# JuliaGraphics/Hikari.jl

Measured on AMD Instinct MI355X. Metric: Mrays/s, higher is better.
Workload: dtype f32

## Files before the change

hikari.jl_amd/_abi.py:

```python
import ctypes as C

c_f = C.c_float
c_i = C.c_int32
c_u = C.c_uint32
PF = C.POINTER(C.c_float)

HK_OK = 0
HK_ERR_INVALID, HK_ERR_DEVICE, HK_ERR_UNSUPPORTED = -1, -2, -3
HK_UNSET = -100

(HK_MAT_MATTE, HK_MAT_MIRROR, HK_MAT_GLASS, HK_MAT_CONDUCTOR, HK_MAT_COATED_DIFFUSE, HK_MAT_THIN_DIELECTRIC,
 HK_MAT_DIFFUSE_TRANSMISSION, HK_MAT_COATED_DIFFUSE_TRANSMISSION, HK_MAT_COATED_CONDUCTOR, HK_MAT_MIX,
 HK_MAT_FALLBACK) = range(11)
HK_MATF_REMAP_ROUGHNESS, HK_MATF_USE_ETA_K = 1, 2
(HK_LIGHT_POINT, HK_LIGHT_SPOT, HK_LIGHT_DIRECTIONAL, HK_LIGHT_SUN, HK_LIGHT_AMBIENT, HK_LIGHT_ENVIRONMENT,
 HK_LIGHT_DIFFUSE_AREA) = range(7)
HK_SPEC_RGB, HK_SPEC_ILLUMINANT = 0, 1
HK_TONEMAP_NONE, HK_TONEMAP_REINHARD, HK_TONEMAP_REINHARD_EXT, HK_TONEMAP_ACES, HK_TONEMAP_UNCHARTED2, HK_TONEMAP_FILMIC = range(6)
HK_MEDIUM_HOMOGENEOUS, HK_MEDIUM_GRID, HK_MEDIUM_RGB_GRID, HK_MEDIUM_NANOVDB = range(4)
HK_FILTER_BOX, HK_FILTER_TRIANGLE, HK_FILTER_GAUSSIAN, HK_FILTER_MITCHELL, HK_FILTER_LANCZOS = 1, 2, 3, 4, 5
HK_COHERENCE_NONE, HK_COHERENCE_SORTED, HK_COHERENCE_PER_TYPE = 0, 1, 2


class hk_texture(C.Structure):
    _fields_ = [("width", c_i), ("height", c_i), ("channels", c_i), ("kind", c_i), ("data", PF)]


class hk_tex_rgba(C.Structure):
    _fields_ = [("c", c_f * 4), ("tex", c_i)]


class hk_tex_f32(C.Structure):
    _fields_ = [("v", c_f), ("tex", c_i)]


class hk_material(C.Structure):
    _fields_ = [("kind", c_i), ("flags", c_i), ("rgb", hk_tex_rgba * 4), ("f", hk_tex_f32 * 8), ("i", c_i * 4),
                ("spectrum", c_i * 2), ("mix_key", c_u * 4)]


class hk_pl_spectrum(C.Structure):
    _fields_ = [("n", c_i), ("_pad", c_i), ("lambdas", PF), ("values", PF)]


class hk_medium_interface(C.Structure):
    _fields_ = [("material", c_i), ("inside", c_i), ("outside", c_i)]


class hk_tri_meta(C.Structure):
    _fields_ = [("medium_interface_idx", c_u), ("primitive_index", c_u), ("arealight_flat_idx_1based", c_u)]


class hk_light(C.Structure):
    _fields_ = [("kind", c_i), ("spectrum_kind", c_i), ("i_rgb", c_f * 4), ("poly", c_f * 3), ("illum_scale", c_f),
                ("scale", c_f), ("position", c_f * 3), ("direction", c_f * 3), ("world_to_light", c_f * 16),
                ("light_to_world", c_f * 16), ("cos_total_width", c_f), ("cos_falloff_start", c_f), ("v", c_f * 9),
                ("normal", c_f * 3), ("area", c_f), ("uv", c_f * 6), ("Le", hk_tex_rgba), ("two_sided", c_i),
                ("envmap", c_i)]


class hk_envmap(C.Structure):
    _fields_ = [("width", c_i), ("height", c_i), ("data", PF), ("rotation", c_f * 9), ("nu", c_i), ("nv", c_i),
                ("conditional_func", PF), ("conditional_cdf", PF), ("conditional_func_int", PF), ("marginal_func", PF),
                ("marginal_cdf", PF), ("marginal_func_int", c_f), ("_pad", c_i)]


class hk_medium(C.Structure):
    _fields_ = [("kind", c_i), ("sigma_a", c_f * 4), ("sigma_s", c_f * 4), ("Le", c_f * 4), ("g", c_f),
                ("sigma_scale", c_f), ("Le_scale", c_f), ("bounds_min", c_f * 3), ("bounds_max", c_f * 3),
                ("render_to_medium", c_f * 16), ("medium_to_render", c_f * 16), ("res", c_i * 3), ("density", PF),
                ("sigma_a_grid", PF), ("sigma_s_grid", PF), ("Le_grid", PF), ("majorant_res", c_i * 3),
                ("majorant", PF), ("max_density", c_f), ("nvdb_bytes", C.POINTER(C.c_uint8)), ("nvdb_size", C.c_int64),
                ("root_offset_1based", C.c_int64), ("upper_offset_1based", C.c_int64),
                ("lower_offset_1based", C.c_int64), ("leaf_offset_1based", C.c_int64), ("upper_count", c_i),
                ("lower_count", c_i), ("leaf_count", c_i), ("root_table_size", c_i), ("inv_mat", c_f * 9),
                ("vec", c_f * 3), ("index_bbox_min", c_i * 3), ("index_bbox_max", c_i * 3)]


class hk_scene_desc(C.Structure):
    _fields_ = [("n_triangles", c_i), ("n_materials", c_i), ("n_textures", c_i), ("n_media_interfaces", c_i),
                ("n_lights", c_i), ("n_envmaps", c_i), ("n_media", c_i), ("n_spectra", c_i), ("positions", PF),
                ("normals", PF), ("uvs", PF), ("tangents", PF), ("meta", C.POINTER(hk_tri_meta)),
                ("materials", C.POINTER(hk_material)), ("textures", C.POINTER(hk_texture)),
                ("media_interfaces", C.POINTER(hk_medium_interface)), ("lights", C.POINTER(hk_light)),
                ("envmaps", C.POINTER(hk_envmap)), ("media", C.POINTER(hk_medium)),
                ("spectra", C.POINTER(hk_pl_spectrum))]


class hk_tables(C.Structure):
    _fields_ = [("sobol_matrices", C.POINTER(c_u)), ("sobol_count", c_i), ("rgb2spec_res", c_i), ("cie_x", PF),
                ("cie_y", PF), ("cie_z", PF), ("rgb2spec_scale", PF), ("rgb2spec_coeffs", PF)]


class hk_integrator_params(C.Structure):
    _fields_ = [("max_depth", c_i), ("samples_per_pixel", c_i), ("russian_roulette_depth", c_i), ("regularize", c_i),
                ("material_coherence", c_i), ("max_component_value", c_f), ("filter_type", c_i),
                ("filter_radius", c_f * 2), ("filter_param1", c_f), ("filter_param2", c_f), ("accumulate_f64", c_i),
                ("sampler_seed", c_u), ("samples_per_pass", c_i)]


class hk_postprocess_params(C.Structure):
    _fields_ = [("exposure", c_f), ("tonemap", c_i), ("inv_gamma", c_f), ("apply_gamma", c_i), ("white_point", c_f),
                ("imaging_ratio", c_f), ("apply_wb", c_i), ("wb", c_f * 9), ("mask_escaped", c_i), ("bg", c_f * 3)]


class hk_denoise_params(C.Structure):
    _fields_ = [("iterations", c_i), ("sigma_color", c_f), ("sigma_normal", c_f), ("sigma_depth", c_f), ("use_variance", c_i)]


class hk_camera(C.Structure):
    _fields_ = [("raster_to_camera", c_f * 16), ("camera_to_world", c_f * 16), ("lens_radius", c_f),
                ("focal_distance", c_f), ("shutter_open", c_f), ("shutter_close", c_f), ("dx_camera", c_f * 3),
                ("dy_camera", c_f * 3)]


class hk_stats(C.Structure):
    _fields_ = [("rays_closest", C.c_uint64), ("rays_shadow", C.c_uint64), ("bvh_nodes_visited", C.c_uint64),
                ("tris_tested", C.c_uint64), ("hits_accepted", C.c_uint64), ("path_vertices", C.c_uint64),
                ("medium_collisions", C.c_uint64), ("light_bvh_nodes", C.c_uint64), ("seconds_trace", C.c_double),
                ("seconds_total", C.c_double), ("trace_launches", C.c_uint64), ("trace_nodes", C.c_uint64),
                ("trace_tris", C.c_uint64), ("shadow_nodes", C.c_uint64), ("shadow_tris", C.c_uint64),
                ("shadow_launches", C.c_uint64), ("shade_launches", C.c_uint64), ("seconds_shadow", C.c_double),
                ("seconds_shade", C.c_double), ("seconds_other", C.c_double), ("bytes_algorithmic_trace", C.c_uint64),
                ("bytes_algorithmic_shadow", C.c_uint64), ("bytes_algorithmic_shade", C.c_uint64), ("seconds_media", C.c_double),
                ("track_collisions", C.c_uint64), ("shadow_collisions", C.c_uint64), ("track_dda_steps", C.c_uint64),
                ("shadow_dda_steps", C.c_uint64), ("scatter_vertices", C.c_uint64), ("media_launches", C.c_uint64),
                ("bytes_algorithmic_media", C.c_uint64), ("seconds_select", C.c_double), ("select_launches", C.c_uint64),
                ("fused_passes", C.c_uint64), ("view_cache_hits", C.c_uint64)]


EXPORTED_SYMBOLS = [
    "hk_ctx_create", "hk_ctx_destroy", "hk_last_error", "hk_ctx_set_tables", "hk_scene_create", "hk_scene_destroy",
    "hk_integrator_create", "hk_integrator_destroy", "hk_film_create", "hk_film_destroy", "hk_film_clear", "hk_render",
    "hk_film_read_rgb", "hk_film_read_accum", "hk_film_accum_device_ptr", "hk_sync", "hk_stats_get", "hk_stats_reset",
    "hk_stats_enable_counters", "hk_trace_closest", "hk_test_sobol", "hk_test_camera", "hk_test_uplift",
    "hk_test_light_bvh", "hk_test_bsdf", "hk_film_postprocess", "hk_film_fill_aux", "hk_postprocess", "hk_test_light", "hk_scene_bvh_info", "hk_scene_light_bvh_copy",
    "hk_denoise", "hk_test_mix", "hk_test_medium", "hk_test_trace_lean",
    "hk_render_tile", "hk_comm_create", "hk_comm_unique_id", "hk_comm_create_rank", "hk_comm_destroy", "hk_film_reduce",
    "hk_ctx_set_option", "hk_ctx_get_option", "hk_trim_cache", "hk_flush", "hk_film_read_rgb_async", "hk_film_read_wait",
    "hk_film_pin_host", "hk_film_unpin_host", "hk_scene_set_transform", "hk_scene_update_materials", "hk_scene_update_lights", "hk_scene_update_envmap",
    "hk_film_update_aux", "hk_film_read_aux", "hk_film_present", "hk_film_present_async",
    "hk_scene_update_medium", "hk_scene_medium_copy", "hk_test_medium_bricks",
]
```

hikari.jl_amd/csrc/hk_ctx.cpp:

```cpp
#include "hk_host.h"

thread_local std::string g_err;
SlabCache g_slabs;

namespace hk {
static thread_local const Knobs* tl_knobs = nullptr;
const char* knob(const char* name) {
    if (!tl_knobs) return nullptr;
    auto it = tl_knobs->kv.find(name);
    return it == tl_knobs->kv.end() ? nullptr : it->second.c_str();
}
static const char* const KNOB_NAMES[] = {
    "HK_BATCH_PATHS_M", "HK_BVH_LEAF", "HK_BVH_BINS", "HK_QNODES", "HK_DEBUG_ALLOC", "HK_DELTA_ADVANCE", "HK_DYNAMIC_SEGMENTS", "HK_GREY", "HK_GREY_COMPACT", "HK_GREY_FLAT", "HK_MAX_PATHS_M",
    "HK_MID_LISTS", "HK_MID_PASS_PATHS_M", "HK_NODE_CACHE", "HK_NVDB_DENSE_MB", "HK_OVERLAP", "HK_PIPELINE", "HK_PIPELINE_AFTER", "HK_PIPELINE_MAX_PATHS_M", "HK_PRESELECT",
    "HK_SELECT_MIN_IDLE", "HK_SHADOW_FEED_ROUNDS", "HK_SHADOW_TRACK_BATCH", "HK_SMALL_PASS", "HK_SMALL_PASS_WAVES", "HK_SOBOL_LO_GB", "HK_SOBOL_TABLE_ONLY",
    "HK_STATE_CACHE_GB", "HK_STATE_SLAB", "HK_TICKET_SHARE", "HK_TRACK_ADVANCE", "HK_TRACK_EXTRA_ADVANCE", "HK_TRACK_MIN_PENDING", "HK_TRACK_POOL", "HK_TRACK_REFILL_IDLE",
    "HK_WALK_POOL", "HK_WALK_REFILL_IDLE", "HK_WALK_SPLIT", "HK_WAVES_PER_CU", "HK_READBACK_PIN", "HK_DEFER_EXTERNAL", "HK_SELECT_POOL", "HK_SMALL_PASS_FUSED", "HK_SMALL_PASS_MERGED", "HK_OCC_SCALE", "HK_ESCAPED_UNROLL", "HK_SHADOW_FINAL", "HK_TRI_PACK", "HK_LEAN_RECORDS", "HK_VIEW_CACHE", "HK_MAJORANT_BLOCK_VOXELS"};
static bool known_knob(const char* name) {
    for (const char* k : KNOB_NAMES)
        if (std::strcmp(k, name) == 0) return true;
    return false;
}
}
KnobScope::KnobScope(const hk::Knobs* k) : prev(hk::tl_knobs) { hk::tl_knobs = k; }
KnobScope::~KnobScope() { hk::tl_knobs = prev; }

void quiesce(hk_ctx* c) {
    if (!c) return;
    (void)hipStreamSynchronize(c->stream);
    if (c->aux) (void)hipStreamSynchronize(c->aux);
    for (auto& l : c->lanes)
        if (l.stream) (void)hipStreamSynchronize(l.stream);
}
int join_lanes(hk_ctx* c) {
    if (!c) return HK_OK;
    if (int e = flush_pending(c)) return e;
    if (!c->lanes_dirty) return HK_OK;
    for (auto& l : c->lanes)
        if (l.done) HIP_TRY(hipStreamWaitEvent(c->stream, l.done, 0));
    c->lanes_dirty = false;
    c->film_chain = false;
    if (c->have_span) HIP_TRY(hipEventRecord(c->ev_end, c->stream));
    return HK_OK;
}
hipEvent_t get_event(hk_ctx* c) {
    if (!c->event_pool.empty()) {
        hipEvent_t e = c->event_pool.back();
        c->event_pool.pop_back();
        return e;
    }
    hipEvent_t e;
    (void)hipEventCreate(&e);
    return e;
}
DCamera make_camera(const hk_camera& c) {
    DCamera d;
    std::memcpy(d.r2c, c.raster_to_camera, 64);
    std::memcpy(d.c2w, c.camera_to_world, 64);
    d.lens_radius = c.lens_radius;
    d.focal_distance = c.focal_distance;
    d.shutter_open = c.shutter_open;
    d.shutter_close = c.shutter_close;
    return d;
}

extern "C" const char* hk_last_error(void) { return g_err.c_str(); }

extern "C" int32_t hk_ctx_create(int32_t device_id, void* stream, hk_ctx** out) {
    if (!out) return fail(HK_ERR_INVALID, "out is null");
    int n = 0;
    HIP_TRY(hipGetDeviceCount(&n));
    if (device_id < 0 || device_id >= n) return fail(HK_ERR_INVALID, "bad device id");
    HIP_TRY(hipSetDevice(device_id));
    hk_ctx* c = new hk_ctx();
    c->device = device_id;
    c->stream = (hipStream_t)stream;
    hipDeviceProp_t prop;
    HIP_TRY(hipGetDeviceProperties(&prop, device_id));
    c->n_cu = prop.multiProcessorCount > 0 ? prop.multiProcessorCount : 256;
    c->own_stream_order = stream == nullptr;
    for (const char* name : hk::KNOB_NAMES)
        if (const char* e = std::getenv(name)) c->knobs.kv[name] = e;
    KnobScope knobs(&c->knobs);
    {
        c->waves_per_cu = hk::knob_int_in("HK_WAVES_PER_CU", 1, INT_MAX, 0);
        c->stat_rows = c->n_cu * 32 * 2;
        if (const char* e = hk::knob("HK_OVERLAP")) c->overlap = std::atoi(e) ? 1 : 0;
        else c->overlap = -1;
        if (const char* e = hk::knob("HK_STATE_CACHE_GB"))
            if (std::atol(e) >= 0) g_slabs.cap_bytes = (size_t)std::atol(e) << 30;
    }
    {
        std::vector<DStats> zero((size_t)c->stat_rows);
        std::memset(zero.data(), 0, zero.size() * sizeof(DStats));
        HIP_TRY(c->stats.upload(zero.data(), zero.size() * sizeof(DStats)));
    }
    HIP_TRY(hipEventCreate(&c->ev_begin));
    HIP_TRY(hipEventCreate(&c->ev_end));
    *out = c;
    return HK_OK;
}
extern "C" int32_t hk_ctx_destroy(hk_ctx* c) {
    if (!c) return HK_OK;
    (void)hipSetDevice(c->device);
    int status = join_lanes(c);
    if (hipStreamSynchronize(c->stream) != hipSuccess && status == HK_OK) status = fail(HK_ERR_DEVICE, "hk_ctx_destroy: the context's stream reports an error");
    for (auto& l : c->lanes) {
        if (l.stream) (void)hipStreamSynchronize(l.stream);
        if (l.done) (void)hipEventDestroy(l.done);
        if (l.stream) (void)hipStreamDestroy(l.stream);
    }
    if (c->ev_main) (void)hipEventDestroy(c->ev_main);
    if (c->ev_film) (void)hipEventDestroy(c->ev_film);
    for (auto& e : c->trace_events) {
        (void)hipEventDestroy(e.first);
        (void)hipEventDestroy(e.second);
    }
    for (auto e : c->event_pool) (void)hipEventDestroy(e);
    if (c->ev_begin) (void)hipEventDestroy(c->ev_begin);
    if (c->ev_end) (void)hipEventDestroy(c->ev_end);
    if (c->ev_fork) (void)hipEventDestroy(c->ev_fork);
    if (c->ev_join) (void)hipEventDestroy(c->ev_join);
    if (c->aux) (void)hipStreamDestroy(c->aux);
    g_slabs.trim(c->device);
    delete c;
    return status;
}
extern "C" int32_t hk_ctx_set_option(hk_ctx* c, const char* name, const char* value) {
    if (!c || !name) return fail(HK_ERR_INVALID, "null argument");
    if (!hk::known_knob(name)) return fail(HK_ERR_INVALID, std::string("unknown option ") + name);
    HIP_TRY(hipSetDevice(c->device));
    if (int e = join_lanes(c)) return e;
    if (value) c->knobs.kv[name] = value;
    else c->knobs.kv.erase(name);
    if (std::strcmp(name, "HK_STATE_CACHE_GB") == 0) {
        g_slabs.cap_bytes = (size_t)(value && std::atol(value) >= 0 ? std::atol(value) : 128) << 30;
        if (g_slabs.cap_bytes == 0) g_slabs.trim(c->device);
    }
    return HK_OK;
}
extern "C" int32_t hk_ctx_get_option(hk_ctx* c, const char* name, char* out, int32_t out_bytes) {
    if (!c || !name || (out_bytes > 0 && !out)) return fail(HK_ERR_INVALID, "null argument");
    if (!hk::known_knob(name)) return fail(HK_ERR_INVALID, std::string("unknown option ") + name);
    auto it = c->knobs.kv.find(name);
    if (it == c->knobs.kv.end()) {
        if (out_bytes > 0) out[0] = 0;
        return HK_UNSET;
    }
    if (out_bytes > 0) std::snprintf(out, (size_t)out_bytes, "%s", it->second.c_str());
    return (int32_t)it->second.size();
}
extern "C" int32_t hk_flush(hk_ctx* c) {
    if (!c) return fail(HK_ERR_INVALID, "null ctx");
    HIP_TRY(hipSetDevice(c->device));
    return join_lanes(c);
}
extern "C" int32_t hk_trim_cache(hk_ctx* c) {
    if (!c) return fail(HK_ERR_INVALID, "null ctx");
    HIP_TRY(hipSetDevice(c->device));
    g_slabs.trim(c->device);
    return HK_OK;
}
extern "C" int32_t hk_ctx_set_tables(hk_ctx* c, const hk_tables* t) {
    if (!c || !t || !t->sobol_matrices || t->sobol_count < 104 || !t->cie_x || !t->rgb2spec_coeffs) return fail(HK_ERR_INVALID, "bad tables");
    HIP_TRY(hipSetDevice(c->device));
    if (int e = flush_pending(c)) return e;
    if (c->lanes_dirty) {
        if (int e = join_lanes(c)) return e;
        HIP_TRY(hipStreamSynchronize(c->stream));
    }
    HIP_TRY(c->sobol.upload(t->sobol_matrices, 104 * sizeof(uint32_t)));
    std::vector<float> cie(3 * 471);
    std::memcpy(&cie[0], t->cie_x, 471 * 4);
    std::memcpy(&cie[471], t->cie_y, 471 * 4);
    std::memcpy(&cie[942], t->cie_z, 471 * 4);
    HIP_TRY(c->cie.upload(cie.data(), cie.size() * 4));
    int res = t->rgb2spec_res;
    size_t nco = (size_t)3 * res * res * res * 3;
    c->h_r2s_scale.assign(t->rgb2spec_scale, t->rgb2spec_scale + res);
    c->h_r2s_coeffs.assign(t->rgb2spec_coeffs, t->rgb2spec_coeffs + nco);
    c->r2s_host.res = res;
    c->r2s_host.scale = c->h_r2s_scale.data();
    c->r2s_host.coeffs = c->h_r2s_coeffs.data();
    HIP_TRY(c->r2s_scale.upload(t->rgb2spec_scale, res * 4));
    HIP_TRY(c->r2s_coeffs.upload(t->rgb2spec_coeffs, nco * 4));
    {
        const size_t R = (size_t)res;
        std::vector<float> pts(3 * R * R * R * 4);
        for (size_t m = 0; m < 3; ++m)
            for (size_t z = 0; z < R; ++z)
                for (size_t y = 0; y < R; ++y)
                    for (size_t x = 0; x < R; ++x) {
                        float* o = &pts[((((m * R + z) * R + y) * R) + x) * 4];
                        for (size_t k = 0; k < 3; ++k) o[k] = t->rgb2spec_coeffs[m + 3 * (z + R * (y + R * (x + R * k)))];
                        o[3] = 0.0f;
                    }
        HIP_TRY(c->r2s_points.upload(pts.data(), pts.size() * 4));
        bool sorted = true;
        for (int i = 1; i < res; ++i)
            if (!(t->rgb2spec_scale[i - 1] <= t->rgb2spec_scale[i])) sorted = false;
        c->tables.rgb2spec_sorted = sorted ? 1 : 0;
    }
    bool closed = true;
    {
        uint32_t col = 0x80000000u;
        for (int b = 0; b < 52; ++b) {
            uint32_t d0 = b < 32 ? (0x80000000u >> b) : 0u;
            if (t->sobol_matrices[b] != d0) closed = false;
            if (b % 32 == 0) col = 0x80000000u;
            if (t->sobol_matrices[52 + b] != col) closed = false;
            col ^= col >> 1;
        }
    }
    c->tables.sobol = closed ? nullptr : c->sobol.as<uint32_t>();
    c->tables.cie = c->cie.as<float>();
    c->tables.rgb2spec_scale = c->r2s_scale.as<float>();
    c->tables.rgb2spec_coeffs = c->r2s_coeffs.as<float>();
    c->tables.rgb2spec_res = res;
    c->tables.rgb2spec_points = c->r2s_points.as<float4>();
    c->have_tables = true;
    c->tables_epoch++;
    return HK_OK;
}

extern "C" int32_t hk_sync(hk_ctx* c) {
    if (!c) return fail(HK_ERR_INVALID, "null ctx");
    HIP_TRY(hipSetDevice(c->device));
    if (int e = join_lanes(c)) return e;
    HIP_TRY(hipStreamSynchronize(c->stream));
    if (c->aux) HIP_TRY(hipStreamSynchronize(c->aux));
    return HK_OK;
}
extern "C" int32_t hk_stats_enable_counters(hk_ctx* c, int32_t flags) {
    if (!c) return fail(HK_ERR_INVALID, "null ctx");
    if (int e = join_lanes(c)) return e;
    c->count_nodes = (flags & 1) ? 1 : 0;
    c->time_kernels = (flags & 2) ? 1 : 0;
    return HK_OK;
}
extern "C" int32_t hk_stats_reset(hk_ctx* c) {
    if (!c) return fail(HK_ERR_INVALID, "null ctx");
    HIP_TRY(hipSetDevice(c->device));
    if (int e = join_lanes(c)) return e;
    HIP_TRY(hipStreamSynchronize(c->stream));
    HIP_TRY(hipMemset(c->stats.p, 0, (size_t)c->stat_rows * sizeof(DStats)));
    for (auto& l : c->lanes)
        if (l.stats.p) HIP_TRY(hipMemset(l.stats.p, 0, (size_t)c->stat_rows * sizeof(DStats)));
    for (auto& e : c->trace_events) {
        c->event_pool.push_back(e.first);
        c->event_pool.push_back(e.second);
    }
    c->trace_events.clear();
    for (auto& v : c->class_events) {
        for (auto& e : v) {
            c->event_pool.push_back(e.first);
            c->event_pool.push_back(e.second);
        }
        v.clear();
    }
    c->seconds_trace = c->seconds_total = 0.0;
    c->trace_launches = c->shadow_launches = c->shade_launches = c->media_launches = c->select_launches = 0;
    c->fused_passes = c->view_cache_hits = 0;
    c->have_span = false;
    return HK_OK;
}
extern "C" int32_t hk_stats_get(hk_ctx* c, hk_stats* out) {
    if (!c || !out) return fail(HK_ERR_INVALID, "null argument");
    HIP_TRY(hipSetDevice(c->device));
    if (int e = join_lanes(c)) return e;
    HIP_TRY(hipStreamSynchronize(c->stream));
    DStats h{};
    {
        std::vector<const void*> blocks{c->stats.p};
        for (const auto& l : c->lanes)
            if (l.stats.p) blocks.push_back(l.stats.p);
        std::vector<DStats> rows((size_t)c->stat_rows * blocks.size());
        for (size_t b = 0; b < blocks.size(); ++b)
            HIP_TRY(hipMemcpy(rows.data() + b * (size_t)c->stat_rows, blocks[b], (size_t)c->stat_rows * sizeof(DStats), hipMemcpyDeviceToHost));
        for (const DStats& r : rows) {
            h.rays_closest += r.rays_closest;
            h.rays_shadow += r.rays_shadow;
            h.nodes += r.nodes;
            h.tris += r.tris;
            h.hits += r.hits;
            h.vertices += r.vertices;
            h.collisions += r.collisions;
            h.light_nodes += r.light_nodes;
            h.sh_nodes += r.sh_nodes;
            h.sh_tris += r.sh_tris;
            h.sh_collisions += r.sh_collisions;
            h.nvdb_collisions += r.nvdb_collisions;
            h.sh_nvdb_collisions += r.sh_nvdb_collisions;
            h.dda_steps += r.dda_steps;
            h.sh_dda_steps += r.sh_dda_steps;
            h.scatter_vertices += r.scatter_vertices;
            h.sc_light_nodes += r.sc_light_nodes;
#ifdef HK_DEBUG_UTIL
            for (int k = 0; k < 32; ++k) h.dbg[k] += r.dbg[k];
#endif
        }
#ifdef HK_DEBUG_UTIL
        for (int k = 0; k < 16; ++k)
            if (h.dbg[2 * k]) std::fprintf(stderr, "HK_DEBUG_UTIL[%d]: %.3f of %llu lane-slots\n", k, (double)h.dbg[2 * k + 1] / (double)h.dbg[2 * k], h.dbg[2 * k]);
#endif
    }
    double tr = 0.0;
    for (auto& e : c->trace_events) {
        float ms = 0.0f;
        if (hipEventElapsedTime(&ms, e.first, e.second) == hipSuccess) tr += ms * 1e-3;
    }
    double total = 0.0;
    if (c->have_span) {
        float ms = 0.0f;
        if (hipEventElapsedTime(&ms, c->ev_begin, c->ev_end) == hipSuccess) total = ms * 1e-3;
    }
    std::memset(out, 0, sizeof *out);
    out->rays_closest = h.rays_closest;
    out->rays_shadow = h.rays_shadow;
    out->bvh_nodes_visited = h.nodes;
    out->tris_tested = h.tris;
    out->hits_accepted = h.hits;
    out->path_vertices = h.vertices;
    out->medium_collisions = h.collisions + h.sh_collisions;
    out->track_collisions = h.collisions;
    out->shadow_collisions = h.sh_collisions;
    out->track_dda_steps = h.dda_steps;
    out->shadow_dda_steps = h.sh_dda_steps;
    out->scatter_vertices = h.scatter_vertices;
    out->light_bvh_nodes = h.light_nodes + h.sc_light_nodes;
    out->seconds_trace = tr;
    out->seconds_total = total;
    out->trace_launches = c->trace_launches;
    out->trace_nodes = h.nodes;
    out->trace_tris = h.tris;
    out->shadow_nodes = h.sh_nodes;
    out->shadow_tris = h.sh_tris;
    out->bvh_nodes_visited = h.nodes + h.sh_nodes;
    out->tris_tested = h.tris + h.sh_tris;
    out->shadow_launches = c->shadow_launches;
    out->shade_launches = c->shade_launches;
    out->media_launches = c->media_launches;
    double cls[6] = {0, 0, 0, 0, 0, 0};
    for (int k = 1; k < 6; ++k)
        for (auto& e : c->class_events[k]) {
            float ms = 0.0f;
            if (hipEventElapsedTime(&ms, e.first, e.second) == hipSuccess) cls[k] += ms * 1e-3;
        }
    out->seconds_shadow = cls[1];
    out->seconds_shade = cls[2] + cls[5];
    out->seconds_other = cls[3];
    out->seconds_media = cls[4];
    out->seconds_select = cls[5];
    out->select_launches = c->select_launches;
    out->fused_passes = c->fused_passes;
    out->view_cache_hits = c->view_cache_hits;
    {
        const uint64_t hits_closest = h.hits < h.rays_closest ? h.hits : h.rays_closest;
        out->bytes_algorithmic_trace = h.rays_closest * (32 + 16) + 64 * h.nodes + 36 * h.tris + 96 * hits_closest;
        out->bytes_algorithmic_shadow = h.rays_shadow * (32 + 16) + 64 * h.sh_nodes + 36 * h.sh_tris;
        out->bytes_algorithmic_shade = h.vertices * (2 * 104 + 64 + 96) + 60 * h.light_nodes;
        out->bytes_algorithmic_media = h.collisions * 36 + h.nvdb_collisions * (84 - 36) + 4 * h.dda_steps + h.scatter_vertices * (2 * 104 + 96) + 60 * h.sc_light_nodes;
        out->bytes_algorithmic_shadow += h.sh_collisions * 36 + h.sh_nvdb_collisions * (84 - 36) + 4 * h.sh_dda_steps;
    }
    return HK_OK;
}
```

hikari.jl_amd/csrc/hk_host.h:

```cpp
#pragma once
#include <hip/hip_runtime.h>

#include <climits>
#include <cstddef>
#include <cmath>
#include <cstdio>
#include <cstdlib>
#include <cstring>
#include <limits>
#include <map>
#include <memory>
#include <mutex>
#include <string>
#include <unordered_map>
#include <vector>

#include "bvh_build.h"
#include "hikari_mi355x.h"
#include "hk_launch.h"
#include "hk_nanovdb.h"
#include "hk_types.h"

#pragma GCC visibility push(hidden)

extern thread_local std::string g_err;
inline int fail(int code, const std::string& msg) {
    g_err = msg;
    return code;
}

namespace hk {
struct Knobs {
    std::unordered_map<std::string, std::string> kv;
};
}
struct KnobScope {
    const hk::Knobs* prev;
    explicit KnobScope(const hk::Knobs* k);
    ~KnobScope();
};
#define HIP_TRY(expr)                                                                                          \
    do {                                                                                                       \
        hipError_t e_ = (expr);                                                                                \
        if (e_ != hipSuccess) return fail(HK_ERR_DEVICE, std::string(#expr) + ": " + hipGetErrorString(e_)); \
    } while (0)

struct SlabCache {
    struct Entry {
        void* p;
        size_t bytes;
        int dev;
    };
    std::mutex m;
    std::vector<Entry> free_list;
    size_t cap_bytes = (size_t)128 << 30;
    size_t cap() const { return cap_bytes; }
    size_t total(int dev) {
        std::lock_guard<std::mutex> g(m);
        size_t t = 0;
        for (const Entry& e : free_list) t += e.dev == dev ? e.bytes : 0;
        return t;
    }
    void* take(int dev, size_t need, size_t& got) {
        std::lock_guard<std::mutex> g(m);
        int best = -1;
        for (int i = 0; i < (int)free_list.size(); ++i) {
            const Entry& e = free_list[i];
            if (e.dev == dev && e.bytes >= need && e.bytes <= 2 * need + ((size_t)64 << 20) && (best < 0 || e.bytes < free_list[best].bytes)) best = i;
        }
        if (best < 0) return nullptr;
        void* p = free_list[best].p;
        got = free_list[best].bytes;
        free_list.erase(free_list.begin() + best);
        return p;
    }
    void give(int dev, void* p, size_t bytes) {
        std::vector<void*> drop;
        {
            std::lock_guard<std::mutex> g(m);
            free_list.push_back(Entry{p, bytes, dev});
            size_t t = 0;
            for (const Entry& e : free_list) t += e.bytes;
            const size_t limit = cap();
            while (!free_list.empty() && (t > limit || free_list.size() > 8)) {
                int k = 0;
                for (int i = 1; i < (int)free_list.size(); ++i)
                    if (free_list[i].bytes < free_list[k].bytes) k = i;
                t -= free_list[k].bytes;
                drop.push_back(free_list[k].p);
                free_list.erase(free_list.begin() + k);
            }
        }
        for (void* q : drop) (void)hipFree(q);
    }
    void trim(int dev) {
        std::vector<void*> drop;
        {
            std::lock_guard<std::mutex> g(m);
            for (int i = (int)free_list.size() - 1; i >= 0; --i)
                if (dev < 0 || free_list[i].dev == dev) {
                    drop.push_back(free_list[i].p);
                    free_list.erase(free_list.begin() + i);
                }
        }
        for (void* q : drop) (void)hipFree(q);
    }
};
extern SlabCache g_slabs;
struct DevBuf {
    void* p = nullptr;
    size_t bytes = 0;
    int slab_dev = -1;
    void release() {
        if (p && slab_dev >= 0) {
            g_slabs.give(slab_dev, p, bytes);
        } else if (p)
            (void)hipFree(p);
        p = nullptr, bytes = 0, slab_dev = -1;
    }
    ~DevBuf() { release(); }
    hipError_t alloc(size_t n) {
        release();
        bytes = n;
        if (n == 0) return hipSuccess;
        hipError_t e = hipMalloc(&p, n);
        if (e != hipSuccess) {
            (void)hipGetLastError();
            g_slabs.trim(-1);
            e = hipMalloc(&p, n);
        }
        if (e != hipSuccess) p = nullptr, bytes = 0;
        return e;
    }
    hipError_t alloc_slab(int dev, size_t n) {
        release();
        size_t got = 0;
        if (void* q = g_slabs.take(dev, n, got)) {
            p = q, bytes = got, slab_dev = dev;
            return hipSuccess;
        }
        const hipError_t e = alloc(n);
        if (e == hipSuccess) slab_dev = dev;
        return e;
    }
    hipError_t upload(const void* src, size_t n) {
        hipError_t e = alloc(n ? n : 4);
        if (e != hipSuccess) return e;
        if (n) e = hipMemcpy(p, src, n, hipMemcpyHostToDevice);
        return e;
    }
    template <class T>
    T* as() const {
        return reinterpret_cast<T*>(p);
    }
};

struct hk_ctx {
    int device = 0;
    hk::Knobs knobs;
    bool own_stream_order = true;
    hipStream_t stream = nullptr;
    hipStream_t aux = nullptr;
    hipEvent_t ev_fork = nullptr, ev_join = nullptr;
    int overlap = -1;
    int small_streak = 0;
    int n_cu = 256;
    int waves_per_cu = 0;
    int stat_rows = 8192;
    DevBuf sobol, cie, r2s_scale, r2s_coeffs, r2s_points, stats;
    DTables tables{};
    bool have_tables = false;
    unsigned tables_epoch = 0;
    std::vector<float> h_r2s_scale, h_r2s_coeffs;
    hk::RGB2Spec r2s_host;
    int count_nodes = 0, time_kernels = 0;
    unsigned long long fused_passes = 0;
    unsigned long long view_cache_hits = 0;
    std::vector<std::pair<hipEvent_t, hipEvent_t>> trace_events;
    std::vector<std::pair<hipEvent_t, hipEvent_t>> class_events[6];
    uint64_t shadow_launches = 0, shade_launches = 0, media_launches = 0, select_launches = 0;
    std::vector<hipEvent_t> event_pool;
    hipEvent_t ev_begin = nullptr, ev_end = nullptr;
    bool have_span = false;
    double seconds_trace = 0.0, seconds_total = 0.0;
    uint64_t trace_launches = 0;
    DStats host_stats{};
    struct Lane {
        hipStream_t stream = nullptr;
        hipEvent_t done = nullptr;
        DevBuf stats;
    };
    enum { MAX_LANES = 16 };
    Lane lanes[MAX_LANES];
    int next_lane = 0;
    struct Pending {
        bool active = false;
        hk_scene* sc = nullptr;
        hk_integrator* I = nullptr;
        hk_film* film = nullptr;
        hk_camera cam{};
        int first = 0, n = 0, stride = 1, x0 = 0, y0 = 0, x1 = 0, y1 = 0, calls = 0;
    } pending;
    bool lanes_dirty = false;
    bool film_chain = false;
    hipEvent_t ev_main = nullptr, ev_film = nullptr;
};

void quiesce(hk_ctx* c);
int flush_pending(hk_ctx* c);
int join_lanes(hk_ctx* c);
hipEvent_t get_event(hk_ctx* c);
DCamera make_camera(const hk_camera& c);

struct hk_scene {
    hk_ctx* ctx = nullptr;
    DevBuf nodes, qnodes, leaf_tris, positions, normals, uvs, tangents, meta, tri_shade, materials, textures, spectra, mis, lights, lnodes, trails, infinite;
    DevBuf envmaps;
    DevBuf media;
    DScene d{};
    uint32_t kinds_mask = 0;
    int n_materials = 0;
    int bvh_nodes = 0, bvh_leaf_tris = 0, bvh_depth = 0;
    hk::LightBVH lbvh;
    std::vector<hk_material> h_materials;
    std::vector<hk_light> h_lights;
    std::vector<DEnvMap> h_envmaps;
    int n_textures = 0, n_spectra = 0;
    std::vector<int> level_start;
    DevBuf base_pos, base_nrm, base_tan, slot_of_prim;
    bool have_base = false;
    bool qnodes_built = false;
    enum { XF_BLOCK = 1024 };
    std::vector<float> block_box;
    struct Xf {
        int end;
        bool identity;
        float m[12];
    };
    std::map<int, Xf> xf;
    struct Staging {
        void* host = nullptr;
        size_t bytes = 0;
        hipEvent_t ev = nullptr;
    };
    std::vector<Staging> staging;
    struct Medium {
        hk_medium rec{};
        DMedium d{};
        DevBuf *majorant = nullptr, *maj_zero = nullptr, *density = nullptr, *rgb[3] = {nullptr, nullptr, nullptr};
        DevBuf *nvdb = nullptr, *blocks = nullptr, *bricks = nullptr;
    };
    std::vector<Medium> h_media;
    std::vector<std::unique_ptr<DevBuf>> owned;
    DevBuf& own() {
        owned.emplace_back(new DevBuf());
        return *owned.back();
    }
    ~hk_scene() {
        for (auto& st : staging) {
            if (st.ev) (void)hipEventSynchronize(st.ev), (void)hipEventDestroy(st.ev);
            if (st.host) (void)hipHostFree(st.host);
        }
    }
};
void bake_material(const hk::RGB2Spec& t, const hk_material& m, DMaterial& o);
bool material_alpha_tested(const hk_material& m);
void bake_light(const hk::RGB2Spec& r2s, const hk_light& l, DLight& o);
std::string check_medium_record(const hk_medium& m);
void bake_medium_fields(const hk::RGB2Spec& r2s, const hk_medium& m, DMedium& o);
struct NvdbPlan {
    int nvb_min[3] = {0, 0, 0}, nvb_dim[3] = {0, 0, 0};
    float background = 0.0f;
    long long total = 0;
    std::vector<uint2> table;
    bool bricks = false;
    void fill(DMedium& o) const;
};
int plan_nanovdb(const hk_medium& m, NvdbPlan& p);
struct MediaClasses {
    int media_mask = 0, all_grey = 0, grey_pool = 0, grey_bricks = 0;
};
MediaClasses classify_media(const std::vector<DMedium>& dmed, int n_media);
inline size_t light_table_capacity(int n_lights) { return n_lights > 0 ? (size_t)n_lights : 1; }

struct hk_film {
    hk_ctx* ctx = nullptr;
    int width = 0, height = 0;
    bool f64 = false;
    DevBuf own;
    void* accum = nullptr;
    bool external = false;
    bool exposed = false;
    DevBuf readback;
    float* staging[2] = {nullptr, nullptr};
    int staging_next = 0, staging_last = -1;
    bool read_in_flight = false;
    hipEvent_t ev_read = nullptr;
    void* last_out = nullptr;
    void* pinned_user = nullptr;
    bool pinned_explicit = false;
    void* pin_failed = nullptr;
    DevBuf guides, albedo;
    DevBuf frame[2], variance;
    bool have_aux = false;
};

struct hk_integrator {
    hk_ctx* ctx = nullptr;
    hk_integrator_params p{};
    DFilter filter{};
    DevBuf f_func, f_mcdf, f_mfunc, f_ccdf;
    DPathState st{};
    std::vector<std::unique_ptr<DevBuf>> bufs;
    int st_capacity = 0, st_depth = 0, st_media = -1;
    DPathGen cam_gen{};
    bool cam_unfit = false;
    std::string view_key;
    bool mid_pass = false;
    int slab_mode = 0;
    void* slab_base = nullptr;
    size_t slab_off = 0;
    DevBuf sobol_table;
    int sobol_rows = 0, sobol_stride = 0, sobol_log2 = -1, sobol_digits = -1, sobol_x0 = -1, sobol_y0 = -1, sobol_tiles_x = -1;
    DevBuf sobol_lo;
    int lo_rows = 0, lo_base = -1, lo_sample_stride = -1, lo_count = 0;
    struct StateSet {
        DPathState st{};
        std::vector<std::unique_ptr<DevBuf>> bufs;
        int st_capacity = 0, st_depth = 0, st_media = -1;
        DPathGen cam_gen{};
        bool cam_unfit = false;
        std::string view_key;
    };
    std::vector<StateSet> lane_sets;
    void swap_set(StateSet& o) {
        std::swap(st, o.st);
        std::swap(bufs, o.bufs);
        std::swap(st_capacity, o.st_capacity);
        std::swap(st_depth, o.st_depth);
        std::swap(st_media, o.st_media);
        std::swap(cam_gen, o.cam_gen);
        std::swap(cam_unfit, o.cam_unfit);
        std::swap(view_key, o.view_key);
    }
};
int ceil_log2(long v);
DSobol make_sobol(const hk_integrator_params& p, int w, int h);

struct hk_comm {
    std::vector<hk_ctx*> ctxs;
    std::vector<void*> comms;
    int world = 1;
};

#pragma GCC visibility pop
```

hikari.jl_amd/csrc/hk_kernels.hip:

```cpp
#include <hip/hip_runtime.h>
#include <type_traits>
#include <cstdlib>
#include <cstdio>

#include "hikari_mi355x.h"
#include "hk_device.h"

using namespace hkd;

namespace {

__device__ __forceinline__ int lane_id() { return (int)(threadIdx.x & 63); }

struct WaveQ {
    uint32_t* base;
    int count;
};
__device__ __forceinline__ int global_wave() {
    const int w = (int)(threadIdx.x >> 6), b = (int)blockIdx.x;
    if (blockDim.x == 1024 && (gridDim.x & 7) == 0) return ((((b >> 3) * 4 + (w >> 2)) * 8 + (b & 7)) << 2) + (w & 3);
    if (blockDim.x == 512 && (gridDim.x & 7) == 0) return ((((b >> 3) * 2 + (w >> 2)) * 8 + (b & 7)) << 2) + (w & 3);
    return b * (int)(blockDim.x >> 6) + w;
}
__device__ __forceinline__ int physical_waves() { return (int)(gridDim.x * (blockDim.x >> 6)); }
// ... 589 lines not shown
#ifndef HK_LEAF_BREAK_A
#define HK_LEAF_BREAK_A 2
#endif
#ifndef HK_POSTPONE_CLOSEST
#define HK_POSTPONE_CLOSEST 0
#endif
#ifndef HK_POSTPONE_ANYHIT
#define HK_POSTPONE_ANYHIT 0
#endif
#ifndef HK_NODE_UNROLL
#define HK_NODE_UNROLL 3
#endif
struct LaneRay {
    v3 o, d;
    RaySlab rs;
    float t_max;
    HitRec best;
    int cur, sp;
    int pend;
    bool any;
};
template <bool QN = false>
HKD void lane_ray_start(LaneRay& r, const DScene& sc, v3 o, v3 d, float t_max) {
    r.o = o;
    r.d = d;
    r.t_max = t_max;
    r.best.t = t_max;
    r.best.prim = -1;
    r.best.u = r.best.v = 0.0f;
    r.rs = QN ? ray_slab_grid(sc, o, d) : ray_slab(o, d);
    r.sp = 0;
    r.cur = sc.n_tris == 0 ? (int)0x80000000 : sc.root_ref;
    r.pend = (int)0x80000000;
    r.any = false;
}
template <bool ANYHIT, bool COUNT, int NC = 0, bool POSTPONE = (ANYHIT ? HK_POSTPONE_ANYHIT != 0 : HK_POSTPONE_CLOSEST != 0), bool MIXED = false, bool QN = false>
HKD void lane_ray_round(LaneRay& r, bool active, const DScene& sc, int* __restrict__ stack, int lane, unsigned& n_nodes, unsigned& n_tris, const NodeCache& cache = NodeCache(),
                        bool may_wait = false
#ifdef HK_DEBUG_UTIL
                        , unsigned long long* dbg_ = nullptr
#endif
                        ) {
    const int DONE = (int)0x80000000;
    const unsigned long long act_m = __builtin_amdgcn_ballot_w64(active);
    const int break_a = (!ANYHIT && NC > 0 && sc.n_nodes <= NC) ? HK_LEAF_BREAK_A : 1;
    for (;;) {
        const unsigned long long in_nodes = act_m & __builtin_amdgcn_ballot_w64(r.cur >= 0);
        if (in_nodes == 0ull) break;
        const int n_desc = __builtin_popcountll(in_nodes), n_leaf = __builtin_popcountll(act_m & __builtin_amdgcn_ballot_w64((unsigned)r.cur > 0x80000000u));
        if (break_a * n_desc < n_leaf) break;
#ifdef HK_DEBUG_UTIL
        if (dbg_) HK_DBG(0, active && r.cur >= 0);
#endif
#pragma unroll
        for (int rep = 1; rep < HK_NODE_UNROLL; ++rep)
            if (active && r.cur >= 0) {
                if (COUNT) ++n_nodes;
                node_step<NC, QN>(sc, r.rs, r.best.t, stack, lane, r.cur, r.sp, cache);
            }
        if (active && r.cur >= 0) {
            if (COUNT) ++n_nodes;
            node_step<NC, QN>(sc, r.rs, r.best.t, stack, lane, r.cur, r.sp, cache);
            if (POSTPONE) {
                if (r.cur == DONE) {
                    r.cur = r.pend;
                    r.pend = DONE;
                } else if (r.cur < 0 && r.pend == DONE && r.sp > 0) {
                    r.pend = r.cur;
                    --r.sp;
                    r.cur = stack[r.sp * 64 + lane];
                }
            }
        }
    }
    constexpr int LEAF_MIN = ANYHIT ? (NC > 0 ? HK_ANYHIT_LEAF_MIN : 0) : HK_CLOSEST_LEAF_MIN;
    static_assert(LEAF_MIN == 0 || 64 - 2 * LEAF_MIN >= HK_TRACE_MIN_IDLE, "waiting leaf holders must leave enough idle lanes for the caller's refill to trigger");
    if (LEAF_MIN > 0 && may_wait && __builtin_popcountll(act_m & __builtin_amdgcn_ballot_w64((unsigned)r.cur > 0x80000000u)) < LEAF_MIN) return;
    const bool has_pend = POSTPONE && r.pend != DONE;
#ifdef HK_DEBUG_UTIL
    if (dbg_) HK_DBG(1, active && (has_pend || (r.cur < 0 && r.cur != DONE)));
#endif
#ifdef HK_DEBUG_UTIL
    if (dbg_) {
        const bool holds = active && (has_pend || (r.cur < 0 && r.cur != DONE));
        int c = holds ? ((~(has_pend ? r.pend : r.cur)) & 7) + 1 : 0, mx = c, sm = c;
        for (int off = 32; off > 0; off >>= 1) {
            mx = max(mx, __shfl_xor(mx, off));
            sm += __shfl_xor(sm, off);
        }
        dbg_[ANYHIT ? 8 : 12] += 64ull * (unsigned)mx;
        dbg_[ANYHIT ? 9 : 13] += (unsigned)sm;
    }
#endif
    if (active && (has_pend || (r.cur < 0 && r.cur != DONE))) {
        int ref = ~(has_pend ? r.pend : r.cur);
        int first = ref >> 3, count = (ref & 7) + 1;
        bool stop = false;
        if (!ANYHIT && !MIXED) {
            const float4* tp = sc.leaf_tris + 3 * (size_t)first;
            float4 T0 = tp[0], T1 = tp[1], T2 = tp[2];
            for (int i = 0; i < count; ++i) {
                float4 N0 = T0, N1 = T1, N2 = T2;
                if (i + 1 < count) N0 = tp[3 * i + 3], N1 = tp[3 * i + 4], N2 = tp[3 * i + 5];
                asm volatile("" ::"v"(T0.x), "v"(T0.y), "v"(T0.z), "v"(T0.w));
                if (COUNT) ++n_tris;
                float t, u, v;
                if (intersect_triangle(r.o, r.d, r.t_max, mk3(T0.x, T0.y, T0.z), mk3(T1.x, T1.y, T1.z), mk3(T2.x, T2.y, T2.z), t, u, v)) {
                    int prim = __float_as_int(T0.w);
                    if (r.best.prim < 0 || t < r.best.t || (t == r.best.t && prim < r.best.prim)) {
                        r.best.t = t;
                        r.best.prim = prim;
                        r.best.u = u;
                        r.best.v = v;
                    }
                }
                T0 = N0, T1 = N1, T2 = N2;
            }
        } else
        for (int i = 0; i < count && !stop; ++i) {
            const float4* tp = sc.leaf_tris + 3 * (size_t)(first + i);
            float4 T0 = tp[0], T1 = tp[1], T2 = tp[2];
            asm volatile("" ::"v"(T0.x), "v"(T0.y), "v"(T0.z), "v"(T0.w));
            if (COUNT) ++n_tris;
            float t, u, v;
            if (intersect_triangle(r.o, r.d, r.t_max, mk3(T0.x, T0.y, T0.z), mk3(T1.x, T1.y, T1.z), mk3(T2.x, T2.y, T2.z), t, u, v)) {
                int prim = __float_as_int(T0.w);
                if (MIXED ? r.any : ANYHIT) {
                    r.best.t = t;
                    r.best.prim = prim;
                    stop = true;
                } else if (r.best.prim < 0 || t < r.best.t || (t == r.best.t && prim < r.best.prim)) {
                    r.best.t = t;
                    r.best.prim = prim;
                    r.best.u = u;
                    r.best.v = v;
                }
            }
        }
        if (stop) {
            r.cur = DONE;
            if (POSTPONE) r.pend = DONE;
        } else if (has_pend)
            r.pend = DONE;
        else if (r.sp > 0) {
            --r.sp;
            r.cur = stack[r.sp * 64 + lane];
        } else
            r.cur = DONE;
    }
}

enum { LR_EMPTY = 0, LR_ACTIVE = 1 };

template <bool COUNT, int NC, bool QN = false, int MIN_IDLE = HK_TRACE_MIN_IDLE>
__device__ __forceinline__ void trace_lean_body(const DPathState& st, const DScene& sc, int depth, DStats* stats, const SegTickets& src, int* __restrict__ stack, const NodeCache& cache) {
    const int lane = lane_id();
    const unsigned long long lt_mask = (1ull << lane) - 1ull;
    const int DONE = (int)0x80000000;
    unsigned n_nodes = 0, n_tris = 0, n_casts = 0, n_hits = 0;
    HK_DBG_DECL
    HK_FOR_EACH_SEGMENT_FROM(gw, st, src) {
    const DPathGen g = gen_at(st, depth);
    const uint32_t seg = (uint32_t)gw * (uint32_t)st.wave_cap;
    const int n = *count_ptr(st, depth, Q_RAY, gw);
    WaveQ q_escaped = wq_open(st.escaped_q, st, gw);
    int kind_count[HK_MAX_KINDS];
#pragma unroll
    for (int k = 0; k < HK_MAX_KINDS; ++k) kind_count[k] = 0;
    int cursor = 0;
    int state = LR_EMPTY;
    uint32_t slot = 0;
    LaneRay r;
    r.cur = r.pend = DONE;
    for (;;) {
        const unsigned long long run_m = __ballot(state == LR_ACTIVE && r.cur != DONE);
        if (run_m == 0ull || (64 - __popcll(run_m) >= MIN_IDLE && cursor < n)) {
            HK_DBG(8, state == LR_ACTIVE && r.cur == DONE);
            int kind = -1;
            if (state == LR_ACTIVE && r.cur == DONE) {
                if (r.best.prim < 0)
                    kind = -2;
                else {
                    ++n_hits;
                    const DTriMeta hm = sc.meta[r.best.prim];
                    int mat = sc.mis[hm.mi].material;
                    if (sc.materials[mat].kind == HK_MAT_MIX) {
                        float w = 1.0f - r.best.u - r.best.v;
                        mat = resolve_mix_material(sc, mat, r.o + r.d * r.best.t, -r.d, uv_at(sc, r.best.prim, w, r.best.u, r.best.v));
                    }
                    kind = sc.materials[mat].kind;
                    if (kind == HK_MAT_MIX) kind = HK_MAT_FALLBACK;
                    stream_st(&st.hit[slot], make_float4(r.best.t, __int_as_float(r.best.prim), r.best.u, r.best.v));
                    stream_st(reinterpret_cast<uint32_t*>(st.mat_id) + slot, (uint32_t)(mat | (hm.arealight > 0 ? HK_MAT_EMISSIVE_BIT : 0)));
                }
                state = LR_EMPTY;
            }
            wq_push(q_escaped, slot, kind == -2);
            unsigned long long pending = __ballot(kind >= 0);
            while (pending) {
                int src = __ffsll((long long)pending) - 1;
                const int k = __builtin_amdgcn_readlane(kind, src);
                bool mine = kind == k;
                unsigned long long m = __ballot(mine);
                int cnt = 0;
#pragma unroll
                for (int kk = 0; kk < HK_MAX_KINDS; ++kk) cnt = (kk == k) ? kind_count[kk] : cnt;
                if (mine) stream_st(&st.mat_q[((size_t)k * st.n_waves + gw) * st.wave_cap + cnt + __popcll(m & lt_mask)], slot);
                int add = __popcll(m);
#pragma unroll
                for (int kk = 0; kk < HK_MAX_KINDS; ++kk) kind_count[kk] += (kk == k) ? add : 0;
                pending &= ~m;
            }
            const unsigned long long want = __ballot(state == LR_EMPTY);
            const int avail = n - cursor;
            const int rank = __popcll(want & lt_mask);
            if (state == LR_EMPTY && rank < avail) {
                slot = seg + (uint32_t)(cursor + rank);
                float4 O = ld_ray_o(st, g, slot, depth, seg), D = stream_ld(&g.ray_d[slot]);
                ++n_casts;
                lane_ray_start<QN>(r, sc, mk3(O.x, O.y, O.z), mk3(D.x, D.y, D.z), O.w);
                state = LR_ACTIVE;
            }
            const int want_n = __popcll(want);
            cursor += want_n < avail ? want_n : (avail > 0 ? avail : 0);
            if (__ballot(state == LR_ACTIVE) == 0ull) break;
        }
#ifdef HK_DEBUG_UTIL
        HK_DBG(2, state == LR_ACTIVE && r.cur != DONE);
        lane_ray_round<false, COUNT, NC, HK_POSTPONE_CLOSEST != 0, false, QN>(r, state == LR_ACTIVE && r.cur != DONE, sc, stack, lane, n_nodes, n_tris, cache, cursor < n, dbg_);
#else
        lane_ray_round<false, COUNT, NC, HK_POSTPONE_CLOSEST != 0, false, QN>(r, state == LR_ACTIVE && r.cur != DONE, sc, stack, lane, n_nodes, n_tris, cache, cursor < n);
#endif
    }
    wq_close(q_escaped, count_ptr(st, depth, Q_ESCAPED, gw));
    if (lane == 0) {
        *count_ptr(st, depth, Q_MEDIUM, gw) = 0;
#pragma unroll
        for (int k = 0; k < HK_MAX_KINDS; ++k) *count_ptr(st, depth, Q_MAT0 + k, gw) = kind_count[k];
    }
    }
    stats += global_wave();
    wave_add(&stats->rays_closest, n_casts);
    wave_add(&stats->hits, n_hits);
    if (COUNT) {
        wave_add(&stats->nodes, n_nodes);
        wave_add(&stats->tris, n_tris);
    }
    HK_DBG_FLUSH(stats);
}
template <bool COUNT, int STACK, int BLOCK = HK_TRACE_BLOCK, int NC = 0, bool QN = false>
__global__ void __launch_bounds__(BLOCK) k_trace_lean(DPathState st, DScene sc, int depth, DStats* stats) {
    __shared__ int lds_stack[(BLOCK / 64) * STACK * 64];
    __shared__ float4 lds_box[NC > 0 ? 3 * NC : 1];
    __shared__ int2 lds_child[NC > 0 ? NC : 1];
    int* stack = lds_stack + (threadIdx.x >> 6) * (STACK * 64);
    const NodeCache cache = node_cache_fill<NC, BLOCK, QN>(sc, lds_box, lds_child);
    trace_lean_body<COUNT, NC, QN, (NC >= 1024 ? HK_CLOSEST_MIN_IDLE_LDS : HK_TRACE_MIN_IDLE)>(st, sc, depth, stats, seg_open(st, ticket_ptr(st, depth, TK_TRACE), st.dynamic_segments != 0, depth, Q_RAY), stack, cache);
}

#ifndef HK_REFILL_MIN_IDLE
#define HK_REFILL_MIN_IDLE 8
#endif
#ifndef HK_MEDIA_WAVES
#define HK_MEDIA_WAVES 2
#endif
#ifndef HK_TRACK_ADVANCE
#define HK_TRACK_ADVANCE 4
#endif
#ifndef HK_DELTA_ADVANCE
#define HK_DELTA_ADVANCE 6
#endif
#ifndef HK_SKIP_ZERO
#define HK_SKIP_ZERO 0
#endif
#ifndef HK_GREY_TRACK_WAVES
#define HK_GREY_TRACK_WAVES 4
#endif
enum { TR_BUSY = -101, TR_EMPTY = -100, TR_SCATTER = -3, TR_ESCAPED = -2 };

struct TrackSeg {
    int gw;
    int esc, sca;
    int kind_count[HK_MAX_KINDS];
};
template <int MM, bool GREY = false>
__global__ void __attribute__((amdgpu_flat_work_group_size(256, 256), amdgpu_waves_per_eu(GREY ? HK_GREY_TRACK_WAVES : HK_MEDIA_WAVES))) k_track(DPathState st, DScene sc, DTables T, DFrame fr, int depth, DStats* stats, const DMedium* __restrict__ media) {
    const int lane = lane_id();
    const unsigned long long lt_mask = (1ull << lane) - 1ull;
    unsigned n_coll = 0, n_dda = 0;
    const DPathGen g = gen_at(st, depth);
    const bool ones = depth == 0 && fr.implicit_ones;
    SegStream stream = stream_open(st, ticket_ptr(st, depth, TK_TRACK), true, depth, Q_MEDIUM);
    TrackSeg seg[2];
    seg[0].gw = seg[1].gw = -1;
    int cur_tag = 0;
    const uint32_t* __restrict__ queue = st.medium_q;
    int n = 0, cursor = 0;
    bool more = true;
    auto open_seg = [&](TrackSeg& s, int gw) {
        s.gw = gw;
        s.esc = *count_ptr(st, depth, Q_ESCAPED, gw);
        s.sca = 0;
#pragma unroll
        for (int k = 0; k < HK_MAX_KINDS; ++k) s.kind_count[k] = *count_ptr(st, depth, Q_MAT0 + k, gw);
    };
    auto close_seg = [&](TrackSeg& s) {
        if (s.gw >= 0 && lane == 0) {
            *count_ptr(st, depth, Q_SCATTER, s.gw) = s.sca;
            *count_ptr(st, depth, Q_ESCAPED, s.gw) = s.esc;
#pragma unroll
            for (int k = 0; k < HK_MAX_KINDS; ++k) *count_ptr(st, depth, Q_MAT0 + k, s.gw) = s.kind_count[k];
        }
        s.gw = -1;
    };
    {
        int state = TR_EMPTY, tag = 0;
        uint32_t slot = 0, pslot = 0;
        v3 ro = mk3(0, 0, 0), rd = mk3(0, 0, 1), cur_o = mk3(0, 0, 0);
        S4 lambda = s4(0.0f), beta = s4(0.0f), r_u = s4(0.0f), r_l = s4(0.0f), base_a = s4(0.0f), base_s = s4(0.0f), base_Le = s4(0.0f), sm = s4(0.0f);
        float a0 = 0.0f, s0 = 0.0f, rl_f = 1.0f;
        bool dead_null = false;
        uint64_t rng = 0;
        MajorantIter it = exhausted_iter();
        float seg1 = 0.0f, sm0 = 0.0f, t = 0.0f;
        bool in_seg = false, pending = false;
        float pend_dt = 0.0f;
        int k_in_seg = 0, segi = 0, medium_idx = 0;
        for (;;) {
            const unsigned long long busy_m = __ballot(state == TR_BUSY);
            if (busy_m == 0ull || (64 - __popcll(busy_m) >= fr.refill_idle && (cursor < n || more))) {
#pragma unroll
                for (int tg = 0; tg < 2; ++tg) {
                    TrackSeg& S = seg[tg];
                    const bool sel = tag == tg && state != TR_BUSY && state != TR_EMPTY;
                    if (__ballot(sel) == 0ull) continue;
                    const size_t base = (size_t)S.gw * st.wave_cap;
                    {
                        const unsigned long long m = __ballot(sel && state == TR_SCATTER);
                        if (sel && state == TR_SCATTER) st.scatter_q[base + S.sca + __popcll(m & lt_mask)] = slot;
                        S.sca += __popcll(m);
                    }
                    {
                        const unsigned long long m = __ballot(sel && state == TR_ESCAPED);
                        if (sel && state == TR_ESCAPED) st.escaped_q[base + S.esc + __popcll(m & lt_mask)] = slot;
                        S.esc += __popcll(m);
                    }
                    unsigned long long todo_k = __ballot(sel && state >= 0);
                    while (todo_k) {
                        int src = __ffsll((long long)todo_k) - 1;
                        const int k = __builtin_amdgcn_readlane(state, src);
                        bool mine = sel && state == k;
                        unsigned long long m = __ballot(mine);
                        int cnt = 0;
#pragma unroll
                        for (int kk = 0; kk < HK_MAX_KINDS; ++kk) cnt = (kk == k) ? S.kind_count[kk] : cnt;
                        if (mine) st.mat_q[((size_t)k * st.n_waves + S.gw) * st.wave_cap + cnt + __popcll(m & lt_mask)] = slot;
                        int add = __popcll(m);
#pragma unroll
                        for (int kk = 0; kk < HK_MAX_KINDS; ++kk) S.kind_count[kk] += (kk == k) ? add : 0;
                        todo_k &= ~m;
                    }
                }
                if (state != TR_BUSY) state = TR_EMPTY;
                while (more && cursor >= n) {
                    const int other = cur_tag ^ 1;
                    const bool other_busy = __ballot(state == TR_BUSY && tag == other) != 0ull;
                    if (other_busy) break;
                    if (other == 0) close_seg(seg[0]); else close_seg(seg[1]);
                    const int gw = stream_next(stream, st.n_waves);
                    if (gw >= st.n_waves) {
                        more = false;
                        break;
                    }
                    if (other == 0) open_seg(seg[0], gw); else open_seg(seg[1], gw);
                    cur_tag = other;
                    queue = st.medium_q + (size_t)gw * st.wave_cap;
                    n = *count_ptr(st, depth, Q_MEDIUM, gw);
                    cursor = 0;
                }
                const unsigned long long want = __ballot(state == TR_EMPTY);
                const int avail = n - cursor;
                const int rank = __popcll(want & lt_mask);
                if (state == TR_EMPTY && rank < avail) {
                    slot = queue[cursor + rank];
                    tag = cur_tag;
                    float4 O = g.ray_o[slot], D = g.ray_d[slot];
                    ro = mk3(O.x, O.y, O.z);
                    rd = mk3(D.x, D.y, D.z);
                    const float t_max = st.hit[slot].x;
                    const uint2 meta = g.meta[slot];
                    medium_idx = (int)(meta.x >> 16) - 1;
                    pslot = meta.y;
                    const DMedium& med = sc.n_media == 1 ? media[0] : media[medium_idx];
                    if constexpr (GREY) {
                        a0 = eval_flat(med.sigma_a);
                        s0 = eval_flat(med.sigma_s);
                        base_a = s4(a0);
                        base_s = s4(s0);
                        rl_f = 1.0f;
                        dead_null = is_black(ld_throughput(g.beta, slot, ones)) || is_black(ld_throughput(g.r_u, slot, ones));
                    } else {
                        lambda = ld_lambda(st, g, slot, pslot);
                        beta = ld_throughput(g.beta, slot, ones);
                        r_u = ld_throughput(g.r_u, slot, ones);
                        r_l = ld_throughput(g.r_l, slot, ones);
                        base_a = eval_scaled(med.sigma_a, lambda);
                        base_s = eval_scaled(med.sigma_s, lambda);
                        if (HK_HAS_MEDIUM(MM, HK_MEDIUM_HOMOGENEOUS)) base_Le = eval_scaled(med.Le, lambda);
                    }
                    rng = lcg_init(ro, rd, t_max);
// ... 1164 lines not shown
                        int pix, k;
                        split_slot(fr, ld_meta(st, g, e, depth).y, pix, k);
                        const SobolCtx sctx = sobol_ctx_slot(sob, T.sobol, fr.x0, fr.y0, fr.tiles_x, pix, k, fr.first_sample + k * fr.sample_stride);
                        const float u = sobol_1d<FT>(sctx, base_dim + 1);
                        int res_light = 0;
                        float res_pmf = 0.0f;
                        if (ninf + nbvh > 0) {
                            if (ninf > 0 && u < p_inf) {
                                const float ur = u / p_inf;
                                int idx = (int)floorf(ur * (float)ninf);
                                idx = (idx < ninf - 1 ? idx : ninf - 1) + 1;
                                res_pmf = p_inf / (float)ninf;
                                res_light = sc.infinite_lights[idx - 1];
                            } else if (has_bvh) {
                                u_b = ninf > 0 ? minf((u - p_inf) / (1.0f - p_inf), 0.99999994f) : minf(u, 0.99999994f);
                                if (root_bits & 2u) {
                                    res_pmf = 1.0f - p_inf;
                                    res_light = (int)root_child;
                                } else
                                    descend = true;
                            }
                        }
                        if (!descend) st.sel_light[e] = make_uint2((uint32_t)res_light, __float_as_uint(res_pmf));
                    }
                    cursor += take;
                    const unsigned long long dm = __ballot(descend);
                    if (descend) {
                        const int at = __popcll(dm & lt_mask);
                        pool[0][at] = e;
                        pool[1][at] = __float_as_uint(sp.x), pool[2][at] = __float_as_uint(sp.y), pool[3][at] = __float_as_uint(sp.z);
                        pool[4][at] = __float_as_uint(sn.x), pool[5][at] = __float_as_uint(sn.y), pool[6][at] = __float_as_uint(sn.z);
                        pool[7][at] = __float_as_uint(u_b);
                    }
                    pool_n = __popcll(dm);
                    __builtin_amdgcn_wave_barrier();
                }
            }
            const int avail = pool_n - pool_head;
            if (avail > 0) {
                const int rank = __popcll(free_m & lt_mask);
                if (!busy && rank < avail) {
                    const int at = pool_head + rank;
                    slot = pool[0][at];
                    p = mk3(__uint_as_float(pool[1][at]), __uint_as_float(pool[2][at]), __uint_as_float(pool[3][at]));
                    nn = mk3(__uint_as_float(pool[4][at]), __uint_as_float(pool[5][at]), __uint_as_float(pool[6][at]));
                    ub = __uint_as_float(pool[7][at]);
                    pmf = 1.0f - p_inf;
                    bits = root_bits, child = root_child;
                    lvl = 0;
                    busy = true;
                }
                const int free_n = __popcll(free_m);
                pool_head += free_n < avail ? free_n : avail;
            }
            if (__ballot(busy) == 0ull) {
                if (!more && pool_head == pool_n) break;
                continue;
            }
        }
        if (busy) {
            int res_light = -1;
            float res_pmf = 0.0f;
            if (lvl >= 64) {
                res_light = 0;
            } else {
                ++lvl;
                DLightNode n0, n1;
                if (NTOP > 0 && (int)child + 1 < n_top) {
                    n0 = lds_light_node<NTOP>(top, (int)child), n1 = lds_light_node<NTOP>(top, (int)child + 1);
                    asm volatile("" : "+v"(n0.bits));
                } else
                    n0 = load_light_node(sc.lnodes, (int)child), n1 = load_light_node(sc.lnodes, (int)child + 1);
                const float c0 = node_importance(n0, p, nn);
                const float c1 = node_importance(n1, p, nn);
                n_lnodes += 2;
                if (c0 == 0.0f && c1 == 0.0f) {
                    res_light = 0;
                } else {
                    const float p0 = c0 / (c0 + c1);
                    if (ub < p0) {
                        pmf *= p0;
                        ub = ub / p0;
                        bits = n0.bits, child = n0.child1_or_light;
                    } else {
                        pmf *= (1.0f - p0);
                        ub = (ub - p0) / (1.0f - p0);
                        bits = n1.bits, child = n1.child1_or_light;
                    }
                    if ((bits & 2u) && lvl < 64) {
                        res_light = (int)child;
                        res_pmf = pmf;
                    }
                }
            }
            if (res_light >= 0) {
                st.sel_light[slot] = make_uint2((uint32_t)res_light, __float_as_uint(res_pmf));
                busy = false;
            }
        }
    }
    stats += global_wave();
    wave_add(&stats->light_nodes, n_lnodes);
}

#ifndef HK_SHADE_WAVES_MATTE
#define HK_SHADE_WAVES_MATTE 4
#endif
#ifndef HK_SHADE_WAVES
#define HK_SHADE_WAVES 3
#endif
template <bool TWO_PLANES, bool SIMPLE>
HKD void shade_emission(const DPathState& st, const DPathGen& g, bool ones, const DScene& sc, const DTables& T, uint32_t slot, unsigned& n_lnodes, int depth, size_t seg) {
    const float4 H = st.hit[slot];
    const float4 O = ld_ray_o(st, g, slot, depth, seg), D = g.ray_d[slot];
    const v3 ro = mk3(O.x, O.y, O.z), rd = mk3(D.x, D.y, D.z);
    const float t_hit = H.x;
    const int prim = __float_as_int(H.y);
    const DTriMeta meta = tri_meta(sc, prim);
    if (meta.arealight <= 0) return;
    const Surface sf = surface_at(sc, prim, H.z, H.w, ro, rd, t_hit);
    const v3 wo = -rd;
    const uint2 pmeta = ld_meta(st, g, slot, depth);
    const S4 lambda = ld_lambda(st, g, slot, pmeta.y);
    const DLight& light = sc.lights[meta.arealight - 1];
    S4 Le = arealight_Le<TWO_PLANES, SIMPLE>(sc, T, light, wo, sf.n, sf.uv, lambda);
    if (is_black(Le)) return;
    const S4 beta = ld_throughput(g.beta, slot, ones), r_u = ld_ru(g, slot, ones, st.compact != 0), r_l = ld_rl(g, slot, ones, st.compact != 0);
    const uint32_t fl = pmeta.x;
    const int pdepth = (int)(fl & 0xff);
    const bool specular_bounce = (fl >> 8) & 1u;
    S4 contribution = beta * Le;
    S4 fin;
    if (pdepth == 0 || specular_bounce)
        fin = contribution / average(r_u);
    else {
        float choice = bvh_pmf(sc, sf.pi, sf.n, (int)meta.arealight, n_lnodes);
        float ct = fabsf(dot(sf.n, normalize(rd)));
        float light_pdf = 0.0f;
        if (ct > 0.0f && sf.area > 0.0f) light_pdf = choice * ((t_hit * t_hit) / (ct * sf.area));
        S4 rl = r_l * light_pdf;
        float den = average(r_u + rl);
        fin = den > 1e-10f ? contribution / den : contribution / average(r_u);
    }
    st4(&st.L[pmeta.y], ld4(&st.L[pmeta.y]) + fin);
}

template <int KIND>
struct ShadeWaves {
    static constexpr int value = (KIND == HK_MAT_COATED_DIFFUSE || KIND == HK_MAT_COATED_DIFFUSE_TRANSMISSION) ? 1 : (KIND == HK_MAT_MATTE ? HK_SHADE_WAVES_MATTE : HK_SHADE_WAVES);
};
#ifndef HK_SHADE_MIN_WAVES
#define HK_SHADE_MIN_WAVES 1
#endif
template <int KIND, bool SIMPLE, bool FT, bool PRE>
__device__ __forceinline__ void shade_body(const DPathState& st, const DScene& sc, const DTables& T, const DFrame& fr, const DSobol& sob, int depth, int first_kind, DStats* stats, const SegTickets& src,
                                           uint32_t* __restrict__ elist) {
    const int lane = lane_id();
    unsigned n_vertices = 0, n_lnodes = 0;
    HK_FOR_EACH_SEGMENT_FROM(gw, st, src) {
    const uint32_t* __restrict__ queue = st.mat_q + ((size_t)KIND * st.n_waves + gw) * st.wave_cap;
    const int n = *count_ptr(st, depth, Q_MAT0 + KIND, gw);
    const DPathGen g = gen_at(st, depth), gn = st.gen[(depth + 1) & 1];
    const size_t seg = (size_t)gw * st.wave_cap;
    const bool ones = depth == 0 && fr.implicit_ones;
    WavePos q_shadow{0}, q_next{0};
    if (!first_kind) {
        q_shadow.count = *count_ptr(st, depth, Q_SHADOW, gw);
        q_next.count = *count_ptr(st, depth + 1, Q_RAY, gw);
    }
    {
        int n_emit = 0;
        for (int base = 0; base < n || n_emit > 0; base += 64) {
            if (base < n) {
                const int i = base + lane;
                const uint32_t cand = i < n ? queue[i] : 0u;
                const bool em = i < n && (st.mat_id[cand] & HK_MAT_EMISSIVE_BIT) != 0;
                const unsigned long long m = __ballot(em);
                if (em) elist[n_emit + __popcll(m & ((1ull << lane) - 1ull))] = cand;
                n_emit += __popcll(m);
                if (n_emit < 64 && base + 64 < n) continue;
            }
            __builtin_amdgcn_fence(__ATOMIC_SEQ_CST, "wavefront");
            const int take = n_emit < 64 ? n_emit : 64;
            if (lane < take) shade_emission<KIND == HK_MAT_MATTE, SIMPLE>(st, g, ones, sc, T, elist[lane], n_lnodes, depth, seg);
            const int rest = n_emit - take;
            const uint32_t moved = lane < rest ? elist[64 + lane] : 0u;
            __builtin_amdgcn_fence(__ATOMIC_SEQ_CST, "wavefront");
            if (lane < rest) elist[lane] = moved;
            n_emit = rest;
        }
    }
    for (int base = 0; base < n; base += 64) {
        int i = base + lane;
        bool active = i < n;
        uint32_t slot = active ? queue[i] : 0u;
        bool push_shadow = false, push_ray = false;
        float4 H = make_float4(0, 0, 0, 0);
        Surface sf;
        v3 wo = mk3(0, 0, 1);
        DTriMeta meta{0u, 0u, 0u};
        S4 lambda = s4(0.0f), beta = s4(0.0f), r_u = s4(0.0f), kd_matte = s4(0.0f);
        uint32_t fl = 0, pslot = 0;
        int pdepth = 0, medium = -1;
        bool any_non_specular = false;
        SobolCtx sctx;
        const int base_dim = 6 + 7 * depth;
        float4 shO = make_float4(0, 0, 0, 0), shD = shO;
        S4 shLd = s4(0.0f), shRu = s4(0.0f), shRl = s4(0.0f);
        if (active) {
            ++n_vertices;
            H = stream_ld(&st.hit[slot]);
            float4 O = ld_ray_o(st, g, slot, depth, seg), D = stream_ld(&g.ray_d[slot]);
            v3 ro = mk3(O.x, O.y, O.z), rd = mk3(D.x, D.y, D.z);
            float t_hit = H.x;
            int prim = __float_as_int(H.y);
            sf = surface_at(sc, prim, H.z, H.w, ro, rd, t_hit);
            wo = -rd;
            meta = tri_meta(sc, prim);
            const uint2 pmeta = ld_meta(st, g, slot, depth);
            lambda = ld_lambda(st, g, slot, pmeta.y);
            if (ones)
                beta = s4(1.0f);
            else {
                const float4 bv = stream_ld(&g.beta[slot]);
                beta = s4(bv.x, bv.y, bv.z, bv.w);
            }
            r_u = ld_ru(g, slot, ones, st.compact != 0);
            fl = pmeta.x;
            pslot = pmeta.y;
            pdepth = (int)(fl & 0xff);
            any_non_specular = (fl >> 9) & 1u;
            medium = (int)(fl >> 16) - 1;

            int pix, k;
            split_slot(fr, pslot, pix, k);
            sctx = sobol_ctx_slot(sob, T.sobol, fr.x0, fr.y0, fr.tiles_x, pix, k, fr.first_sample + k * fr.sample_stride);

            if (KIND == HK_MAT_MATTE) kd_matte = matte_kd<SIMPLE>(sc, T, sc.materials[st.mat_id[slot] & ~HK_MAT_EMISSIVE_BIT], TexCtx(sf.uv, meta.prim_index, H.z, H.w), lambda);
#ifdef HK_ABLATE
            {
                float sink = 0.0f;
                if (HK_ABLATE == 1) {
                    uint32_t ps2 = pslot;
                    int d2 = base_dim;
                    asm volatile("" : "+v"(ps2));
                    asm volatile("" : "+s"(d2));
                    int pix2, k2;
                    split_slot(fr, ps2, pix2, k2);
                    SobolCtx c2 = sobol_ctx_slot(sob, T.sobol, fr.x0, fr.y0, fr.tiles_x, pix2, k2, fr.first_sample + k2 * fr.sample_stride);
                    v2 a = sobol_2d(c2, d2 + 3), b = sobol_2d(c2, d2 + 6);
                    sink = sobol_1d(c2, d2 + 1) + a.x + a.y + b.x + b.y + sobol_1d(c2, d2 + 7);
                }
                if (HK_ABLATE == 2 && sc.n_lights > 0) {
                    float u2 = H.z, pmf2;
                    asm volatile("" : "+v"(u2));
                    unsigned dummy = 0;
                    sink = (float)bvh_sample_light(sc, sf.pi, sf.ns, u2, pmf2, dummy) + pmf2;
                }
                if (HK_ABLATE == 3 && sc.n_lights > 0) {
                    uint32_t li = pslot;
                    asm volatile("" : "+v"(li));
                    LightSample l2 = sample_light(sc, T, sc.lights[li % (uint32_t)sc.n_lights], sf.pi, lambda, mk2(H.z, H.w));
                    sink = l2.pdf + l2.Li.x + l2.Li.w + l2.wi.x + l2.p_light.z;
                }
                if (HK_ABLATE == 4) {
                    S4 l2 = lambda;
                    asm volatile("" : "+v"(l2.x), "+v"(l2.y), "+v"(l2.z), "+v"(l2.w));
                    S4 k2 = matte_kd(sc, T, sc.materials[st.mat_id[slot] & ~HK_MAT_EMISSIVE_BIT], TexCtx(sf.uv, meta.prim_index, H.z, H.w), l2);
                    sink = k2.x + k2.y + k2.z + k2.w;
                }
                if (HK_ABLATE == 5) {
                    float b2 = H.z;
                    asm volatile("" : "+v"(b2));
                    Surface s2 = surface_at(sc, prim, b2, H.w, ro, rd, t_hit);
                    sink = s2.pi.x + s2.n.y + s2.ns.z + s2.uv.x + s2.area;
                }
                if (HK_ABLATE == 6) {
                    v3 w2 = wo;
                    asm volatile("" : "+v"(w2.x), "+v"(w2.y), "+v"(w2.z));
                    float p2;
                    S4 f2 = eval_matte_kd(kd_matte, w2, sf.n, sf.ns, p2);
                    BSDFSample s2 = sample_matte_kd(sc, sc.materials[st.mat_id[slot] & ~HK_MAT_EMISSIVE_BIT], kd_matte, w2, sf.ns, TexCtx(sf.uv, meta.prim_index, H.z, H.w), mk2(H.z, H.w));
                    sink = f2.x + f2.w + p2 + s2.pdf + s2.wi.x + s2.f.y;
                }
                asm volatile("" : : "v"(sink));
            }
#endif

            if (sc.n_lights > 0) {
                const DMaterial& mat = sc.materials[st.mat_id[slot] & ~HK_MAT_EMISSIVE_BIT];
                float light_pmf;
                int light_idx;
                if constexpr (PRE) {
                    const uint2 pre = st.sel_light[slot];
                    light_idx = (int)pre.x;
                    light_pmf = __uint_as_float(pre.y);
                } else {
                    float light_select = sobol_1d<FT>(sctx, base_dim + 1);
                    light_idx = bvh_sample_light(sc, sf.pi, sf.ns, light_select, light_pmf, n_lnodes);
                }
                if (light_idx >= 1 && light_idx <= sc.n_lights && light_pmf > 0.0f) {
                    const DLight& sel = sc.lights[light_idx - 1];
                    v2 u_light = mk2(0.0f, 0.0f);
                    if (sel.kind >= HK_LIGHT_AMBIENT) u_light = sobol_2d<FT>(sctx, base_dim + 3);
                    LightSample ls = sample_light<KIND == HK_MAT_MATTE, SIMPLE>(sc, T, sel, sf.pi, lambda, u_light);
                    if (ls.pdf > 0.0f && !is_black(ls.Li)) {
                        float bsdf_pdf;
                        S4 f = KIND == HK_MAT_MATTE ? eval_matte_kd(kd_matte, wo, ls.wi, sf.ns, bsdf_pdf)
                                                    : eval_bsdf<KIND>(sc, T, mat, wo, ls.wi, sf.ns, TexCtx(sf.uv, meta.prim_index, H.z, H.w), lambda, bsdf_pdf);
                        if (!is_black(f)) {
                            float ct = fabsf(dot(ls.wi, sf.ns));
                            S4 Ld = beta * f * ls.Li * ct;
                            if (!is_black(Ld)) {
                                v3 off = 1e-4f * sf.ns;
                                v3 so = dot(ls.wi, sf.ns) > 0.0f ? sf.pi + off : sf.pi - off;
                                v3 tl = ls.p_light - so;
                                float tmax = sqrtf(dot(tl, tl)) - 1e-3f;
                                float nbp = ls.is_delta ? 0.0f : bsdf_pdf;
                                shO = make_float4(so.x, so.y, so.z, tmax);
                                shD = make_float4(ls.wi.x, ls.wi.y, ls.wi.z, __int_as_float(medium));
                                shLd = Ld;
                                shRu = r_u * nbp;
                                shRl = (r_u * ls.pdf) * light_pmf;
                                push_shadow = true;
                            }
                        }
                    }
                }
            }
        }
        {
            const size_t ps = seg + (size_t)wp_push(q_shadow, push_shadow);
            if (push_shadow && st.sh_final) {
                const S4 mis = s4(shRu.x) * s4(1.0f) + s4(shRl.x) * s4(1.0f);
                shD.w = average(mis);
                stream_st(&st.sh_o[ps], shO);
                stream_st(&st.sh_d[ps], shD);
                stream_st(&st.sh_Ld[ps], shLd);
                stream_st(&st.sh_slot[ps], pslot);
            } else if (push_shadow) {
                stream_st(&st.sh_o[ps], shO);
                stream_st(&st.sh_d[ps], shD);
                stream_st(&st.sh_Ld[ps], shLd);
                if (st.compact) {
#if HK_NT
                    __builtin_nontemporal_store((hk_f2){shRu.x, shRl.x}, (hk_f2*)(reinterpret_cast<float2*>(st.sh_ru) + ps));
#else
                    reinterpret_cast<float2*>(st.sh_ru)[ps] = make_float2(shRu.x, shRl.x);
#endif
                } else
                    st_shadow_weights(st, ps, shRu, shRl);
                stream_st(&st.sh_slot[ps], pslot);
            }
        }
        float4 nO = make_float4(0, 0, 0, 0), nD = nO;
        S4 nb = s4(0.0f), nrl = s4(0.0f);
        uint32_t nflags = 0;
        if (active) {
            int new_depth = pdepth + 1;
            if (new_depth < fr.max_depth) {
                const DMaterial& mat = sc.materials[st.mat_id[slot] & ~HK_MAT_EMISSIVE_BIT];
                const DMediumInterface mi = sc.mis[meta.mi];
                float uc = (KIND == HK_MAT_GLASS || KIND > HK_MAT_CONDUCTOR) && KIND != HK_MAT_FALLBACK ? sobol_1d<FT>(sctx, base_dim + 4) : 0.0f;
                v2 u = (KIND == HK_MAT_MIRROR || KIND == HK_MAT_GLASS || KIND == HK_MAT_THIN_DIELECTRIC) ? mk2(0.0f, 0.0f) : sobol_2d<FT>(sctx, base_dim + 6);
                bool regularize = fr.regularize && any_non_specular;
                BSDFSample s = KIND == HK_MAT_MATTE ? sample_matte_kd<SIMPLE>(sc, mat, kd_matte, wo, sf.ns, TexCtx(sf.uv, meta.prim_index, H.z, H.w), u)
                                                    : sample_bsdf<KIND>(sc, T, mat, wo, sf.ns, TexCtx(sf.uv, meta.prim_index, H.z, H.w), lambda, u, uc, regularize);
                if (s.pdf > 0.0f && !is_black(s.f)) {
                    float ct = fabsf(dot(s.wi, sf.ns));
                    nb = s.is_specular ? beta * s.f : beta * s.f * ct / s.pdf;
                    nrl = s.is_specular ? r_u : r_u / s.pdf;
                    bool cont = true;
                    if (new_depth > 3) {
                        float rr = sobol_1d<FT>(sctx, base_dim + 7);
                        float q = maxf(0.05f, 1.0f - max_component(nb));
                        if (rr < q)
                            cont = false;
                        else
                            nb = nb * (1.0f / (1.0f - q));
                    }
                    if (cont) {
                        int new_medium = (mi.inside != mi.outside) ? (dot(s.wi, sf.n) > 0.0f ? mi.outside : mi.inside) : medium;
                        v3 off = dot(s.wi, sf.n) > 0.0f ? sf.n : -sf.n;
                        v3 no = sf.pi + off * 0.0001f;
                        nO = make_float4(no.x, no.y, no.z, INF_F);
                        nD = make_float4(s.wi.x, s.wi.y, s.wi.z, 0.0f);
                        bool ans = any_non_specular || !s.is_specular;
                        nflags = (uint32_t)new_depth | ((s.is_specular ? 1u : 0u) << 8) | ((ans ? 1u : 0u) << 9) | ((uint32_t)(new_medium + 1) << 16);
                        push_ray = true;
                    }
                }
            }
        }
        {
            const size_t pn = seg + (size_t)wp_push(q_next, push_ray);
            if (push_ray) {
                stream_st(&gn.ray_o[pn], nO);
                if (st.compact) nD.w = nrl.x;
                stream_st(&gn.ray_d[pn], nD);
                stream_st(&gn.beta[pn], nb);
                st_ru_rl(gn, pn, r_u, nrl, st.compact != 0);
                st_lambda(gn, pn, lambda);
                st_meta(st, gn, pn, nflags, pslot);
            }
        }
    }
    if (lane == 0) {
        *count_ptr(st, depth, Q_SHADOW, gw) = q_shadow.count;
        *count_ptr(st, depth + 1, Q_RAY, gw) = q_next.count;
    }
    }
    stats += global_wave();
    wave_add(&stats->vertices, n_vertices);
    wave_add(&stats->light_nodes, n_lnodes);
}
template <int KIND, bool SIMPLE = false, bool FT = false, bool PRE = false>
__global__ void __attribute__((amdgpu_flat_work_group_size(256, 256), amdgpu_waves_per_eu(ShadeWaves<KIND>::value))) k_shade(DPathState st, DScene sc, DTables T, DFrame fr, DSobol sob, int depth, int first_kind, DStats* stats) {
    __shared__ uint32_t emit_list[4 * 128];
    shade_body<KIND, SIMPLE, FT, PRE>(st, sc, T, fr, sob, depth, first_kind, stats, seg_open(st, ticket_ptr(st, depth, TK_SHADE0 + KIND), st.dynamic_segments != 0, depth, Q_MAT0 + KIND),
                                      emit_list + (threadIdx.x >> 6) * 128);
}

template <class W> HKD W wone();
template <> HKD float wone<float>() { return 1.0f; }
template <> HKD S4 wone<S4>() { return s4(1.0f); }
HKD S4 wide(S4 v) { return v; }
HKD S4 wide(float v) { return s4(v); }
HKD bool is_black(float v) { return v == 0.0f; }
template <bool COMPACT>
HKD void shadow_contribute(const DPathState& st, uint32_t rec, S4 T_ray, S4 tr_u, S4 tr_l) {
    if (is_black(T_ray)) return;
    S4 w_u, w_l;
    ld_shadow_weights<COMPACT>(st, rec, w_u, w_l);
    S4 mis = w_u * tr_u + w_l * tr_l;
    float den = average(mis);
    if (den > 1e-10f) {
        S4 fin = ld4(&st.sh_Ld[rec]) * T_ray / den;
        if (!is_black(fin)) {
            const uint32_t pslot = st.sh_slot[rec];
            st4(&st.L[pslot], ld4(&st.L[pslot]) + fin);
        }
    }
}

HKD void shadow_contribute_final(const DPathState& st, uint32_t rec, float den) {
    if (den > 1e-10f) {
        const S4 fin = ld4(&st.sh_Ld[rec]) * s4(1.0f) / den;
        if (!is_black(fin)) {
            const uint32_t pslot = st.sh_slot[rec];
            st4(&st.L[pslot], ld4(&st.L[pslot]) + fin);
        }
    }
}
HKD void shadow_contribute_rt(const DPathState& st, uint32_t rec, S4 T_ray, S4 tr_u, S4 tr_l) {
    if (st.compact)
        shadow_contribute<true>(st, rec, T_ray, tr_u, tr_l);
    else
        shadow_contribute<false>(st, rec, T_ray, tr_u, tr_l);
}

template <bool COUNT, int NC, bool QN = false>
__device__ __forceinline__ void shadow_body(const DPathState& st, const DScene& sc, int depth, DStats* stats, SegStream stream, int* __restrict__ stack, const NodeCache& cache) {
    const int lane = lane_id();
    const unsigned long long lt_mask = (1ull << lane) - 1ull;
    const int DONE = (int)0x80000000;
    unsigned n_nodes = 0, n_tris = 0, n_casts = 0, n_hits = 0;
    HK_DBG_DECL
    uint32_t seg = 0;
    int n = 0, cursor = 0;
    bool more = true;
    bool have = false;
    uint32_t slot = 0;
    float rec_den = 0.0f;
    LaneRay r;
    r.cur = r.pend = DONE;
    for (;;) {
        const unsigned long long run_m = __ballot(have && r.cur != DONE);
        if (run_m == 0ull || (64 - __popcll(run_m) >= HK_TRACE_MIN_IDLE && (cursor < n || more))) {
            if (have && r.cur == DONE) {
                if (r.best.prim < 0) {
                    if (st.sh_final)
                        shadow_contribute_final(st, slot, rec_den);
                    else
                        shadow_contribute<true>(st, slot, s4(1.0f), s4(1.0f), s4(1.0f));
                } else
                    ++n_hits;
                have = false;
            }
            while (more && cursor >= n) {
                const int gw = stream_next(stream, st.n_waves);
                if (gw >= st.n_waves) {
                    more = false;
                    break;
                }
                seg = (uint32_t)gw * (uint32_t)st.wave_cap;
                n = *count_ptr(st, depth, Q_SHADOW, gw);
                cursor = 0;
            }
            const unsigned long long want = __ballot(!have);
            const int avail = n - cursor;
            const int rank = __popcll(want & lt_mask);
            if (!have && rank < avail) {
                slot = seg + (uint32_t)(cursor + rank);
                float4 O = stream_ld(&st.sh_o[slot]), D = stream_ld(&st.sh_d[slot]);
                rec_den = D.w;
                if (O.w >= 1e-6f) {
                    ++n_casts;
                    lane_ray_start<QN>(r, sc, mk3(O.x, O.y, O.z), mk3(D.x, D.y, D.z), O.w);
                    have = true;
                }
            }
            const int want_n = __popcll(want);
            cursor += want_n < avail ? want_n : (avail > 0 ? avail : 0);
            if (__ballot(have) == 0ull) {
                if (cursor >= n && !more) break;
                continue;
            }
        }
#ifdef HK_DEBUG_UTIL
        HK_DBG(5, have && r.cur != DONE);
        lane_ray_round<true, COUNT, NC, HK_POSTPONE_ANYHIT != 0, false, QN>(r, have && r.cur != DONE, sc, stack, lane, n_nodes, n_tris, cache, cursor < n || more, dbg_ + 6);
#else
        lane_ray_round<true, COUNT, NC, HK_POSTPONE_ANYHIT != 0, false, QN>(r, have && r.cur != DONE, sc, stack, lane, n_nodes, n_tris, cache, cursor < n || more);
#endif
    }
    stats += global_wave();
    HK_DBG_FLUSH(stats);
    wave_add(&stats->rays_shadow, n_casts);
    wave_add(&stats->hits, n_hits);
    if (COUNT) {
        wave_add(&stats->sh_nodes, n_nodes);
        wave_add(&stats->sh_tris, n_tris);
    }
}
template <bool COUNT, int STACK, int BLOCK = HK_TRACE_BLOCK, int NC = 0, bool QN = false>
__global__ void __launch_bounds__(BLOCK) k_shadow(DPathState st, DScene sc, int depth, DStats* stats) {
    __shared__ int lds_stack[(BLOCK / 64) * STACK * 64];
    __shared__ float4 lds_box[NC > 0 ? 3 * NC : 1];
    __shared__ int2 lds_child[NC > 0 ? NC : 1];
    int* stack = lds_stack + (threadIdx.x >> 6) * (STACK * 64);
    const NodeCache cache = node_cache_fill<NC, BLOCK, QN>(sc, lds_box, lds_child);
    shadow_body<COUNT, NC, QN>(st, sc, depth, stats, stream_open(st, ticket_ptr(st, depth, TK_SHADOW), false, depth, Q_SHADOW), stack, cache);
}

template <int NC>
__device__ __forceinline__ void trace_shadow_body(const DPathState& st, const DScene& sc, int depth, DStats* stats, int gw, int* __restrict__ stack, const NodeCache& cache) {
    const int lane = lane_id();
    const unsigned long long lt_mask = (1ull << lane) - 1ull;
    const int DONE = (int)0x80000000;
    unsigned n_nodes = 0, n_tris = 0, n_casts = 0, n_hits = 0, n_sh_casts = 0;
    const int dt = depth + 1;
    const DPathGen g = gen_at(st, dt);
    const uint32_t seg = (uint32_t)gw * (uint32_t)st.wave_cap;
    const int n_ray = *count_ptr(st, dt, Q_RAY, gw), n_sh = *count_ptr(st, depth, Q_SHADOW, gw);
    WaveQ q_escaped = wq_open(st.escaped_q, st, gw);
    int kind_count[HK_MAX_KINDS];
#pragma unroll
    for (int k = 0; k < HK_MAX_KINDS; ++k) kind_count[k] = 0;
    int cur_ray = 0, cur_sh = 0;
    int state = LR_EMPTY;
    uint32_t slot = 0;
    float rec_den = 0.0f;
    LaneRay r;
    r.cur = r.pend = DONE;
    r.any = false;
    for (;;) {
        const unsigned long long run_m = __ballot(state == LR_ACTIVE && r.cur != DONE);
        if (run_m == 0ull || (64 - __popcll(run_m) >= HK_TRACE_MIN_IDLE && (cur_ray < n_ray || cur_sh < n_sh))) {
            int kind = -1;
            if (state == LR_ACTIVE && r.cur == DONE) {
                if (r.any) {
                    if (r.best.prim < 0) {
                        if (st.sh_final)
// ... 1630 lines not shown
```

hikari.jl_amd/csrc/hk_launch.h:

```cpp
#pragma once
#include "hikari_mi355x.h"
#include "hk_types.h"

namespace hk {

inline bool lean_scene(const DScene& sc) { return sc.all_opaque != 0 && sc.n_media == 0; }
inline int walk_split_mode() { return knob_int("HK_WALK_SPLIT", 0); }

bool grey_compact_ok(const DScene& sc);
bool preselect_lights(const DScene& sc, const DPathState& st);
bool small_pass_fusable(const DScene& sc, uint32_t kinds_mask);

void launch_camera(hipStream_t s, int n_cu, const DPathState& st, const DFrame& fr, const DTables& T, const DFilter& flt, const DCamera& cam, const DSobol& sob, int initial_medium);
void launch_trace(hipStream_t s, int n_cu, const DPathState& st, const DScene& sc, const DTables& T, const DFrame& fr, int depth, DStats* stats);
void launch_shadow(hipStream_t s, int n_cu, const DPathState& st, const DScene& sc, const DTables& T, const DFrame& fr, int depth, DStats* stats);
void launch_escaped(hipStream_t s, int n_cu, const DPathState& st, const DScene& sc, const DTables& T, const DFrame& fr, int depth);
void launch_medium(hipStream_t s, int n_cu, const DPathState& st, const DScene& sc, const DTables& T, const DFrame& fr, const DSobol& sob, int depth, DStats* stats);
void launch_detect_camera_medium(hipStream_t s, const DPathState& st, const DScene& sc, float x, float y, float z, DStats* stats);
void launch_light_select(hipStream_t s, int n_cu, const DPathState& st, const DScene& sc, const DTables& T, const DFrame& fr, const DSobol& sob, int depth, uint32_t kinds_mask, DStats* stats);
void launch_shade(hipStream_t s, int n_cu, int kind, const DPathState& st, const DScene& sc, const DTables& T, const DFrame& fr, const DSobol& sob, int depth, int first_kind, DStats* stats);
bool launch_small_pass(hipStream_t s, int n_cu, const DPathState& st, const DScene& sc, const DTables& T, const DFrame& fr, const DFilter& flt, const DCamera& cam, const DSobol& sob, int max_depth,
                       uint32_t kinds_mask, DStats* stats, bool dry, void* accum, int film_mode);
void launch_segment_lists(hipStream_t s, const DPathState& st, int n, const int* depths, const int* queues);
void launch_film(hipStream_t s, const DPathState& st, const DFrame& fr, const DTables& T, void* accum, bool f64);

void launch_sobol_table(hipStream_t s, const DSobol& sob, const DFrame& fr, uint2* table, int rows);
void launch_sobol_lo_table(hipStream_t s, const DSobol& sob, const DFrame& fr, uint16_t* table, int rows, int base, int stride, int count);
template <class Layout> void launch_finalize(hipStream_t s, const void* accum, bool f64, Layout out, int w, int h);
template <class Layout> void launch_aux(hipStream_t s, const DScene& sc, const DCamera& cam, int h, int w, float miss_depth, float* albedo, Layout out);
template <class Layout> void launch_variance(hipStream_t s, Layout src, float* variance, int h, int w);
template <class Layout> void launch_postprocess(hipStream_t s, const hk_postprocess_params& P, Layout src, float* out, int h, int w);
void launch_atrous(hipStream_t s, const hk_denoise_params& P, int step, PlanarPixels src, const float* variance, PlanarPixels dst, int h, int w);
void launch_atrous(hipStream_t s, const hk_denoise_params& P, int step, PackedPixels src, const float* variance, PackedPixels dst, float* out, const hk_postprocess_params* pp, int h, int w);
void launch_slot_of_prim(hipStream_t s, const float4* leaf, int n, int* slot_of_prim);
void launch_xform_tris(hipStream_t s, const DXform& X, int first, int n, const float* bp, const float* bn, const float* bt, const int* slot_of_prim, float* pos, float* nrm, float* tan, float* shade,
                       float4* leaf);
void launch_refit_level(hipStream_t s, int begin, int end, DNode* nodes, DQNode* qnodes, const DQGrid& grid, const float4* leaf, const float* pos);
void launch_envmap_tables(hipStream_t s, const DEnvMap& e, DEnvMap* record);
void launch_majorant_grid(hipStream_t s, const DMedium& m);
void launch_majorant_nanovdb(hipStream_t s, const DMedium& m, const DIndexBox& index_bbox);
void launch_nvdb_bricks(hipStream_t s, const DMedium& m, size_t n_blocks);

void launch_test_trace(hipStream_t s, const DScene& sc, int n, const float* o, const float* d, const float* tmax, float* t, int* prim, float* uv);
void launch_test_trace_lean(hipStream_t s, int n_cu, const DScene& sc, int anyhit, int n, const float* o, const float* d, const float* tmax, float* t, int* prim, float* uv);
void launch_test_sobol(hipStream_t s, const DTables& T, const DSobol& sob, int n, const int* px, const int* py, const int* si, const int* dim, float* o1, float* o2);
void launch_test_camera(hipStream_t s, const DTables& T, const DFilter& flt, const DCamera& cam, const DSobol& sob, int height, int n, const int* px, const int* py, const int* si, float* out);
void launch_test_uplift(hipStream_t s, const DTables& T, int mode, int n, const float* rgb, const float* lam, float* out);
void launch_test_light_bvh(hipStream_t s, const DScene& sc, int n, const float* p, const float* nn, const float* u, int* out_light, float* out_pmf, const int* query, float* out_qpmf);
void launch_test_light(hipStream_t s, const DScene& sc, const DTables& T, int mode, int light_idx, int n, const float* p3, const float* in3, const float* lambda, float* out);
void launch_test_bsdf(hipStream_t s, const DScene& sc, const DTables& T, int mode, int mat_idx, int regularize, int n, const float* wo, const float* wi, const float* ns, const float* lambda,
                      const float* u, const float* uc, float* out);
void launch_test_mix(hipStream_t s, const DScene& sc, int mat_idx, int n, const float* p3, const float* wo3, const float* uv2, int* out);
void launch_test_medium(hipStream_t s, const DScene& sc, const DTables& T, int mode, int medium_idx, int n, const float* a3, const float* b3, const float* tmax, const float* lambda, float* out);
int test_majorant_stride();

}
```

hikari.jl_amd/csrc/hk_launch_impl.h:

```cpp
#pragma once
#include "hk_launch.h"

namespace hk {

template <bool V>
using bool_c = std::bool_constant<V>;
template <int V>
using int_c = std::integral_constant<int, V>;
template <class F>
static void with_bool(bool b, F&& f) {
    if (b) f(bool_c<true>{});
    else f(bool_c<false>{});
}
template <int V0, int... Vs, class F>
static void with_int(int v, F&& f) {
    if constexpr (sizeof...(Vs) == 0) f(int_c<V0>{});
    else if (v == V0) f(int_c<V0>{});
    else with_int<Vs...>(v, f);
}

#ifndef HK_OCC_SCALE_DEFAULT
#define HK_OCC_SCALE_DEFAULT 1.0f
#endif
static inline int grid_for(int n, int block, int cap) {
    long g = ((long)n + block - 1) / block;
    if (g < 1) g = 1;
    if (g > cap) g = cap;
    return (int)g;
}

template <class K>
static int resident_blocks(K kernel, int block) {
    int per_cu = 0;
    if (hipOccupancyMaxActiveBlocksPerMultiprocessor(&per_cu, kernel, block, 0) != hipSuccess || per_cu < 1) per_cu = 1;
    return per_cu;
}
static float occ_scale() {
    const char* e = hk::knob("HK_OCC_SCALE");
    const float v = e ? (float)std::atof(e) : HK_OCC_SCALE_DEFAULT;
    return v >= 0.25f && v <= 8.0f ? v : 1.0f;
}
#define HK_MAX_DEVICES 64
template <auto Kernel>
static int cached_blocks(int block, int n_cu, int cap_per_cu) {
    static int cache[HK_MAX_DEVICES];
    int dev = 0, per_cu;
    if (hipGetDevice(&dev) != hipSuccess || dev < 0 || dev >= HK_MAX_DEVICES)
        per_cu = resident_blocks(Kernel, block);
    else {
        if (cache[dev] == 0) {
            cache[dev] = resident_blocks(Kernel, block);
            if (hk::knob("HK_DEBUG_ALLOC")) std::fprintf(stderr, "HK_DEBUG_ALLOC occupancy API: %d blocks of %d per CU for %s\n", cache[dev], block, __PRETTY_FUNCTION__);
        }
        per_cu = cache[dev];
    }
    per_cu = (int)((float)per_cu * occ_scale() + 0.5f);
    if (per_cu < 1) per_cu = 1;
    if (per_cu > cap_per_cu) per_cu = cap_per_cu;
    return per_cu * n_cu;
}
static int clamp_blocks(int blocks, const DPathState& st, int waves_per_block = 4) {
    const int units = st.n_waves / waves_per_block;
    if (blocks >= units) return units;
    if (st.dynamic_segments) return blocks;
    int best = 1;
    for (int b = blocks; b >= 1; --b)
        if (units % b == 0) {
            best = b;
            break;
        }
    return best * 4 >= blocks * 3 ? best : blocks;
}
template <auto K, class... A>
static void launch_resident(hipStream_t s, int n_cu, const DPathState& st, int block, int cap_per_cu, A&&... args) {
    const int blocks = cached_blocks<K>(block, n_cu, cap_per_cu);
    hipLaunchKernelGGL(K, dim3(clamp_blocks(blocks, st, block / 64)), dim3(block), 0, s, st, args...);
}

static bool node_cache_on() { return knob_on("HK_NODE_CACHE"); }
static int grey_mode() { return knob_int("HK_GREY", 1); }
static int grey_flat_mode() { return knob_int("HK_GREY_FLAT", 1); }
static int walk_pool_mode() { return knob_int("HK_WALK_POOL", 1); }
static int track_pool_mode() { return knob_int("HK_TRACK_POOL", 1); }
static bool sobol_tables_cover(const DSobol& sob, int depth) {
    return sob.hi_table != nullptr && sob.lo_table != nullptr && 9 + 5 * depth < sob.lo_rows && 9 + 5 * depth < sob.hi_rows && knob_on("HK_SOBOL_TABLE_ONLY");
}
static int media_mask_class(const DScene& sc) {
    int m = sc.media_mask;
    return (m == 1 || m == 2 || m == 4 || m == 8) ? m : 15;
}

void launch_camera(hipStream_t s, int n_cu, const DPathState& st, const DFrame& fr, const DTables& T, const DFilter& flt, const DCamera& cam, const DSobol& sob, int initial_medium) {
    launch_resident<k_camera>(s, n_cu, st, 256, 8, fr, T, flt, cam, sob, initial_medium);
}

#ifndef HK_SHADOW_NC16
#define HK_SHADOW_NC16 560
#endif
#ifndef HK_SHADOW_BLOCK16
#define HK_SHADOW_BLOCK16 768
#endif
#ifndef HK_SHADOW_NC32
#define HK_SHADOW_NC32 0
#endif
#ifndef HK_TRACE_NC32
#define HK_TRACE_NC32 128
#endif
template <int B16, int NC16, int NC32, class F>
static void lean_dispatch(const DScene& sc, const DFrame& fr, F&& launch) {
    with_bool(fr.count_nodes != 0, [&](auto COUNT) {
        with_bool(node_cache_on(), [&](auto CACHE) {
            constexpr bool cache = decltype(CACHE)::value;
            if (sc.bvh_depth <= 16) launch(COUNT, int_c<16>{}, int_c<cache ? B16 : HK_TRACE_BLOCK>{}, int_c<cache ? NC16 : 0>{}, bool_c<false>{});
            else with_bool(sc.qnodes != nullptr, [&](auto QN) { launch(COUNT, int_c<HK_LDS_STACK>{}, int_c<HK_TRACE_BLOCK>{}, int_c<cache ? NC32 : 0>{}, QN); });
        });
    });
}
void launch_trace(hipStream_t s, int n_cu, const DPathState& st, const DScene& sc, const DTables& T, const DFrame& fr, int depth, DStats* stats) {
    if (lean_scene(sc)) {
        lean_dispatch<1024, 1536, HK_TRACE_NC32>(sc, fr, [&](auto COUNT, auto STACK, auto BLOCK, auto NC, auto QN) {
            constexpr int block = decltype(BLOCK)::value;
            launch_resident<k_trace_lean<decltype(COUNT)::value, decltype(STACK)::value, block, decltype(NC)::value, decltype(QN)::value>>(s, n_cu, st, block, 8, sc, depth, stats);
        });
        return;
    }
    with_bool(fr.count_nodes != 0, [&](auto COUNT) { launch_resident<k_trace<decltype(COUNT)::value>>(s, n_cu, st, HK_TRACE_BLOCK, 8, sc, T, fr, depth, stats); });
}
template <bool C, int MM>
static void launch_walk_split(hipStream_t s, int n_cu, const DPathState& st, const DScene& sc, const DFrame& fr, int depth, DStats* stats) {
    const int cb = clamp_blocks(cached_blocks<k_walk_cast<C, MM, 16>>(HK_TRACE_BLOCK, n_cu, 8), st);
    const int tb = clamp_blocks(cached_blocks<k_walk_track<MM>>(256, n_cu, 8), st);
    for (int round = 0; round < HK_WALK_ROUNDS; ++round) {
        hipLaunchKernelGGL((k_walk_cast<C, MM, 16>), dim3(cb), dim3(HK_TRACE_BLOCK), 0, s, st, sc, depth, round, stats, sc.media);
        hipLaunchKernelGGL((k_walk_track<MM>), dim3(tb), dim3(256), 0, s, st, sc, depth, round, fr.walk_tune, stats, sc.media);
    }
}
bool grey_compact_ok(const DScene& sc) {
    if (!knob_on("HK_GREY_COMPACT")) return false;
    const int mc = sc.n_media > 0 ? media_mask_class(sc) : 0;
    return sc.n_media == 1 && sc.all_grey && sc.grey_pool && (mc == 2 || mc == 8) && sc.bvh_depth <= 16 && grey_mode() && grey_flat_mode() && track_pool_mode() && walk_pool_mode() &&
           !walk_split_mode();
}
template <bool C, int MM>
static void launch_shadow_walk(hipStream_t s, int n_cu, const DPathState& st, const DScene& sc, const DTables& T, const DFrame& fr, int depth, DStats* stats) {
    constexpr bool grey_kind = MM == 2 || MM == 8;
    constexpr int M2 = grey_kind ? MM : 8;
    const bool shallow = sc.bvh_depth <= 16;
    const int pool = walk_pool_mode();
    if (shallow && grey_kind && sc.grey_pool && grey_mode() && grey_flat_mode() && pool) {
        if (M2 == 8 && sc.grey_bricks && sc.bvh_depth <= 8 && pool == 1)
            launch_resident<k_walk_pool<C, 8, true, 8, 64>>(s, n_cu, st, HK_TRACE_BLOCK, 8, sc, depth, fr.walk_tune, fr.track_gate, stats, sc.media);
        else if (M2 == 8 && sc.grey_bricks)
            launch_resident<k_walk_pool<C, 8, true, 16, 56>>(s, n_cu, st, HK_TRACE_BLOCK, 8, sc, depth, fr.walk_tune, fr.track_gate, stats, sc.media);
        else
            launch_resident<k_walk_pool<C, M2, false, 16, 56>>(s, n_cu, st, HK_TRACE_BLOCK, 8, sc, depth, fr.walk_tune, fr.track_gate, stats, sc.media);
    } else if (shallow && grey_kind && sc.all_grey && grey_mode())
        launch_resident<k_shadow_walk<C, M2, 16, true>>(s, n_cu, st, HK_TRACE_BLOCK, 8, sc, T, depth, fr.walk_tune, stats, sc.media);
    else if (shallow)
        launch_resident<k_shadow_walk<C, MM, 16>>(s, n_cu, st, HK_TRACE_BLOCK, 8, sc, T, depth, fr.walk_tune, stats, sc.media);
    else
        launch_resident<k_shadow_walk<C, MM>>(s, n_cu, st, HK_TRACE_BLOCK, 8, sc, T, depth, fr.walk_tune, stats, sc.media);
}
void launch_shadow(hipStream_t s, int n_cu, const DPathState& st, const DScene& sc, const DTables& T, const DFrame& fr, int depth, DStats* stats) {
    if (lean_scene(sc)) {
        lean_dispatch<HK_SHADOW_BLOCK16, HK_SHADOW_NC16, HK_SHADOW_NC32>(sc, fr, [&](auto COUNT, auto STACK, auto BLOCK, auto NC, auto QN) {
            constexpr int block = decltype(BLOCK)::value;
            launch_resident<k_shadow<decltype(COUNT)::value, decltype(STACK)::value, block, decltype(NC)::value, decltype(QN)::value>>(s, n_cu, st, block, 8, sc, depth, stats);
        });
        return;
    }
    const int mc = sc.n_media > 0 ? media_mask_class(sc) : 0;
    const bool split = sc.all_grey && grey_mode() && walk_split_mode() && sc.bvh_depth <= 16 && st.wq_a != nullptr;
    with_bool(fr.count_nodes != 0, [&](auto COUNT) {
        constexpr bool c = decltype(COUNT)::value;
        if (split && mc == 8) launch_walk_split<c, 8>(s, n_cu, st, sc, fr, depth, stats);
        else if (split && mc == 2) launch_walk_split<c, 2>(s, n_cu, st, sc, fr, depth, stats);
        else with_int<0, 1, 2, 4, 8, 15>(mc, [&](auto MM) { launch_shadow_walk<c, decltype(MM)::value>(s, n_cu, st, sc, T, fr, depth, stats); });
    });
}
void launch_segment_lists(hipStream_t s, const DPathState& st, int n, const int* depths, const int* queues) {
    if (n <= 0) return;
    SegQueues qs;
    qs.n = n;
    for (int i = 0; i < n; ++i) {
        qs.depth[i] = depths[i];
        qs.q[i] = queues[i];
    }
    hipLaunchKernelGGL(k_segment_lists, dim3(n, HK_LIST_SPLIT), dim3(1024), 0, s, st, qs);
}
void launch_medium(hipStream_t s, int n_cu, const DPathState& st, const DScene& sc, const DTables& T, const DFrame& fr, const DSobol& sob, int depth, DStats* stats) {
    {
        const int d = depth, q = Q_MEDIUM;
        launch_segment_lists(s, st, 1, &d, &q);
    }
    const bool grey = sc.all_grey && grey_mode();
    const bool flat = grey && grey_flat_mode();
    const bool pool = flat && track_pool_mode() && sc.grey_pool;
    auto track = [&](auto MM, auto GREY) { launch_resident<k_track<decltype(MM)::value, decltype(GREY)::value>>(s, n_cu, st, 256, 8, sc, T, fr, depth, stats, sc.media); };
    auto track_flat = [&](auto MM, auto BRICKS) {
        constexpr int mm = decltype(MM)::value;
        constexpr bool bricks = decltype(BRICKS)::value;
        if (pool) launch_resident<k_track_pool<mm, bricks>>(s, n_cu, st, 256, 8, sc, fr, depth, stats, sc.media);
        else launch_resident<k_track_flat<mm, bricks>>(s, n_cu, st, 256, 8, sc, fr, depth, stats, sc.media);
    };
    switch (media_mask_class(sc)) {
        case 1: track(int_c<1>{}, bool_c<false>{}); break;
        case 2:
            if (flat) track_flat(int_c<2>{}, bool_c<false>{});
            else with_bool(grey, [&](auto GREY) { track(int_c<2>{}, GREY); });
            break;
        case 4: track(int_c<4>{}, bool_c<false>{}); break;
        case 8:
            if (flat) with_bool(sc.grey_bricks != 0, [&](auto BRICKS) { track_flat(int_c<8>{}, BRICKS); });
            else with_bool(grey, [&](auto GREY) { track(int_c<8>{}, GREY); });
            break;
        default: track(int_c<15>{}, bool_c<false>{}); break;
    }
    {
        const int d = depth, q = Q_SCATTER;
        launch_segment_lists(s, st, 1, &d, &q);
    }
    with_bool(sobol_tables_cover(sob, depth), [&](auto FT) { launch_resident<k_scatter<decltype(FT)::value>>(s, n_cu, st, 256, 8, sc, T, fr, sob, depth, stats); });
}
void launch_detect_camera_medium(hipStream_t s, const DPathState& st, const DScene& sc, float x, float y, float z, DStats* stats) {
    hipLaunchKernelGGL(k_detect_camera_medium, dim3(1), dim3(64), 0, s, st, sc, x, y, z, stats);
}
void launch_escaped(hipStream_t s, int n_cu, const DPathState& st, const DScene& sc, const DTables& T, const DFrame& fr, int depth) {
    with_bool(knob_int("HK_ESCAPED_UNROLL", 1) != 2, [&](auto ONE) { launch_resident<k_escaped<decltype(ONE)::value ? 1 : 2>>(s, n_cu, st, 256, 8, sc, T, depth, fr.implicit_ones); });
}
bool preselect_lights(const DScene& sc, const DPathState& st) {
    return sc.n_media == 0 && sc.num_bvh_lights >= HK_PRESELECT_MIN && st.sel_light != nullptr && knob_on("HK_PRESELECT");
}
void launch_light_select(hipStream_t s, int n_cu, const DPathState& st, const DScene& sc, const DTables& T, const DFrame& fr, const DSobol& sob, int depth, uint32_t kinds_mask, DStats* stats) {
    const int min_idle = knob_int_in("HK_SELECT_MIN_IDLE", 1, 64, HK_SELECT_MIN_IDLE);
    const bool pool = knob_on("HK_SELECT_POOL");
    with_bool(sobol_tables_cover(sob, depth), [&](auto FT) {
        constexpr bool ft = decltype(FT)::value;
        if (pool) launch_resident<k_light_select_pool<ft>>(s, n_cu, st, HK_SELECT_BLOCK, 8, sc, T, fr, sob, depth, kinds_mask, stats);
        else launch_resident<k_light_select<ft>>(s, n_cu, st, 256, 8, sc, T, fr, sob, depth, kinds_mask, min_idle, stats);
    });
}
void launch_shade(hipStream_t s, int n_cu, int kind, const DPathState& st, const DScene& sc, const DTables& T, const DFrame& fr, const DSobol& sob, int depth, int first_kind, DStats* stats) {
    auto shade = [&](auto KIND, auto SIMPLE, auto FT, auto PRE) {
        launch_resident<k_shade<decltype(KIND)::value, decltype(SIMPLE)::value, decltype(FT)::value, decltype(PRE)::value>>(s, n_cu, st, 256, 8, sc, T, fr, sob, depth, first_kind, stats);
    };
    const bool ft = sobol_tables_cover(sob, depth);
    const bool light_kind = kind == HK_MAT_MATTE || kind == HK_MAT_MIRROR || kind == HK_MAT_GLASS || kind == HK_MAT_CONDUCTOR;
    if (light_kind && preselect_lights(sc, st))
        with_int<HK_MAT_MATTE, HK_MAT_MIRROR, HK_MAT_GLASS, HK_MAT_CONDUCTOR>(kind, [&](auto KIND) { with_bool(ft, [&](auto FT) { shade(KIND, bool_c<false>{}, FT, bool_c<true>{}); }); });
    else if (kind == HK_MAT_MATTE && sc.simple_lights)
        with_bool(ft, [&](auto FT) { shade(int_c<HK_MAT_MATTE>{}, bool_c<true>{}, FT, bool_c<false>{}); });
    else if (light_kind && ft)
        with_int<HK_MAT_MATTE, HK_MAT_MIRROR, HK_MAT_GLASS, HK_MAT_CONDUCTOR>(kind, [&](auto KIND) { shade(KIND, bool_c<false>{}, bool_c<true>{}, bool_c<false>{}); });
    else
        with_int<HK_MAT_MATTE, HK_MAT_MIRROR, HK_MAT_GLASS, HK_MAT_CONDUCTOR, HK_MAT_COATED_DIFFUSE, HK_MAT_THIN_DIELECTRIC, HK_MAT_DIFFUSE_TRANSMISSION, HK_MAT_COATED_DIFFUSE_TRANSMISSION,
                 HK_MAT_COATED_CONDUCTOR, HK_MAT_FALLBACK>(kind, [&](auto KIND) { shade(KIND, bool_c<false>{}, bool_c<false>{}, bool_c<false>{}); });
}
#ifndef HK_SMALL_PASS_NC
#define HK_SMALL_PASS_NC 1536
#endif
static int small_pass_class(const DScene& sc, uint32_t kinds_mask) {
    const int mode = knob_int("HK_SMALL_PASS_FUSED", 2);
    if (mode == 0) return 0;
    if (!(lean_scene(sc) && sc.bvh_depth <= HK_LDS_STACK && node_cache_on())) return 0;
    if (kinds_mask == (1u << HK_MAT_MATTE) && sc.simple_lights && !sc.has_escape_lights && sc.bvh_depth <= 16 && sc.num_bvh_lights < HK_PRESELECT_MIN) return 1;
    const uint32_t light_kinds = (1u << HK_MAT_MATTE) | (1u << HK_MAT_MIRROR) | (1u << HK_MAT_GLASS) | (1u << HK_MAT_CONDUCTOR);
    return (mode >= 2 && kinds_mask != 0 && (kinds_mask & ~light_kinds) == 0) ? 2 : 0;
}
bool small_pass_fusable(const DScene& sc, uint32_t kinds_mask) { return small_pass_class(sc, kinds_mask) != 0; }
template <int BLOCK, bool GENERAL, int STACK, class... A>
static bool small_pass_blocks(hipStream_t s, int n_cu, const DPathState& st, bool dry, A&&... args) {
    constexpr auto kernel = k_small_pass<HK_SMALL_PASS_NC, BLOCK, GENERAL, STACK>;
    int blocks = cached_blocks<kernel>(BLOCK, n_cu, 1);
    if (blocks * (BLOCK / 64) > st.n_waves) blocks = st.n_waves / (BLOCK / 64);
    if (blocks < 1) return false;
    if (!dry) hipLaunchKernelGGL(kernel, dim3(blocks), dim3(BLOCK), 0, s, st, args...);
    return true;
}
bool launch_small_pass(hipStream_t s, int n_cu, const DPathState& st, const DScene& sc, const DTables& T, const DFrame& fr, const DFilter& flt, const DCamera& cam, const DSobol& sob, int max_depth,
                       uint32_t kinds_mask, DStats* stats, bool dry, void* accum, int film_mode) {
    const int cls = small_pass_class(sc, kinds_mask);
    if (cls == 0 || !st.small_pass || st.dynamic_segments || fr.count_nodes) return false;
    if (((long)st.capacity + 63) / 64 / 16 > 4L * n_cu) return false;
    for (int depth = 0; depth < max_depth; ++depth)
        if (sobol_tables_cover(sob, depth)) return false;
    const int merged = knob_on("HK_SMALL_PASS_MERGED") ? 1 : 0;
    if (st.n_waves > 8 * n_cu) return false;
    bool launched = false;
    auto pass = [&](auto GENERAL, auto STACK) {
        with_bool(st.n_waves > 4 * n_cu, [&](auto WIDE) {
            launched = small_pass_blocks<decltype(WIDE)::value ? 512 : 256, decltype(GENERAL)::value, decltype(STACK)::value>(s, n_cu, st, dry, sc, T, fr, flt, cam, sob, max_depth, sc.n_lights > 0 ? 1 : 0, merged,
                                                                                                                       accum, film_mode, kinds_mask, stats);
        });
    };
    if (cls == 2 && sc.bvh_depth > 16) pass(bool_c<true>{}, int_c<HK_LDS_STACK>{});
    else if (cls == 2) pass(bool_c<true>{}, int_c<16>{});
    else pass(bool_c<false>{}, int_c<16>{});
    return launched;
}
void launch_film(hipStream_t s, const DPathState& st, const DFrame& fr, const DTables& T, void* accum, bool f64) {
    int g = grid_for(fr.n_pixels_padded >> 6, 4, 4096);
    if (f64)
        hipLaunchKernelGGL(k_film<double>, dim3(g), dim3(256), 0, s, st, fr, T, (double*)accum);
    else
        hipLaunchKernelGGL(k_film<float>, dim3(g), dim3(256), 0, s, st, fr, T, (float*)accum);
}
void launch_sobol_table(hipStream_t s, const DSobol& sob, const DFrame& fr, uint2* table, int rows) {
    hipLaunchKernelGGL(k_sobol_table, dim3(grid_for((long)rows * fr.n_pixels_padded > 0x3fffffff ? 0x3fffffff : rows * fr.n_pixels_padded, 256, 8192)), dim3(256), 0, s, sob, fr, table, rows);
}
void launch_sobol_lo_table(hipStream_t s, const DSobol& sob, const DFrame& fr, uint16_t* table, int rows, int base, int stride, int count) {
    hipLaunchKernelGGL(k_sobol_lo_table, dim3(65536), dim3(256), 0, s, sob, fr, table, rows, base, stride, count);
}
template <class Layout>
void launch_finalize(hipStream_t s, const void* accum, bool f64, Layout out, int w, int h) {
    int g = grid_for(w * h, 256, 4096);
    if (f64)
        hipLaunchKernelGGL((k_finalize<double, Layout>), dim3(g), dim3(256), 0, s, (const double*)accum, out, w, h);
    else
        hipLaunchKernelGGL((k_finalize<float, Layout>), dim3(g), dim3(256), 0, s, (const float*)accum, out, w, h);
}
template <class Layout>
void launch_aux(hipStream_t s, const DScene& sc, const DCamera& cam, int h, int w, float miss_depth, float* albedo, Layout out) {
    hipLaunchKernelGGL(k_aux<Layout>, dim3(grid_for(h * w, HK_TRACE_BLOCK, 2048)), dim3(HK_TRACE_BLOCK), 0, s, sc, cam, h, w, miss_depth, albedo, out);
}
template <class Layout>
void launch_variance(hipStream_t s, Layout src, float* variance, int h, int w) {
    hipLaunchKernelGGL(k_variance<Layout>, dim3(grid_for(h * w, 256, 8192)), dim3(256), 0, s, src, variance, h, w);
}
template <class Layout>
void launch_postprocess(hipStream_t s, const hk_postprocess_params& P, Layout src, float* out, int h, int w) {
    hipLaunchKernelGGL(k_postprocess<Layout>, dim3(grid_for(h * w, 256, 8192)), dim3(256), 0, s, P, src, out, h, w);
}
template void launch_finalize<PlanarPixels>(hipStream_t, const void*, bool, PlanarPixels, int, int);
template void launch_aux<PlanarPixels>(hipStream_t, const DScene&, const DCamera&, int, int, float, float*, PlanarPixels);
template void launch_variance<PlanarPixels>(hipStream_t, PlanarPixels, float*, int, int);
template void launch_postprocess<PlanarPixels>(hipStream_t, const hk_postprocess_params&, PlanarPixels, float*, int, int);
template void launch_finalize<PackedPixels>(hipStream_t, const void*, bool, PackedPixels, int, int);
template void launch_aux<PackedPixels>(hipStream_t, const DScene&, const DCamera&, int, int, float, float*, PackedPixels);
template void launch_variance<PackedPixels>(hipStream_t, PackedPixels, float*, int, int);
template void launch_postprocess<PackedPixels>(hipStream_t, const hk_postprocess_params&, PackedPixels, float*, int, int);
template <class Layout, bool FINAL>
static void atrous(hipStream_t s, const hk_denoise_params& P, int step, Layout src, const float* variance, Layout dst, float* out, const hk_postprocess_params* pp, int h, int w) {
    const hk_postprocess_params PP = pp ? *pp : hk_postprocess_params{};
    hipLaunchKernelGGL((k_atrous<Layout, FINAL>), dim3(grid_for(h * w, 256, 8192)), dim3(256), 0, s, P, PP, pp ? 1 : 0, step, src, variance, dst, out, h, w);
}
void launch_atrous(hipStream_t s, const hk_denoise_params& P, int step, PlanarPixels src, const float* variance, PlanarPixels dst, int h, int w) {
    atrous<PlanarPixels, false>(s, P, step, src, variance, dst, nullptr, nullptr, h, w);
}
void launch_atrous(hipStream_t s, const hk_denoise_params& P, int step, PackedPixels src, const float* variance, PackedPixels dst, float* out, const hk_postprocess_params* pp, int h, int w) {
    with_bool(out != nullptr, [&](auto FINAL) { atrous<PackedPixels, decltype(FINAL)::value>(s, P, step, src, variance, dst, out, pp, h, w); });
}
void launch_slot_of_prim(hipStream_t s, const float4* leaf, int n, int* slot_of_prim) {
    hipLaunchKernelGGL(k_slot_of_prim, dim3(grid_for(n, 256, 8192)), dim3(256), 0, s, leaf, n, slot_of_prim);
}
void launch_xform_tris(hipStream_t s, const DXform& X, int first, int n, const float* bp, const float* bn, const float* bt, const int* slot_of_prim, float* pos, float* nrm,
                       float* tan, float* shade, float4* leaf) {
    hipLaunchKernelGGL(k_xform_tris, dim3(grid_for(n, 256, 8192)), dim3(256), 0, s, X, first, n, bp, bn, bt, slot_of_prim, pos, nrm, tan, shade, leaf);
}
void launch_refit_level(hipStream_t s, int begin, int end, DNode* nodes, DQNode* qnodes, const DQGrid& grid, const float4* leaf, const float* pos) {
    hipLaunchKernelGGL(k_refit_level, dim3(grid_for(end - begin, 256, 8192)), dim3(256), 0, s, begin, end, nodes, qnodes, grid, leaf, pos);
}
void launch_envmap_tables(hipStream_t s, const DEnvMap& e, DEnvMap* record) {
    hipLaunchKernelGGL(k_envmap_rows, dim3((e.nv + 63) / 64), dim3(64), 0, s, e.data, e.nu, e.nv, const_cast<float*>(e.cond_func), const_cast<float*>(e.cond_cdf),
                       const_cast<float*>(e.cond_func_int), const_cast<float*>(e.marg_func));
    hipLaunchKernelGGL(k_envmap_marginal, dim3(1), dim3(64), 0, s, e.nv, e.marg_func, const_cast<float*>(e.marg_cdf), record);
}

static int majorant_block_per_cell(double box_voxels) { return box_voxels > (double)knob_int("HK_MAJORANT_BLOCK_VOXELS", 8192) ? 1 : 0; }
static void majorant_zero_mask(hipStream_t s, const DMedium& m, int ncell) {
    hipLaunchKernelGGL(k_majorant_zero_mask, dim3((unsigned)(((long long)ncell + 255) / 256)), dim3(256), 0, s, m.majorant, ncell, const_cast<uint32_t*>(m.maj_zero));
}
void launch_majorant_grid(hipStream_t s, const DMedium& m) {
    const int ncell = m.mres[0] * m.mres[1] * m.mres[2];
    const int per_block = majorant_block_per_cell((double)m.res[0] * m.res[1] * m.res[2] / ncell);
    const dim3 grid((unsigned)(per_block ? ncell : ((long long)ncell + 3) / 4));
    with_bool(m.kind == HK_MEDIUM_RGB_GRID, [&](auto RGB) {
        hipLaunchKernelGGL((k_majorant_grid<decltype(RGB)::value>), grid, dim3(256), 0, s, m, ncell, per_block, const_cast<float*>(m.majorant));
    });
    majorant_zero_mask(s, m, ncell);
}
void launch_majorant_nanovdb(hipStream_t s, const DMedium& m, const DIndexBox& ib) {
    const int ncell = m.mres[0] * m.mres[1] * m.mres[2];
    double box = 1.0;
    for (int k = 0; k < 3; ++k) box *= ((double)ib.hi[k] - ib.lo[k] + 1.0) / m.mres[k] + 3.0;
    const int per_block = majorant_block_per_cell(box);
    hipLaunchKernelGGL(k_majorant_nanovdb, dim3((unsigned)(per_block ? ncell : ((long long)ncell + 3) / 4)), dim3(256), 0, s, m, ib, ncell, per_block, const_cast<float*>(m.majorant));
    majorant_zero_mask(s, m, ncell);
}
void launch_nvdb_bricks(hipStream_t s, const DMedium& m, size_t n_blocks) {
    const unsigned long long n_out = (unsigned long long)n_blocks * 729u;
    hipLaunchKernelGGL(k_nvdb_bricks, dim3((unsigned)std::min<unsigned long long>((n_out + 255) / 256, 1u << 20)), dim3(256), 0, s, m, n_out, const_cast<float*>(m.nv_bricks));
}

}
```

hikari.jl_amd/csrc/hk_render.cpp:

```cpp
#include "hk_host.h"

namespace {
float gaussian_1d(float x, float sigma) { return std::exp(-(x * x) / (2.0f * (sigma * sigma))); }
float mitchell_1d(float x, float B, float C) {
    x = std::fabs(x);
    if (x <= 1.0f) return ((12.0f - 9.0f * B - 6.0f * C) * (x * x * x) + (-18.0f + 12.0f * B + 6.0f * C) * (x * x) + (6.0f - 2.0f * B)) / 6.0f;
    if (x <= 2.0f) return ((-B - 6.0f * C) * (x * x * x) + (6.0f * B + 30.0f * C) * (x * x) + (-12.0f * B - 48.0f * C) * x + (8.0f * B + 24.0f * C)) / 6.0f;
    return 0.0f;
}
float sinc1(float x) {
    x = std::fabs(x);
    if (x < 1e-5f) return 1.0f;
    x *= 3.14159265358979323846f;
    return std::sin(x) / x;
}
float wsinc(float x, float r, float tau) {
    x = std::fabs(x);
    if (x > r) return 0.0f;
    return sinc1(x) * sinc1(x / tau);
}
float filter_eval(const hk_integrator_params& p, float ex, float ey, float x, float y) {
    float rx = p.filter_radius[0], ry = p.filter_radius[1];
    switch (p.filter_type) {
        case HK_FILTER_BOX: return (std::fabs(x) <= rx && std::fabs(y) <= ry) ? 1.0f : 0.0f;
// ... 332 lines not shown
    {
        const long by_memory = (8L << 30) / (440L * (long)S * fr.n_pixels_padded);
        if (n_lanes > by_memory) n_lanes = by_memory < 1 ? 1 : (int)by_memory;
    }
    const bool small_call = n_samples <= S && (long)S * fr.n_pixels_padded <= max_paths;
    int after = 4;
    after = hk::knob_int_in("HK_PIPELINE_AFTER", 0, INT_MAX, after);
    c->small_streak = small_call ? c->small_streak + 1 : 0;
    const bool lanes_started = c->ev_main != nullptr;
    if (n_lanes > 1 && !c->time_kernels && small_call && (lanes_started || c->small_streak > after)) {
        if ((int)I->lane_sets.size() < (int)hk_ctx::MAX_LANES) I->lane_sets.resize(hk_ctx::MAX_LANES);
        lane_idx = c->next_lane % n_lanes;
        c->next_lane = (lane_idx + 1) % n_lanes;
        hk_ctx::Lane& L = c->lanes[lane_idx];
        if (!L.stream) HIP_TRY(hipStreamCreateWithFlags(&L.stream, hipStreamNonBlocking));
        if (!L.done) {
            HIP_TRY(hipEventCreateWithFlags(&L.done, hipEventDisableTiming));
            std::vector<DStats> zero((size_t)c->stat_rows);
            std::memset(zero.data(), 0, zero.size() * sizeof(DStats));
            HIP_TRY(L.stats.upload(zero.data(), zero.size() * sizeof(DStats)));
        }
        if (!c->ev_main) {
            HIP_TRY(hipEventCreateWithFlags(&c->ev_main, hipEventDisableTiming));
            HIP_TRY(hipEventCreateWithFlags(&c->ev_film, hipEventDisableTiming));
        }
    } else {
        if (int e = join_lanes(c)) return e;
    }
    return HK_OK;
}
int ensure_sobol_tables(hk_ctx* c, hk_integrator* I, const DFrame& fr, DSobol& sob, int first_sample_idx, int n_samples, int sample_stride) {
    const int x0 = fr.x0, y0 = fr.y0;
    const int rows = 4 + 5 * (I->p.max_depth + 1);
    const bool table_same = !(I->sobol_rows != rows || I->sobol_stride != fr.n_pixels_padded || I->sobol_log2 != sob.log2_spp || I->sobol_digits != sob.n_base4_digits ||
                              I->sobol_x0 != x0 || I->sobol_y0 != y0 || I->sobol_tiles_x != fr.tiles_x);
    if (!table_same) {
        if (c->lanes_dirty) {
            if (int e = join_lanes(c)) return e;
            HIP_TRY(hipStreamSynchronize(c->stream));
        }
        HIP_TRY(I->sobol_table.alloc((size_t)rows * fr.n_pixels_padded * sizeof(uint2)));
        hk::launch_sobol_table(c->stream, sob, fr, I->sobol_table.as<uint2>(), rows);
        HIP_TRY(hipGetLastError());
        I->sobol_rows = rows;
        I->sobol_stride = fr.n_pixels_padded;
        I->sobol_log2 = sob.log2_spp;
        I->sobol_digits = sob.n_base4_digits;
        I->sobol_x0 = x0, I->sobol_y0 = y0, I->sobol_tiles_x = fr.tiles_x;
    }
    sob.hi_table = I->sobol_table.as<uint2>();
    sob.hi_rows = rows;
    sob.hi_stride = fr.n_pixels_padded;
    const long last_idx = (long)first_sample_idx + (long)(n_samples - 1) * sample_stride;
    if (n_samples >= 16 && sob.log2_spp >= 2 && sob.log2_spp <= 16 && (last_idx >> sob.log2_spp) == 0) {
        const int base = sample_stride == 1 ? (first_sample_idx & ~15) : first_sample_idx;
        const int count = (int)((((last_idx - base) / sample_stride + 1) + 15) & ~15L);
        bool same = table_same && I->lo_base == base && I->lo_sample_stride == sample_stride && I->lo_count == count && I->lo_rows > 0;
        if (!same) {
            if (c->lanes_dirty) {
                if (int e = join_lanes(c)) return e;
                HIP_TRY(hipStreamSynchronize(c->stream));
            }
            double gb = 32.0;
            if (const char* e = hk::knob("HK_SOBOL_LO_GB")) gb = std::atof(e);
            size_t budget = (size_t)(gb * 1e9), free_b = 0, total_b = 0;
            if (hipMemGetInfo(&free_b, &total_b) == hipSuccess && (free_b + I->sobol_lo.bytes) / 4 < budget) budget = (free_b + I->sobol_lo.bytes) / 4;
            const size_t per_row = (size_t)fr.n_pixels_padded * count * sizeof(uint16_t);
            int lo_rows = (int)(budget / per_row < (size_t)rows ? budget / per_row : (size_t)rows);
            I->lo_rows = 0;
            if (lo_rows > 0 && (size_t)fr.n_pixels_padded * count < 0xffffffffull) {
                bool have_buf = true;
                if (I->sobol_lo.bytes < per_row * lo_rows || I->sobol_lo.bytes > 2 * per_row * lo_rows) {
                    while (lo_rows > 0 && I->sobol_lo.alloc(per_row * lo_rows) != hipSuccess) {
                        (void)hipGetLastError();
                        lo_rows /= 2;
                    }
                    have_buf = lo_rows > 0;
                }
                if (have_buf) {
                    hk::launch_sobol_lo_table(c->stream, sob, fr, I->sobol_lo.as<uint16_t>(), lo_rows, base, sample_stride, count);
                    HIP_TRY(hipGetLastError());
                    I->lo_rows = lo_rows;
                    I->lo_base = base;
                    I->lo_sample_stride = sample_stride;
                    I->lo_count = count;
                }
            }
        }
        if (I->lo_rows > 0) {
            sob.lo_table = I->sobol_lo.as<uint16_t>();
            sob.lo_rows = I->lo_rows;
            sob.lo_count = I->lo_count;
        }
    }
    return HK_OK;
}
int detect_camera_medium(hipStream_t s, hk_integrator* I, const hk_scene* sc, const hk_camera* cam, DStats* dstats) {
    if (sc->d.n_media > 0) {
        const float* m = cam->camera_to_world;
        float w = m[15];
        float cx = m[3], cy = m[7], cz = m[11];
        if (w != 1.0f) {
            float inv = 1.0f / w;
            cx *= inv;
            cy *= inv;
            cz *= inv;
        }
        hk::launch_detect_camera_medium(s, I->st, sc->d, cx, cy, cz, dstats);
    } else
        HIP_TRY(hipMemsetAsync(I->st.initial_medium, 0xff, sizeof(int), s));
    return HK_OK;
}
struct ShadowStream {
    hk_ctx* c;
    bool overlap;
    bool in_flight = false;
    ~ShadowStream() {
        if (in_flight && c->aux) (void)hipStreamSynchronize(c->aux);
    }
};
struct PassCtx {
    hk_ctx* c;
    hk_scene* sc;
    hk_integrator* I;
    hk_film* film;
    DFrame fr;
    DSobol sob;
    DCamera dc;
    DStats* dstats;
    hipStream_t s;
    bool piped;
    int first_sample_idx, sample_stride;
    int view_mode = 0;
    std::string view_key_of() const;

    template <class F>
    int timed(int cls, F&& fn) {
        hipEvent_t e0 = nullptr, e1 = nullptr;
        if (c->time_kernels) {
            e0 = get_event(c);
            e1 = get_event(c);
            if (hipEventRecord(e0, s) != hipSuccess) return fail(HK_ERR_DEVICE, "event record failed");
        }
        fn();
        if (c->time_kernels) {
            if (hipEventRecord(e1, s) != hipSuccess) return fail(HK_ERR_DEVICE, "event record failed");
            (cls == 0 ? c->trace_events : c->class_events[cls]).emplace_back(e0, e1);
        }
        return HK_OK;
    }
    int lists(std::initializer_list<std::pair<int, int>> dq, bool kinds_of_depth = false, int kd = 0) {
        int dd[HK_MAX_KINDS + 6], qq[HK_MAX_KINDS + 6], n = 0;
        for (auto& e : dq) dd[n] = e.first, qq[n] = e.second, ++n;
        if (kinds_of_depth)
            for (int kind = 0; kind < HK_MAX_KINDS; ++kind)
                if (sc->kinds_mask & (1u << kind)) dd[n] = kd, qq[n] = Q_MAT0 + kind, ++n;
        if (I->st.small_pass) return HK_OK;
        return timed(3, [&] { hk::launch_segment_lists(s, I->st, n, dd, qq); });
    }
    int enqueue_depth(ShadowStream& sh, int depth);
    int enqueue_stages(bool view_hit);
    int enqueue_pass(int k, int done);
};
std::string PassCtx::view_key_of() const {
    std::string k;
    auto put = [&k](const void* p, size_t n) { k.append(static_cast<const char*>(p), n); };
    put(&dc, sizeof dc);
    put(&I->filter, sizeof I->filter);
    const int v[] = {fr.width, fr.height, fr.x0, fr.y0, fr.x1, fr.y1, fr.first_sample, fr.sample_stride, fr.samples_in_pass, sob.log2_spp, sob.n_base4_digits, (int)sob.seed, sob.width,
                     fr.implicit_ones, I->st.compact, I->st.meta32, I->st.const_origin, I->st.n_waves, I->st.wave_cap, I->st.dynamic_segments, view_mode, (int)c->tables_epoch};
    put(v, sizeof v);
    return k;
}
int PassCtx::enqueue_depth(ShadowStream& sh, int depth) {
    if (int e = timed(0, [&] { hk::launch_trace(s, c->n_cu, I->st, sc->d, c->tables, fr, depth, dstats); })) return e;
    c->trace_launches++;
    if (sh.in_flight) {
        HIP_TRY(hipStreamWaitEvent(s, c->ev_join, 0));
        sh.in_flight = false;
    }
    int first_kind = 1;
    if (sc->d.n_media > 0) {
        if (int e = timed(4, [&] { hk::launch_medium(s, c->n_cu, I->st, sc->d, c->tables, fr, sob, depth, dstats); })) return e;
        c->media_launches += 2;
        first_kind = 0;
    }
    if (sc->d.has_escape_lights) {
        if (int e = lists({{depth, Q_ESCAPED}}, true, depth)) return e;
        if (int e = timed(3, [&] { hk::launch_escaped(s, c->n_cu, I->st, sc->d, c->tables, fr, depth); })) return e;
    } else if (int e = lists({}, true, depth))
        return e;
    if (sc->d.n_lights > 0 && hk::preselect_lights(sc->d, I->st)) {
        if (int e = timed(5, [&] { hk::launch_light_select(s, c->n_cu, I->st, sc->d, c->tables, fr, sob, depth, sc->kinds_mask, dstats); })) return e;
        c->select_launches++;
    }
    for (int kind = 0; kind < HK_MAX_KINDS; ++kind)
        if (sc->kinds_mask & (1u << kind)) {
            if (int e = timed(2, [&] { hk::launch_shade(s, c->n_cu, kind, I->st, sc->d, c->tables, fr, sob, depth, first_kind, dstats); })) return e;
            first_kind = 0;
            c->shade_launches++;
        }
    if (int e = lists({{depth, Q_SHADOW}, {depth + 1, Q_RAY}})) return e;
    if (sc->d.n_lights > 0) {
        if (sh.overlap) {
            HIP_TRY(hipEventRecord(c->ev_fork, s));
            HIP_TRY(hipStreamWaitEvent(c->aux, c->ev_fork, 0));
            hk::launch_shadow(c->aux, c->n_cu, I->st, sc->d, c->tables, fr, depth, dstats + c->stat_rows / 2);
            HIP_TRY(hipEventRecord(c->ev_join, c->aux));
            sh.in_flight = true;
        } else
            if (int e = timed(1, [&] { hk::launch_shadow(s, c->n_cu, I->st, sc->d, c->tables, fr, depth, dstats); })) return e;
        c->shadow_launches++;
    }
    return HK_OK;
}
int PassCtx::enqueue_stages(bool view_hit) {
    HIP_TRY(hipMemsetAsync(I->st.tickets, 0, (size_t)I->st.ticket_rows * HK_TICKET_COLS * HK_TICKET_WAYS * HK_TICKET_STRIDE * sizeof(int), s));
    const size_t kept = view_hit ? (size_t)I->st.n_waves : 0;
    HIP_TRY(hipMemsetAsync(I->st.counters + kept, 0, ((size_t)(I->st_depth + 2) * Q_COUNT * I->st.n_waves - kept) * sizeof(int), s));
    if (I->st.wq_ctl) HIP_TRY(hipMemsetAsync(I->st.wq_ctl, 0, (size_t)(I->st_depth + 2) * 11 * 4 * sizeof(int), s));
    if (!view_hit) {
        if (int e = timed(3, [&] { hk::launch_camera(s, c->n_cu, I->st, fr, c->tables, I->filter, dc, sob, -1); })) return e;
    } else if (view_mode == 2)
        HIP_TRY(hipMemsetAsync(I->st.L, 0, (size_t)fr.n_pixels_padded * fr.samples_in_pass * sizeof(float4), s));
    if (int e = lists({{0, Q_RAY}})) return e;
    if (const char* e = hk::knob("HK_OVERLAP")) c->overlap = std::atoi(e) ? 1 : 0;
    else c->overlap = -1;
    const bool want_overlap = c->overlap < 0 ? sc->d.bvh_depth > 16 : c->overlap != 0;
    const bool overlap = want_overlap && !c->time_kernels && sc->d.n_lights > 0 && sc->d.n_media == 0 && !piped && (!I->mid_pass || c->overlap == 1);
    if (overlap && !c->aux) {
        HIP_TRY(hipStreamCreateWithFlags(&c->aux, hipStreamNonBlocking));
        HIP_TRY(hipEventCreateWithFlags(&c->ev_fork, hipEventDisableTiming));
        HIP_TRY(hipEventCreateWithFlags(&c->ev_join, hipEventDisableTiming));
    }
    ShadowStream sh{c, overlap};
    for (int depth = 0; depth < I->p.max_depth; ++depth)
        if (int e = enqueue_depth(sh, depth)) return e;
    if (sh.in_flight) {
        HIP_TRY(hipStreamWaitEvent(s, c->ev_join, 0));
        sh.in_flight = false;
    }
    return HK_OK;
}
int PassCtx::enqueue_pass(int k, int done) {
    fr.samples_in_pass = k;
    {
        int L = 0;
        while ((1 << L) < k) ++L;
        fr.s_shr = 30 + L;
        fr.s_mul = (uint32_t)((((uint64_t)1 << fr.s_shr) + (uint64_t)k - 1) / (uint64_t)k);
    }
    fr.first_sample = first_sample_idx + done * sample_stride;
    if (sob.lo_table) sob.lo_offset = (fr.first_sample - I->lo_base) / sample_stride;
    const bool fused = !c->time_kernels && !piped && hk::launch_small_pass(s, c->n_cu, I->st, sc->d, c->tables, fr, I->filter, dc, sob, I->p.max_depth, sc->kinds_mask, dstats, true, nullptr, 0);
    const int vm = fused ? 0 : view_mode;
    I->st.view_cache = vm;
    I->st.gen_cam = vm ? I->cam_gen : I->st.gen[0];
    const std::string view_key = vm ? view_key_of() : std::string();
    const bool view_hit = vm && I->view_key == view_key;
    I->view_key.clear();
    bool film_inline = false;
    if (fused) {
        film_inline = fr.samples_in_pass == 1;
        (void)hk::launch_small_pass(s, c->n_cu, I->st, sc->d, c->tables, fr, I->filter, dc, sob, I->p.max_depth, sc->kinds_mask, dstats, false, film->accum, film_inline ? (film->f64 ? 2 : 1) : 0);
        c->fused_passes++;
    } else if (int e = enqueue_stages(view_hit))
        return e;
    if (piped && c->film_chain) HIP_TRY(hipStreamWaitEvent(s, c->ev_film, 0));
    if (!film_inline)
        if (int e = timed(3, [&] { hk::launch_film(s, I->st, fr, c->tables, film->accum, film->f64); })) return e;
    if (vm) I->view_key = view_key;
    if (view_hit) c->view_cache_hits++;
    if (piped) {
        HIP_TRY(hipEventRecord(c->ev_film, s));
        c->film_chain = true;
    }
    return HK_OK;
}
}

extern "C" int32_t hk_render(hk_ctx* c, hk_scene* sc, hk_integrator* I, hk_film* film, const hk_camera* cam, int32_t first_sample_idx, int32_t n_samples,
                             int32_t sample_stride) {
    if (!film) return fail(HK_ERR_INVALID, "null argument");
    return hk_render_tile(c, sc, I, film, cam, first_sample_idx, n_samples, sample_stride, 0, 0, film->width, film->height);
}

static int render_tile_now(hk_ctx* c, hk_scene* sc, hk_integrator* I, hk_film* film, const hk_camera* cam, int32_t first_sample_idx, int32_t n_samples,
                           int32_t sample_stride, int32_t x0, int32_t y0, int32_t x1, int32_t y1);
int flush_pending(hk_ctx* c) {
    if (!c || !c->pending.active) return HK_OK;
    hk_ctx::Pending p = c->pending;
    c->pending.active = false;
    return render_tile_now(c, p.sc, p.I, p.film, &p.cam, p.first, p.n, p.stride, p.x0, p.y0, p.x1, p.y1);
}
extern "C" int32_t hk_render_tile(hk_ctx* c, hk_scene* sc, hk_integrator* I, hk_film* film, const hk_camera* cam, int32_t first_sample_idx, int32_t n_samples,
                                  int32_t sample_stride, int32_t x0, int32_t y0, int32_t x1, int32_t y1) {
    if (!c || !sc || !I || !film || !cam) return fail(HK_ERR_INVALID, "null argument");
    if (x0 < 0 || y0 < 0 || x1 > film->width || y1 > film->height || x0 > x1 || y0 > y1) return fail(HK_ERR_INVALID, "pixel range outside the film");
    if (x0 == x1 || y0 == y1) return HK_OK;
    if (n_samples < 0 || sample_stride < 1 || first_sample_idx < 1) return fail(HK_ERR_INVALID, "bad sample range");
    if (!c->have_tables) return fail(HK_ERR_INVALID, "hk_ctx_set_tables must be called first");
    if (sc->ctx != c || I->ctx != c || film->ctx != c) return fail(HK_ERR_INVALID, "scene / integrator / film belong to another context");
    if (film->f64 != (I->p.accumulate_f64 != 0)) return fail(HK_ERR_INVALID, "film / integrator accumulation type mismatch");
    if (n_samples == 0) return HK_OK;
    KnobScope knobs(&c->knobs);
    {
        long batch_paths = 64L << 20, small_paths = 8L << 20;
        if (const char* e = hk::knob("HK_BATCH_PATHS_M")) batch_paths = std::atol(e) >= 0 ? std::atol(e) << 20 : batch_paths;
        if (const char* e = hk::knob("HK_PIPELINE_MAX_PATHS_M")) small_paths = std::atol(e) > 0 ? std::atol(e) << 20 : small_paths;
        const long px = (long)((x1 - x0 + 7) / 8) * ((y1 - y0 + 7) / 8) * 64;
        hk_ctx::Pending& p = c->pending;
        const bool visible_order = (c->own_stream_order && !film->external && !film->exposed) || hk::knob_int("HK_DEFER_EXTERNAL", 0);
        const bool small = batch_paths > 0 && visible_order && !c->time_kernels && (long)n_samples * px <= small_paths && I->p.samples_per_pass <= 0;
        if (p.active && small && p.sc == sc && p.I == I && p.film == film && std::memcmp(&p.cam, cam, sizeof(hk_camera)) == 0 && p.stride == sample_stride && p.x0 == x0 &&
            p.y0 == y0 && p.x1 == x1 && p.y1 == y1 && (long)p.first + (long)p.n * p.stride == first_sample_idx && (long)(p.n + n_samples) * px <= batch_paths) {
            p.n += n_samples;
            p.calls += 1;
            return HK_OK;
        }
        if (int e = flush_pending(c)) return e;
        if (small) {
            p.active = true;
            p.sc = sc, p.I = I, p.film = film, p.cam = *cam;
            p.first = first_sample_idx, p.n = n_samples, p.stride = sample_stride, p.x0 = x0, p.y0 = y0, p.x1 = x1, p.y1 = y1, p.calls = 1;
            return HK_OK;
        }
    }
    return render_tile_now(c, sc, I, film, cam, first_sample_idx, n_samples, sample_stride, x0, y0, x1, y1);
}
static int render_tile_now(hk_ctx* c, hk_scene* sc, hk_integrator* I, hk_film* film, const hk_camera* cam, int32_t first_sample_idx, int32_t n_samples,
                           int32_t sample_stride, int32_t x0, int32_t y0, int32_t x1, int32_t y1) {
    HIP_TRY(hipSetDevice(c->device));
    KnobScope knobs(&c->knobs);
    const int W = film->width, H = film->height;
    DFrame fr{};
    fr.width = W;
    fr.height = H;
    fr.x0 = x0, fr.y0 = y0, fr.x1 = x1, fr.y1 = y1;
    fr.tiles_x = (x1 - x0 + 7) / 8;
    fr.tiles_y = (y1 - y0 + 7) / 8;
    fr.n_pixels_padded = fr.tiles_x * fr.tiles_y * 64;
    int S = 0, lane_idx = -1;
    if (int e = choose_samples_per_pass(c, I, fr, n_samples, S)) return e;
    if (int e = pick_lane(c, I, fr, S, n_samples, lane_idx)) return e;
    const bool piped = lane_idx >= 0;
    struct SetGuard {
        hk_integrator* I;
        hk_integrator::StateSet* ls;
        ~SetGuard() {
            if (ls) I->swap_set(*ls);
        }
    } set_guard{I, piped ? &I->lane_sets[lane_idx] : nullptr};
    if (piped) I->swap_set(I->lane_sets[lane_idx]);
    if (int e = ensure_state(I, S * fr.n_pixels_padded, pass_traits(sc, c, n_samples, piped), piped ? c->lanes[lane_idx].stream : nullptr)) return e;
    I->st.const_origin = (I->st.meta32 && !(cam->lens_radius > 0)) ? 1 : 0;
    fr.sample_stride = sample_stride;
    fr.max_depth = I->p.max_depth;
    fr.regularize = I->p.regularize;
    fr.max_component_value = I->p.max_component_value;
    fr.count_nodes = c->count_nodes;
    fr.implicit_ones = sc->d.n_media == 0 ? 1 : 0;
    {
        auto knob = [](const char* name, int dflt) { return hk::knob_int_in(name, 1, 255, dflt); };
        fr.track_gate = hk::knob_int_in("HK_TRACK_MIN_PENDING", 0, 64, 0) | (hk::knob_int_in("HK_TRACK_EXTRA_ADVANCE", 0, 255, 4) << 8);
        fr.delta_advance = knob("HK_DELTA_ADVANCE", 3);
        fr.refill_idle = knob("HK_TRACK_REFILL_IDLE", 24);
        fr.walk_tune = knob("HK_SHADOW_TRACK_BATCH", 8) | (knob("HK_TRACK_ADVANCE", 2) << 8) | (knob("HK_SHADOW_FEED_ROUNDS", 3) << 16) | ((knob("HK_WALK_REFILL_IDLE", 16) > 63 ? 63 : knob("HK_WALK_REFILL_IDLE", 16)) << 24);
    }
    DSobol sob = make_sobol(I->p, W, H);
    if (int e = ensure_sobol_tables(c, I, fr, sob, first_sample_idx, n_samples, sample_stride)) return e;
    DCamera dc = make_camera(*cam);
    DStats* dstats = c->stats.as<DStats>();
    hipStream_t s = c->stream;
    if (piped) {
        HIP_TRY(hipEventRecord(c->ev_main, c->stream));
        s = c->lanes[lane_idx].stream;
        HIP_TRY(hipStreamWaitEvent(s, c->ev_main, 0));
        dstats = c->lanes[lane_idx].stats.as<DStats>();
    }
    if (!c->have_span) {
        HIP_TRY(hipEventRecord(c->ev_begin, s));
        c->have_span = true;
    }
    if (int e = detect_camera_medium(s, I, sc, cam, dstats)) return e;
    PassCtx pass{c, sc, I, film, fr, sob, dc, dstats, s, piped, first_sample_idx, sample_stride};
    if (!piped && n_samples == S && I->cam_gen.ray_d != nullptr && I->st.meta32 && fr.implicit_ones) {
        const int mode = hk::knob_int("HK_VIEW_CACHE", 1);
        pass.view_mode = mode == 2 ? 2 : (mode != 0 ? 1 : 0);
    }
    for (int done = 0; done < n_samples;) {
        const int k = n_samples - done < S ? n_samples - done : S;
        if (int e = pass.enqueue_pass(k, done)) return e;
        done += k;
    }
    HIP_TRY(hipGetLastError());
    if (piped) {
        HIP_TRY(hipEventRecord(c->lanes[lane_idx].done, s));
        c->lanes_dirty = true;
    } else
        HIP_TRY(hipEventRecord(c->ev_end, s));
    return HK_OK;
}
```

hikari.jl_amd/csrc/hk_scene.cpp:

```cpp
#include "hk_host.h"

namespace {
inline float clampf(float v, float lo, float hi) { return v < lo ? lo : (v > hi ? hi : v); }
inline float max3(float a, float b, float c) {
    float m = a > b ? a : b;
    return m > c ? m : c;
}
void bake_bounded(const hk::RGB2Spec& t, float r, float g, float b, float out[4]) {
    hk::rgb_to_coeffs(t, r, g, b, out);
    out[3] = 1.0f;
}
void bake_unbounded(const hk::RGB2Spec& t, float r, float g, float b, float out[4]) {
    float m = max3(r, g, b);
    if (m <= 0.0f) {
        out[0] = out[1] = out[2] = out[3] = 0.0f;
        return;
    }
    hk::rgb_to_coeffs(t, r / m, g / m, b / m, out);
    out[3] = m / hk::poly_max(out);
}
void bake_illuminant(const hk::RGB2Spec& t, float r, float g, float b, float out[4]) {
    float m = max3(r, g, b);
    if (m <= 0.0f) {
        out[0] = out[1] = out[2] = out[3] = 0.0f;
// ... 129 lines not shown
    SurfaceClasses out;
    out.mi_opaque.assign(d->n_media_interfaces > 0 ? d->n_media_interfaces : 1, 1);
    for (int i = 0; i < d->n_media_interfaces; ++i) {
        const hk_medium_interface& mi = d->media_interfaces[i];
        const bool op = mi.inside == mi.outside && !material_alpha_tested(d->materials[mi.material]);
        out.mi_opaque[i] = op;
        if (!op) out.all_opaque = false;
    }
    return out;
}

struct BvhUpload {
    int root_ref = 0;
    bool have_qnodes = false;
    float q_base[3] = {0, 0, 0}, q_cell[3] = {1, 1, 1};
};
std::vector<DNode> pack_nodes(const hk::BVH& bvh) {
    std::vector<DNode> dn(bvh.nodes.size() ? bvh.nodes.size() : 1);
    for (size_t i = 0; i < bvh.nodes.size(); ++i) {
        const hk::BVHNode& n = bvh.nodes[i];
        float lo[2][3], hi[2][3];
        node_boxes(n, lo, hi);
        hk_pack_node_boxes(dn[i], lo, hi);
        dn[i].c0 = n.c0;
        dn[i].c1 = n.c1;
        dn[i].pad0 = dn[i].pad1 = 0;
    }
    return dn;
}
std::vector<float4> pack_leaf_tris(const hk::BVH& bvh, const hk_scene_desc* d, const std::vector<uint8_t>& mi_opaque) {
    std::vector<float4> lt(3 * (bvh.leaf_prims.size() ? bvh.leaf_prims.size() : 1));
    for (size_t i = 0; i < bvh.leaf_prims.size(); ++i) {
        int prim = bvh.leaf_prims[i];
        const float* p = d->positions + 9 * (size_t)prim;
        uint32_t flags = 0;
        uint32_t mi = d->meta[prim].medium_interface_idx;
        if (mi_opaque[mi]) flags |= HK_TRI_OPAQUE;
        float pw, fw;
        std::memcpy(&pw, &prim, 4);
        std::memcpy(&fw, &flags, 4);
        hk_pack_leaf_tri(&lt[3 * i], p, pw, fw, 0.0f);
    }
    return lt;
}
bool quantise_nodes(const hk::BVH& bvh, float q_base[3], float q_cell[3], std::vector<DQNode>& qn) {
    for (int k = 0; k < 3; ++k) {
        const double ext = (double)bvh.hi[k] - (double)bvh.lo[k];
        q_cell[k] = (float)std::max(ext / 65527.0, 1e-30);
        q_base[k] = (float)((double)bvh.lo[k] - 3.0 * (double)q_cell[k]);
    }
    qn.resize(bvh.nodes.size());
    bool ok = true;
    for (size_t i = 0; i < bvh.nodes.size(); ++i) {
        const hk::BVHNode& n = bvh.nodes[i];
        float lo[2][3], hi[2][3];
        node_boxes(n, lo, hi);
        hk_quant_node(qn[i], lo, hi, q_base, q_cell);
        for (int c = 0; c < 2; ++c)
            for (int k = 0; k < 3; ++k) {
                const uint32_t ql = qn[i].w[3 * c + k] & 0xffffu, qh = qn[i].w[3 * c + k] >> 16;
                if (std::isfinite(lo[c][k]) && std::isfinite(hi[c][k]) &&
                    ((double)q_base[k] + ql * (double)q_cell[k] > lo[c][k] || (double)q_base[k] + qh * (double)q_cell[k] < hi[c][k]))
                    ok = false;
            }
        qn[i].c0 = n.c0;
        qn[i].c1 = n.c1;
    }
    return ok;
}
int upload_bvh(hk_scene* s, const hk_scene_desc* d, const std::vector<uint8_t>& mi_opaque, const hk::BVH& bvh, BvhUpload& out) {
    s->bvh_nodes = (int)bvh.nodes.size();
    s->bvh_leaf_tris = (int)bvh.leaf_prims.size();
    s->bvh_depth = bvh.max_depth;
    out.root_ref = bvh.root_ref;
    const std::vector<DNode> dn = pack_nodes(bvh);
    const std::vector<float4> lt = pack_leaf_tris(bvh, d, mi_opaque);
    HIP_TRY(s->nodes.upload(dn.data(), dn.size() * sizeof(DNode)));
    if (bvh.max_depth > 16 && !bvh.nodes.empty() && hk::knob_on("HK_QNODES")) {
        std::vector<DQNode> qn;
        if (quantise_nodes(bvh, out.q_base, out.q_cell, qn)) {
            HIP_TRY(s->qnodes.upload(qn.data(), qn.size() * sizeof(DQNode)));
            out.have_qnodes = true;
        }
    }
    HIP_TRY(s->leaf_tris.upload(lt.data(), lt.size() * sizeof(float4)));
    return HK_OK;
}

int upload_attributes(hk_scene* s, const hk_scene_desc* d) {
    const int T = d->n_triangles;
    HIP_TRY(s->positions.upload(d->positions, (size_t)T * 9 * 4));
    if (d->normals) HIP_TRY(s->normals.upload(d->normals, (size_t)T * 9 * 4));
    if (d->uvs) HIP_TRY(s->uvs.upload(d->uvs, (size_t)T * 6 * 4));
    if (d->tangents) HIP_TRY(s->tangents.upload(d->tangents, (size_t)T * 9 * 4));
    static_assert(sizeof(DTriMeta) == sizeof(hk_tri_meta), "meta layout");
    HIP_TRY(s->meta.upload(d->meta, (size_t)T * sizeof(hk_tri_meta)));
    bool tri_pack = T >= 32768;
    if (const char* e = hk::knob("HK_TRI_PACK")) tri_pack = T > 0 && std::atoi(e) != 0;
    if (tri_pack) {
        std::vector<float> rec((size_t)T * 32, 0.0f);
        const float nan = std::numeric_limits<float>::quiet_NaN();
        static const float default_uv[6] = {0.0f, 0.0f, 1.0f, 0.0f, 1.0f, 1.0f};
        for (int t = 0; t < T; ++t) {
            float* r = rec.data() + (size_t)t * 32;
            std::memcpy(r, d->positions + 9 * (size_t)t, 36);
            if (d->normals) std::memcpy(r + 9, d->normals + 9 * (size_t)t, 36);
            else for (int k = 0; k < 9; ++k) r[9 + k] = nan;
            std::memcpy(r + 18, d->uvs ? d->uvs + 6 * (size_t)t : default_uv, 24);
            std::memcpy(r + 24, &d->meta[t], 12);
        }
        HIP_TRY(s->tri_shade.upload(rec.data(), rec.size() * sizeof(float)));
    }
    return HK_OK;
}

int upload_textures(hk_scene* s, const hk_scene_desc* d) {
    std::vector<DTexture> dt(d->n_textures > 0 ? d->n_textures : 1);
    for (int i = 0; i < d->n_textures; ++i) {
        const hk_texture& t = d->textures[i];
        DevBuf* b = &s->own();
        HIP_TRY(b->upload(t.data, (size_t)t.width * t.height * t.channels * 4));
        dt[i].data = b->as<float>();
        dt[i].width = t.width;
        dt[i].height = t.height;
        dt[i].channels = t.channels;
        dt[i].pad = t.kind;
    }
    HIP_TRY(s->textures.upload(dt.data(), dt.size() * sizeof(DTexture)));
    return HK_OK;
}
int upload_spectra(hk_scene* s, const hk_scene_desc* d) {
    std::vector<DPLSpectrum> dsp(d->n_spectra > 0 ? d->n_spectra : 1);
    for (int i = 0; i < d->n_spectra; ++i) {
        const hk_pl_spectrum& sp = d->spectra[i];
        DevBuf* b = &s->own();
        std::vector<float> both(2 * (size_t)sp.n);
        std::memcpy(both.data(), sp.lambdas, sp.n * 4);
        std::memcpy(both.data() + sp.n, sp.values, sp.n * 4);
        HIP_TRY(b->upload(both.data(), both.size() * 4));
        dsp[i].lambdas = b->as<float>();
        dsp[i].values = b->as<float>() + sp.n;
        dsp[i].n = sp.n;
        dsp[i].pad = 0;
    }
    HIP_TRY(s->spectra.upload(dsp.data(), dsp.size() * sizeof(DPLSpectrum)));
    return HK_OK;
}
int upload_materials(hk_scene* s, const hk_scene_desc* d, const hk::RGB2Spec& r2s) {
    std::vector<DMaterial> dm(d->n_materials > 0 ? d->n_materials : 1);
    std::memset(dm.data(), 0, dm.size() * sizeof(DMaterial));
    for (int i = 0; i < d->n_materials; ++i) {
        bake_material(r2s, d->materials[i], dm[i]);
        if (dm[i].kind != HK_MAT_MIX) s->kinds_mask |= 1u << dm[i].kind;
    }
    s->n_materials = d->n_materials;
    HIP_TRY(s->materials.upload(dm.data(), dm.size() * sizeof(DMaterial)));
    return HK_OK;
}
int upload_medium_interfaces(hk_scene* s, const hk_scene_desc* d) {
    static_assert(sizeof(DMediumInterface) == 16, "mi layout");
    std::vector<DMediumInterface> dmi(d->n_media_interfaces > 0 ? d->n_media_interfaces : 1);
    for (int i = 0; i < d->n_media_interfaces; ++i) dmi[i] = DMediumInterface{d->media_interfaces[i].material, d->media_interfaces[i].inside, d->media_interfaces[i].outside, 0};
    HIP_TRY(s->mis.upload(dmi.data(), dmi.size() * sizeof(DMediumInterface)));
    return HK_OK;
}

}
void bake_light(const hk::RGB2Spec& r2s, const hk_light& l, DLight& o) {
    o.kind = l.kind;
    o.flags = (l.two_sided ? 1 : 0) | (l.spectrum_kind == HK_SPEC_ILLUMINANT ? 2 : 0);
    o.scale = l.scale;
    o.area = l.area;
    o.Le_tex = -1;
    float cf[4] = {0, 0, 0, 0};
    if (l.kind == HK_LIGHT_DIFFUSE_AREA) {
        o.Le_tex = l.Le.tex;
        std::memcpy(o.Le_rgba, l.Le.c, 16);
        if (l.Le.tex < 0) bake_bounded(r2s, l.Le.c[0] * l.scale, l.Le.c[1] * l.scale, l.Le.c[2] * l.scale, cf);
        std::memcpy(o.v, l.v, sizeof o.v);
        std::memcpy(o.normal, l.normal, sizeof o.normal);
        std::memcpy(o.uv, l.uv, sizeof o.uv);
    } else {
        if (l.spectrum_kind == HK_SPEC_ILLUMINANT) {
            cf[0] = l.poly[0];
            cf[1] = l.poly[1];
            cf[2] = l.poly[2];
            cf[3] = l.illum_scale;
        } else
            bake_illuminant(r2s, l.i_rgb[0], l.i_rgb[1], l.i_rgb[2], cf);
        if (l.kind == HK_LIGHT_POINT || l.kind == HK_LIGHT_SPOT) std::memcpy(o.p, l.position, 12);
        if (l.kind == HK_LIGHT_DIRECTIONAL || l.kind == HK_LIGHT_SUN) std::memcpy(o.p, l.direction, 12);
        if (l.kind == HK_LIGHT_SPOT) {
            const float* m = l.world_to_light;
            float rows[9] = {m[0], m[1], m[2], m[4], m[5], m[6], m[8], m[9], m[10]};
            std::memcpy(o.v, rows, sizeof rows);
            o.cos_total_width = l.cos_total_width;
            o.cos_falloff_start = l.cos_falloff_start;
        }
        if (l.kind == HK_LIGHT_ENVIRONMENT) {
            std::memcpy(o.Le_rgba, l.i_rgb, 16);
            o.Le_tex = l.envmap;
        }
    }
    o.coef = make_float4(cf[0], cf[1], cf[2], cf[3]);
}
namespace {
int upload_lights(hk_scene* s, const hk_scene_desc* d, const hk::RGB2Spec& r2s, int& has_escape) {
    std::vector<DLight> dl(d->n_lights > 0 ? d->n_lights : 1);
    std::memset(dl.data(), 0, dl.size() * sizeof(DLight));
    has_escape = 0;
    for (int i = 0; i < d->n_lights; ++i) {
        bake_light(r2s, d->lights[i], dl[i]);
        if (d->lights[i].kind == HK_LIGHT_AMBIENT || d->lights[i].kind == HK_LIGHT_ENVIRONMENT) has_escape = 1;
    }
    HIP_TRY(s->lights.upload(dl.data(), dl.size() * sizeof(DLight)));
    static_assert(sizeof(DLightNode) == 64 && sizeof(hk::LightNodeRec) == sizeof(DLightNode), "light node layout");
    static_assert(offsetof(hk::LightNodeRec, half_diag) == offsetof(DLightNode, half_diag) && offsetof(hk::LightNodeRec, w) == offsetof(DLightNode, w) &&
                      offsetof(hk::LightNodeRec, sin_o) == offsetof(DLightNode, sin_o) && offsetof(hk::LightNodeRec, child1_or_light) == offsetof(DLightNode, child1_or_light),
                  "light node layout");
    hk::LightTables t;
    hk::derive_light_tables(d->lights, d->n_lights, s->lbvh, t);
    auto put = [](DevBuf& b, const void* src, size_t bytes, size_t cap) -> hipError_t {
        hipError_t e = b.alloc(cap);
        if (e == hipSuccess) e = hipMemset(b.p, 0, cap);
        if (e == hipSuccess) e = hipMemcpy(b.p, src, bytes, hipMemcpyHostToDevice);
        return e;
    };
    const size_t cap = light_table_capacity(d->n_lights);
    HIP_TRY(put(s->lnodes, t.nodes.data(), t.nodes.size() * sizeof(DLightNode), 2 * cap * sizeof(DLightNode)));
    HIP_TRY(put(s->trails, t.trails.data(), t.trails.size() * 4, cap * 4));
    HIP_TRY(put(s->infinite, t.infinite.data(), t.infinite.size() * 4, cap * 4));
    return HK_OK;
}

int upload_envmaps(hk_scene* s, const hk_scene_desc* d) {
    std::vector<DEnvMap> de(d->n_envmaps > 0 ? d->n_envmaps : 1);
    std::memset(de.data(), 0, de.size() * sizeof(DEnvMap));
    for (int i = 0; i < d->n_envmaps; ++i) {
        const hk_envmap& e = d->envmaps[i];
        auto up = [&](const float* src, size_t n, const float** dst) -> hipError_t {
            DevBuf* b = &s->own();
            hipError_t err = b->upload(src, n * 4);
            *dst = b->as<float>();
            return err;
        };
        DEnvMap& o = de[i];
        const float* texels = nullptr;
        HIP_TRY(up(e.data, (size_t)e.width * e.height * 4, &texels));
        o.data = reinterpret_cast<const float4*>(texels);
        HIP_TRY(up(e.conditional_func, (size_t)e.nu * e.nv, &o.cond_func));
        HIP_TRY(up(e.conditional_cdf, (size_t)(e.nu + 1) * e.nv, &o.cond_cdf));
        HIP_TRY(up(e.conditional_func_int, (size_t)e.nv, &o.cond_func_int));
        HIP_TRY(up(e.marginal_func, (size_t)e.nv, &o.marg_func));
        HIP_TRY(up(e.marginal_cdf, (size_t)e.nv + 1, &o.marg_cdf));
        o.marg_func_int = e.marginal_func_int;
        o.width = e.width, o.height = e.height, o.nu = e.nu, o.nv = e.nv;
        std::memcpy(o.rot, e.rotation, sizeof o.rot);
    }
    HIP_TRY(s->envmaps.upload(de.data(), de.size() * sizeof(DEnvMap)));
    s->h_envmaps.assign(de.begin(), de.begin() + (d->n_envmaps > 0 ? d->n_envmaps : 0));
    return HK_OK;
}

bool nvdb_block_extent(const hk_medium& m, float& bg_probe, int nvb_min[3], int nvb_dim[3]) {
    const unsigned char* B = m.nvdb_bytes;
    bg_probe = hknv::f32(B, m.root_offset_1based + 28);
    int lo[3] = {m.index_bbox_min[0] >> 3, m.index_bbox_min[1] >> 3, m.index_bbox_min[2] >> 3};
    int hi[3] = {m.index_bbox_max[0] >> 3, m.index_bbox_max[1] >> 3, m.index_bbox_max[2] >> 3};
    auto include = [&](long long x0, long long y0, long long z0, long long nblk) {
        long long o[3] = {x0 >> 3, y0 >> 3, z0 >> 3};
        for (int k = 0; k < 3; ++k) {
            if (o[k] < lo[k]) lo[k] = (int)o[k];
            if (o[k] + nblk - 1 > hi[k]) hi[k] = (int)(o[k] + nblk - 1);
        }
    };
    auto sext21 = [](unsigned long long v) { return (long long)((v & 0x100000ull) ? (v | ~0x1fffffull) : v); };
    bool unbounded = false;
    for (int i = 0; i < m.root_table_size; ++i) {
        long long tile = m.root_offset_1based + 64 + (long long)i * 32;
        unsigned long long key = (unsigned long long)hknv::i64(B, tile);
        long long tz = sext21(key & 0x1fffffull) << 12, ty = sext21((key >> 21) & 0x1fffffull) << 12, tx = sext21((key >> 42) & 0x1fffffull) << 12;
        long long child = hknv::i64(B, tile + 8);
        if (child == 0) {
            if (hknv::f32(B, tile + 20) != bg_probe) unbounded = true;
            continue;
        }
        long long upper = m.root_offset_1based + child;
        for (int nu = 0; nu < 32768; ++nu) {
            long long ux = tx + (((nu >> 10) & 31) << 7), uy = ty + (((nu >> 5) & 31) << 7), uz = tz + ((nu & 31) << 7);
            if (!hknv::mask(B, upper + 4128, nu)) {
                if (hknv::f32(B, upper + 8256 + (long long)nu * 8) != bg_probe) include(ux, uy, uz, 16);
                continue;
            }
            long long lower = upper + hknv::i64(B, upper + 8256 + (long long)nu * 8);
            for (int nl = 0; nl < 4096; ++nl) {
                long long lx = ux + (((nl >> 8) & 15) << 3), ly = uy + (((nl >> 4) & 15) << 3), lz = uz + ((nl & 15) << 3);
                if (hknv::mask(B, lower + 544, nl) || hknv::f32(B, lower + 1088 + (long long)nl * 8) != bg_probe) include(lx, ly, lz, 1);
            }
        }
    }
    if (unbounded) return false;
    for (int k = 0; k < 3; ++k) {
        nvb_min[k] = lo[k] - 1;
        nvb_dim[k] = hi[k] - lo[k] + 3;
    }
    return true;
// ... 324 lines not shown
```

hikari.jl_amd/csrc/hk_types.h:

```cpp
#pragma once
#include <hip/hip_runtime.h>
#include <stdint.h>
#include <cstdlib>

namespace hk {
const char* knob(const char* name);
inline bool knob_on(const char* name) {
    const char* e = knob(name);
    return !(e && std::atoi(e) == 0);
}
inline int knob_int(const char* name, int dflt) {
    const char* e = knob(name);
    return e ? std::atoi(e) : dflt;
}
inline int knob_int_in(const char* name, int lo, int hi, int dflt) {
    const int v = knob_int(name, dflt);
    return v >= lo && v <= hi ? v : dflt;
}
}

#define HK_TICKET_COLS 16
#define HK_TICKET_WAYS 64
#define HK_TICKET_STRIDE 64
#define HK_MAX_KINDS 11
// ... 144 lines not shown
    const double q = upper ? ceil(g) + 1.0 : floor(g) - 1.0;
    return (uint32_t)(q < 0.0 ? 0.0 : (q > 65535.0 ? 65535.0 : q));
}
__host__ __device__ inline void hk_quant_node(DQNode& q, const float lo[2][3], const float hi[2][3], const float base[3], const float cell[3]) {
    for (int c = 0; c < 2; ++c)
        for (int k = 0; k < 3; ++k) q.w[3 * c + k] = hk_quant_plane(lo[c][k], base[k], cell[k], false) | (hk_quant_plane(hi[c][k], base[k], cell[k], true) << 16);
}

struct DXform {
    float m[12];
    float nm[9];
    int copy;
};
struct DQGrid {
    float base[3], cell[3];
};

struct DScene {
    const DNode* nodes;
    const DQNode* qnodes;
    float q_base[3], q_cell[3];
    const float4* leaf_tris;
    int root_ref;
    int n_tris;
    int n_nodes;
    int pad_nodes;
    const float* positions;
    const float* normals;
    const float* uvs;
    const float* tangents;
    const DTriMeta* meta;
    const DMaterial* materials;
    const DTexture* textures;
    const DPLSpectrum* spectra;
    const DMediumInterface* mis;
    const DLight* lights;
    int n_lights;
    int n_materials;
    const DLightNode* lnodes;
    const uint32_t* bit_trails;
    const int* infinite_lights;
    int num_bvh_lights, num_infinite_lights;
    const DMedium* media;
    int n_media;
    int media_mask;
    const DEnvMap* envmaps;
    int n_envmaps;
    int has_escape_lights;
    int simple_lights;
    int all_opaque;
    int bvh_depth;
    int all_grey;
    int grey_pool;
    int grey_bricks;
    const float* tri_shade;
};

struct DTables {
    const uint32_t* sobol;
    const float* cie;
    const float* rgb2spec_scale;
    const float* rgb2spec_coeffs;
    int rgb2spec_res;
    const float4* rgb2spec_points;
    int rgb2spec_sorted;
};

struct DFilter {
    int type;
    float rx, ry, p1, p2;
    int nx, ny;
    const float* func;
    const float* marginal_cdf;
    const float* marginal_func;
    const float* conditional_cdf;
    float dmin_x, dmin_y, dmax_x, dmax_y;
    float func_integral;
};

struct DCamera {
    float r2c[16];
    float c2w[16];
    float lens_radius, focal_distance, shutter_open, shutter_close;
};

struct DSobol {
    int log2_spp, n_base4_digits;
    uint32_t seed;
    int width;
    const uint2* hi_table;
    int hi_rows, hi_stride;
    const uint16_t* lo_table;
    int lo_rows, lo_count;
    int lo_offset;
};

enum { Q_RAY = 0, Q_SHADOW = 1, Q_ESCAPED = 2, Q_MEDIUM = 3, Q_SCATTER = 4, Q_MAT0 = 5, Q_COUNT = Q_MAT0 + HK_MAX_KINDS };

#ifndef HK_LAMBDA_BY_SLOT
#define HK_LAMBDA_BY_SLOT 1
#endif
struct DPathGen {
    float4* ray_o;
    float4* ray_d;
    float4* beta;
    float4* r_u;
    float4* r_l;
    float4* lambda;
    uint2* meta;
};

struct DPathState {
    int capacity;
    int n_waves;
    int wave_cap;
    DPathGen gen[2];
    float4* hit;
    int* mat_id;
    uint2* sel_light;
    float4* lambda_s;
    float4* pdf;
    float4* L;
    float* filter_w;
    float4* sh_o;
    float4* sh_d;
    float4* sh_Ld;
    float4* sh_ru;
    float4* sh_rl;
    uint32_t* sh_slot;
    float4* sh_T;
    uint32_t* sh_aux;
    float4* sh_it;
    uint32_t* wq_a;
    uint32_t* wq_b;
    int* wq_ctl;
    uint32_t* escaped_q;
    uint32_t* medium_q;
    uint32_t* scatter_q;
    int* initial_medium;
    uint32_t* mat_q;
    int* counters;
    int* tickets;
    int ticket_rows;
    int* seg_list;
    int* seg_list_n;
    int dynamic_segments;
    int small_pass;
    int ticket_share;
    int compact;
    int meta32, const_origin;
    int sh_final;
    DPathGen gen_cam;
    int view_cache;
};

struct DStats {
    unsigned long long rays_closest, rays_shadow, nodes, tris, hits, vertices, collisions, light_nodes, sh_nodes, sh_tris;
    unsigned long long nvdb_collisions, sh_nvdb_collisions;
    unsigned long long sh_collisions, dda_steps, sh_dda_steps, scatter_vertices, sc_light_nodes;
#ifdef HK_DEBUG_UTIL
    unsigned long long dbg[32];
#endif
};

struct DFrame {
    int width, height, tiles_x, tiles_y;
    int x0, y0, x1, y1;
    int n_pixels_padded;
    int samples_in_pass;
    uint32_t s_mul;
    int s_shr;
    int first_sample, sample_stride;
    int max_depth;
    int regularize;
    float max_component_value;
    int count_nodes;
    int implicit_ones;
    int track_gate;
    int delta_advance;
    int refill_idle;
    int walk_tune;
};

__device__ __forceinline__ float luminance709(float r, float g, float b) { return 0.2126f * r + 0.7152f * g + 0.0722f * b; }
struct PlanarPixels {
    float *rgb, *normal, *depth;
    static constexpr int tap_unroll = 1;
    __device__ __forceinline__ float4 color(long q) const {
        const float r = rgb[3 * q], g = rgb[3 * q + 1], b = rgb[3 * q + 2];
        return make_float4(r, g, b, luminance709(r, g, b));
    }
    __device__ __forceinline__ float4 guide(long q) const { return make_float4(normal[3 * q], normal[3 * q + 1], normal[3 * q + 2], depth[q]); }
    __device__ __forceinline__ bool has_depth() const { return depth != nullptr; }
    __device__ __forceinline__ float depth_at(long q) const { return depth[q]; }
    __device__ __forceinline__ void store_color(long q, float r, float g, float b) const { rgb[3 * q] = r, rgb[3 * q + 1] = g, rgb[3 * q + 2] = b; }
    __device__ __forceinline__ void store_guide(long q, float4 g) const { normal[3 * q] = g.x, normal[3 * q + 1] = g.y, normal[3 * q + 2] = g.z, depth[q] = g.w; }
};
struct PackedPixels {
    float4 *frame, *guides;
    static constexpr int tap_unroll = 5;
    __device__ __forceinline__ float4 color(long q) const { return frame[q]; }
    __device__ __forceinline__ float4 guide(long q) const { return guides[q]; }
    __device__ __forceinline__ bool has_depth() const { return guides != nullptr; }
    __device__ __forceinline__ float depth_at(long q) const { return guides[q].w; }
    __device__ __forceinline__ void store_color(long q, float r, float g, float b) const { frame[q] = make_float4(r, g, b, luminance709(r, g, b)); }
    __device__ __forceinline__ void store_guide(long q, float4 g) const { guides[q] = g; }
};
```

include/hikari_mi355x.h:

```cpp
#ifndef HIKARI_MI355X_H
#define HIKARI_MI355X_H

#include <stdint.h>

#ifdef __cplusplus
extern "C" {
#endif

#define HK_OK 0
#define HK_ERR_INVALID -1
#define HK_ERR_DEVICE -2
#define HK_ERR_UNSUPPORTED -3
#define HK_UNSET -100

typedef struct hk_texture {
    int32_t width, height, channels;
    int32_t kind;
    const float* data;
} hk_texture;

typedef struct hk_tex_rgba {
    float c[4];
    int32_t tex;
} hk_tex_rgba;
// ... 60 lines not shown
enum {
    HK_SPEC_RGB = 0,
    HK_SPEC_ILLUMINANT = 1
};

typedef struct hk_light {
    int32_t kind;
    int32_t spectrum_kind;
    float i_rgb[4];
    float poly[3];
    float illum_scale;
    float scale;
    float position[3];
    float direction[3];
    float world_to_light[16];
    float light_to_world[16];
    float cos_total_width, cos_falloff_start;
    float v[9];
    float normal[3];
    float area;
    float uv[6];
    hk_tex_rgba Le;
    int32_t two_sided;
    int32_t envmap;
} hk_light;

typedef struct hk_envmap {
    int32_t width, height;
    const float* data;
    float rotation[9];
    int32_t nu, nv;
    const float* conditional_func;
    const float* conditional_cdf;
    const float* conditional_func_int;
    const float* marginal_func;
    const float* marginal_cdf;
    float marginal_func_int;
    int32_t _pad;
} hk_envmap;

enum { HK_MEDIUM_HOMOGENEOUS = 0, HK_MEDIUM_GRID = 1, HK_MEDIUM_RGB_GRID = 2, HK_MEDIUM_NANOVDB = 3 };

typedef struct hk_medium {
    int32_t kind;
    float sigma_a[4], sigma_s[4], Le[4];
    float g;
    float sigma_scale, Le_scale;
    float bounds_min[3], bounds_max[3];
    float render_to_medium[16], medium_to_render[16];
    int32_t res[3];
    const float* density;
    const float* sigma_a_grid;
    const float* sigma_s_grid;
    const float* Le_grid;
    int32_t majorant_res[3];
    const float* majorant;
    float max_density;
    const uint8_t* nvdb_bytes;
    int64_t nvdb_size;
    int64_t root_offset_1based, upper_offset_1based, lower_offset_1based, leaf_offset_1based;
    int32_t upper_count, lower_count, leaf_count, root_table_size;
    float inv_mat[9], vec[3];
    int32_t index_bbox_min[3], index_bbox_max[3];
} hk_medium;

typedef struct hk_scene_desc {
    int32_t n_triangles;
    int32_t n_materials;
    int32_t n_textures;
    int32_t n_media_interfaces;
    int32_t n_lights;
    int32_t n_envmaps;
    int32_t n_media;
    int32_t n_spectra;
    const float* positions;
    const float* normals;
    const float* uvs;
    const float* tangents;
    const hk_tri_meta* meta;
    const hk_material* materials;
    const hk_texture* textures;
    const hk_medium_interface* media_interfaces;
    const hk_light* lights;
    const hk_envmap* envmaps;
    const hk_medium* media;
    const hk_pl_spectrum* spectra;
} hk_scene_desc;

typedef struct hk_tables {
    const uint32_t* sobol_matrices;
    int32_t sobol_count;
    int32_t rgb2spec_res;
    const float* cie_x;
    const float* cie_y;
    const float* cie_z;
    const float* rgb2spec_scale;
    const float* rgb2spec_coeffs;
} hk_tables;

enum { HK_FILTER_BOX = 1, HK_FILTER_TRIANGLE = 2, HK_FILTER_GAUSSIAN = 3, HK_FILTER_MITCHELL = 4, HK_FILTER_LANCZOS = 5 };
enum { HK_COHERENCE_NONE = 0, HK_COHERENCE_SORTED = 1, HK_COHERENCE_PER_TYPE = 2 };

typedef struct hk_integrator_params {
    int32_t max_depth;
    int32_t samples_per_pixel;
    int32_t russian_roulette_depth;
    int32_t regularize;
    int32_t material_coherence;
    float max_component_value;
    int32_t filter_type;
    float filter_radius[2];
    float filter_param1;
    float filter_param2;
    int32_t accumulate_f64;
    uint32_t sampler_seed;
    int32_t samples_per_pass;
} hk_integrator_params;

typedef struct hk_camera {
    float raster_to_camera[16];
    float camera_to_world[16];
    float lens_radius, focal_distance;
    float shutter_open, shutter_close;
    float dx_camera[3], dy_camera[3];
} hk_camera;

typedef struct hk_stats {
    uint64_t rays_closest;
    uint64_t rays_shadow;
    uint64_t bvh_nodes_visited;
    uint64_t tris_tested;
    uint64_t hits_accepted;
    uint64_t path_vertices;
    uint64_t medium_collisions;
    uint64_t light_bvh_nodes;
    double seconds_trace;
    double seconds_total;
    uint64_t trace_launches;
    uint64_t trace_nodes, trace_tris;
    uint64_t shadow_nodes, shadow_tris;
    uint64_t shadow_launches, shade_launches;
    double seconds_shadow, seconds_shade, seconds_other;
    uint64_t bytes_algorithmic_trace, bytes_algorithmic_shadow, bytes_algorithmic_shade;
    double seconds_media;
    uint64_t track_collisions, shadow_collisions;
    uint64_t track_dda_steps, shadow_dda_steps;
    uint64_t scatter_vertices;
    uint64_t media_launches;
    uint64_t bytes_algorithmic_media;
    double seconds_select;
    uint64_t select_launches;
    uint64_t fused_passes;
    uint64_t view_cache_hits;
} hk_stats;

typedef struct hk_ctx hk_ctx;
typedef struct hk_scene hk_scene;
typedef struct hk_film hk_film;
typedef struct hk_integrator hk_integrator;

int32_t hk_ctx_create(int32_t device_id, void* stream, hk_ctx** out);
int32_t hk_ctx_destroy(hk_ctx* ctx);
const char* hk_last_error(void);
int32_t hk_ctx_set_tables(hk_ctx* ctx, const hk_tables* tables);
int32_t hk_ctx_set_option(hk_ctx* ctx, const char* name, const char* value);
int32_t hk_ctx_get_option(hk_ctx* ctx, const char* name, char* out, int32_t out_bytes);
int32_t hk_trim_cache(hk_ctx* ctx);

int32_t hk_scene_create(hk_ctx* ctx, const hk_scene_desc* desc, hk_scene** out);
int32_t hk_scene_destroy(hk_scene* scene);

int32_t hk_scene_set_transform(hk_scene* scene, int32_t first_tri, int32_t n_tris, const float* m34);
int32_t hk_scene_update_materials(hk_scene* scene, int32_t first, int32_t n, const hk_material* materials);
int32_t hk_scene_update_lights(hk_scene* scene, int32_t first, int32_t n, const hk_light* lights);
int32_t hk_scene_update_envmap(hk_scene* scene, int32_t idx, const float* data, const float* rotation);
int32_t hk_scene_update_medium(hk_scene* scene, int32_t idx, const hk_medium* medium);

int32_t hk_integrator_create(hk_ctx* ctx, const hk_integrator_params* params, hk_integrator** out);
int32_t hk_integrator_destroy(hk_integrator* integ);

int32_t hk_film_create(hk_ctx* ctx, int32_t width, int32_t height, int32_t f64, void* external_accum, hk_film** out);
int32_t hk_film_destroy(hk_film* film);
int32_t hk_film_clear(hk_film* film);

int32_t hk_render(hk_ctx* ctx, hk_scene* scene, hk_integrator* integ, hk_film* film, const hk_camera* cam,
                  int32_t first_sample_idx, int32_t n_samples, int32_t sample_stride);

int32_t hk_render_tile(hk_ctx* ctx, hk_scene* scene, hk_integrator* integ, hk_film* film, const hk_camera* cam,
                       int32_t first_sample_idx, int32_t n_samples, int32_t sample_stride, int32_t x0, int32_t y0, int32_t x1, int32_t y1);

typedef struct hk_comm hk_comm;
int32_t hk_comm_create(hk_ctx* const* ctxs, int32_t n, hk_comm** out);
int32_t hk_comm_unique_id(uint8_t* id_out128);
int32_t hk_comm_create_rank(hk_ctx* ctx, const uint8_t* id128, int32_t rank, int32_t world, hk_comm** out);
int32_t hk_comm_destroy(hk_comm* comm);
int32_t hk_film_reduce(hk_comm* comm, hk_film* const* films, int32_t n_films, int32_t root);

int32_t hk_film_read_rgb(hk_ctx* ctx, hk_film* film, float* out_hw3);
int32_t hk_film_read_rgb_async(hk_ctx* ctx, hk_film* film);
int32_t hk_film_read_wait(hk_ctx* ctx, hk_film* film, float* out_hw3, const float** frame);
int32_t hk_film_pin_host(hk_film* film, float* host_hw3);
int32_t hk_film_unpin_host(hk_film* film);
int32_t hk_film_read_accum(hk_ctx* ctx, hk_film* film, void* out);
void* hk_film_accum_device_ptr(hk_film* film);

int32_t hk_flush(hk_ctx* ctx);
int32_t hk_sync(hk_ctx* ctx);
int32_t hk_stats_get(hk_ctx* ctx, hk_stats* out);
int32_t hk_stats_reset(hk_ctx* ctx);
int32_t hk_stats_enable_counters(hk_ctx* ctx, int32_t flags);

int32_t hk_trace_closest(hk_ctx* ctx, hk_scene* scene, int32_t n, const float* o3, const float* d3, const float* tmax,
                         float* out_t, int32_t* out_prim, float* out_uv2);
int32_t hk_test_sobol(hk_ctx* ctx, int32_t width, int32_t height, int32_t spp, uint32_t seed, int32_t n,
                      const int32_t* px, const int32_t* py, const int32_t* sample_idx, const int32_t* dim,
                      float* out_1d, float* out_2d);
int32_t hk_test_camera(hk_ctx* ctx, hk_integrator* integ, const hk_camera* cam, int32_t width, int32_t height, int32_t n,
                       const int32_t* px, const int32_t* py, const int32_t* sample_idx, float* out15);
int32_t hk_test_uplift(hk_ctx* ctx, int32_t mode, int32_t n, const float* rgb, const float* lambda, float* out);
int32_t hk_test_light_bvh(hk_ctx* ctx, hk_scene* scene, int32_t n, const float* p3, const float* n3, const float* u,
                          int32_t* out_light, float* out_pmf, const int32_t* query_light, float* out_query_pmf);
enum { HK_TONEMAP_NONE = 0, HK_TONEMAP_REINHARD = 1, HK_TONEMAP_REINHARD_EXT = 2, HK_TONEMAP_ACES = 3, HK_TONEMAP_UNCHARTED2 = 4, HK_TONEMAP_FILMIC = 5 };
typedef struct hk_postprocess_params {
    float exposure;
    int32_t tonemap;
    float inv_gamma;
    int32_t apply_gamma;
    float white_point;
    float imaging_ratio;
    int32_t apply_wb;
    float wb[9];
    int32_t mask_escaped;
    float bg[3];
} hk_postprocess_params;
int32_t hk_film_postprocess(hk_ctx* ctx, hk_film* film, const hk_postprocess_params* params, const float* depth, float* dst_rgb);
int32_t hk_postprocess(hk_ctx* ctx, const hk_postprocess_params* params, int32_t width, int32_t height, const float* src_rgb,
                       const float* depth, float* dst_rgb);

typedef struct hk_denoise_params {
    int32_t iterations;
    float sigma_color;
    float sigma_normal;
    float sigma_depth;
    int32_t use_variance;
} hk_denoise_params;
int32_t hk_denoise(hk_ctx* ctx, const hk_denoise_params* params, int32_t width, int32_t height, const float* src_rgb, const float* normal,
                   const float* depth, float* dst_rgb, float* src_after);

int32_t hk_film_fill_aux(hk_ctx* ctx, hk_scene* scene, const hk_camera* cam, int32_t width, int32_t height, int32_t has_infinite_lights,
                         float* albedo, float* normal, float* depth);

int32_t hk_film_update_aux(hk_ctx* ctx, hk_film* film, hk_scene* scene, const hk_camera* cam, int32_t has_infinite_lights);
int32_t hk_film_read_aux(hk_ctx* ctx, hk_film* film, float* albedo, float* normal, float* depth);
int32_t hk_film_present(hk_ctx* ctx, hk_film* film, const hk_denoise_params* dn, const hk_postprocess_params* pp, float* out_hw3);
int32_t hk_film_present_async(hk_ctx* ctx, hk_film* film, const hk_denoise_params* dn, const hk_postprocess_params* pp);

int32_t hk_test_bsdf(hk_ctx* ctx, hk_scene* scene, int32_t mode, int32_t mat_idx, int32_t regularize, int32_t n, const float* wo,
                     const float* wi, const float* ns, const float* lambda, const float* u, const float* uc, float* out);
int32_t hk_test_light(hk_ctx* ctx, hk_scene* scene, int32_t mode, int32_t light_idx_1based, int32_t n, const float* p3,
                      const float* in3, const float* lambda, float* out);

int32_t hk_test_mix(hk_ctx* ctx, hk_scene* scene, int32_t mat_idx, int32_t n, const float* p3, const float* wo3, const float* uv2,
                    int32_t* out_mat);
int32_t hk_test_medium(hk_ctx* ctx, hk_scene* scene, int32_t mode, int32_t medium_idx, int32_t n, const float* a3, const float* b3,
                       const float* tmax, const float* lambda, float* out);
int32_t hk_test_trace_lean(hk_ctx* ctx, hk_scene* scene, int32_t anyhit, int32_t n, const float* o3, const float* d3, const float* tmax,
                           float* out_t, int32_t* out_prim, float* out_uv2);

int32_t hk_scene_bvh_info(hk_scene* scene, int32_t* n_nodes, int32_t* n_leaf_tris, int32_t* max_depth);
int32_t hk_scene_light_bvh_copy(hk_scene* scene, int32_t* n_nodes, float* nodes_out ,
                                uint32_t* bit_trails );

int32_t hk_scene_medium_copy(hk_scene* scene, int32_t idx, int32_t* n_cells, float* majorant, uint32_t* zero_mask);
int32_t hk_test_medium_bricks(hk_scene* scene, int32_t idx, int32_t* dims, float* out);

#ifdef __cplusplus
}
#endif
#endif
```

Baseline: 10070.

## Add single-material-kind fast path that skips per-kind queue sorting

When a scene has exactly one non-mix material kind, the trace kernel stops classifying hits into per-kind material queues and only writes hit records and escaped rays. The shade kernel then walks the ray queue directly, skipping misses, and optionally compacts the hits when they are sparse. Emission handling is folded into the main shading loop, and segment-list building for material queues is skipped. This removes queue-sorting and writing work plus one indirection, but shade now scans all rays including misses and takes extra LDS per wave.

New measurement: 10940 (median of 6 runs). 1.09x the previous value.

```diff
diff --git a/hikari.jl_amd/_abi.py b/hikari.jl_amd/_abi.py
--- a/hikari.jl_amd/_abi.py
+++ b/hikari.jl_amd/_abi.py
@@ -126,7 +126,7 @@
                 ("track_collisions", C.c_uint64), ("shadow_collisions", C.c_uint64), ("track_dda_steps", C.c_uint64),
                 ("shadow_dda_steps", C.c_uint64), ("scatter_vertices", C.c_uint64), ("media_launches", C.c_uint64),
                 ("bytes_algorithmic_media", C.c_uint64), ("seconds_select", C.c_double), ("select_launches", C.c_uint64),
-                ("fused_passes", C.c_uint64), ("view_cache_hits", C.c_uint64)]
+                ("fused_passes", C.c_uint64), ("view_cache_hits", C.c_uint64), ("one_kind_passes", C.c_uint64)]
 
 
 EXPORTED_SYMBOLS = [
diff --git a/hikari.jl_amd/csrc/hk_ctx.cpp b/hikari.jl_amd/csrc/hk_ctx.cpp
--- a/hikari.jl_amd/csrc/hk_ctx.cpp
+++ b/hikari.jl_amd/csrc/hk_ctx.cpp
@@ -15,7 +15,7 @@
     "HK_MID_LISTS", "HK_MID_PASS_PATHS_M", "HK_NODE_CACHE", "HK_NVDB_DENSE_MB", "HK_OVERLAP", "HK_PIPELINE", "HK_PIPELINE_AFTER", "HK_PIPELINE_MAX_PATHS_M", "HK_PRESELECT",
     "HK_SELECT_MIN_IDLE", "HK_SHADOW_FEED_ROUNDS", "HK_SHADOW_TRACK_BATCH", "HK_SMALL_PASS", "HK_SMALL_PASS_WAVES", "HK_SOBOL_LO_GB", "HK_SOBOL_TABLE_ONLY",
     "HK_STATE_CACHE_GB", "HK_STATE_SLAB", "HK_TICKET_SHARE", "HK_TRACK_ADVANCE", "HK_TRACK_EXTRA_ADVANCE", "HK_TRACK_MIN_PENDING", "HK_TRACK_POOL", "HK_TRACK_REFILL_IDLE",
-    "HK_WALK_POOL", "HK_WALK_REFILL_IDLE", "HK_WALK_SPLIT", "HK_WAVES_PER_CU", "HK_READBACK_PIN", "HK_DEFER_EXTERNAL", "HK_SELECT_POOL", "HK_SMALL_PASS_FUSED", "HK_SMALL_PASS_MERGED", "HK_OCC_SCALE", "HK_ESCAPED_UNROLL", "HK_SHADOW_FINAL", "HK_TRI_PACK", "HK_LEAN_RECORDS", "HK_VIEW_CACHE", "HK_MAJORANT_BLOCK_VOXELS"};
+    "HK_WALK_POOL", "HK_WALK_REFILL_IDLE", "HK_WALK_SPLIT", "HK_WAVES_PER_CU", "HK_READBACK_PIN", "HK_DEFER_EXTERNAL", "HK_SELECT_POOL", "HK_SMALL_PASS_FUSED", "HK_SMALL_PASS_MERGED", "HK_OCC_SCALE", "HK_ESCAPED_UNROLL", "HK_SHADOW_FINAL", "HK_TRI_PACK", "HK_LEAN_RECORDS", "HK_VIEW_CACHE", "HK_MAJORANT_BLOCK_VOXELS", "HK_ONE_KIND"};
 static bool known_knob(const char* name) {
     for (const char* k : KNOB_NAMES)
         if (std::strcmp(k, name) == 0) return true;
@@ -260,7 +260,7 @@
     }
     c->seconds_trace = c->seconds_total = 0.0;
     c->trace_launches = c->shadow_launches = c->shade_launches = c->media_launches = c->select_launches = 0;
-    c->fused_passes = c->view_cache_hits = 0;
+    c->fused_passes = c->view_cache_hits = c->one_kind_passes = 0;
     c->have_span = false;
     return HK_OK;
 }
@@ -354,6 +354,7 @@
     out->select_launches = c->select_launches;
     out->fused_passes = c->fused_passes;
     out->view_cache_hits = c->view_cache_hits;
+    out->one_kind_passes = c->one_kind_passes;
     {
         const uint64_t hits_closest = h.hits < h.rays_closest ? h.hits : h.rays_closest;
         out->bytes_algorithmic_trace = h.rays_closest * (32 + 16) + 64 * h.nodes + 36 * h.tris + 96 * hits_closest;
diff --git a/hikari.jl_amd/csrc/hk_host.h b/hikari.jl_amd/csrc/hk_host.h
--- a/hikari.jl_amd/csrc/hk_host.h
+++ b/hikari.jl_amd/csrc/hk_host.h
@@ -176,6 +176,7 @@
     int count_nodes = 0, time_kernels = 0;
     unsigned long long fused_passes = 0;
     unsigned long long view_cache_hits = 0;
+    unsigned long long one_kind_passes = 0;
     std::vector<std::pair<hipEvent_t, hipEvent_t>> trace_events;
     std::vector<std::pair<hipEvent_t, hipEvent_t>> class_events[6];
     uint64_t shadow_launches = 0, shade_launches = 0, media_launches = 0, select_launches = 0;
@@ -219,6 +220,7 @@
     DevBuf media;
     DScene d{};
     uint32_t kinds_mask = 0;
+    bool has_mix = false;
     int n_materials = 0;
     int bvh_nodes = 0, bvh_leaf_tris = 0, bvh_depth = 0;
     hk::LightBVH lbvh;
diff --git a/hikari.jl_amd/csrc/hk_kernels.hip b/hikari.jl_amd/csrc/hk_kernels.hip
--- a/hikari.jl_amd/csrc/hk_kernels.hip
+++ b/hikari.jl_amd/csrc/hk_kernels.hip
@@ -765,7 +765,7 @@
 
 enum { LR_EMPTY = 0, LR_ACTIVE = 1 };
 
-template <bool COUNT, int NC, bool QN = false, int MIN_IDLE = HK_TRACE_MIN_IDLE>
+template <bool COUNT, int NC, bool QN = false, int MIN_IDLE = HK_TRACE_MIN_IDLE, bool ONE = false>
 __device__ __forceinline__ void trace_lean_body(const DPathState& st, const DScene& sc, int depth, DStats* stats, const SegTickets& src, int* __restrict__ stack, const NodeCache& cache) {
     const int lane = lane_id();
     const unsigned long long lt_mask = (1ull << lane) - 1ull;
@@ -789,6 +789,15 @@
         const unsigned long long run_m = __ballot(state == LR_ACTIVE && r.cur != DONE);
         if (run_m == 0ull || (64 - __popcll(run_m) >= MIN_IDLE && cursor < n)) {
             HK_DBG(8, state == LR_ACTIVE && r.cur == DONE);
+            if constexpr (ONE) {
+                const bool fin = state == LR_ACTIVE && r.cur == DONE;
+                if (fin) {
+                    n_hits += r.best.prim >= 0 ? 1u : 0u;
+                    stream_st(&st.hit[slot], make_float4(r.best.t, __int_as_float(r.best.prim), r.best.u, r.best.v));
+                    state = LR_EMPTY;
+                }
+                wq_push(q_escaped, slot, fin && r.best.prim < 0);
+            } else {
             int kind = -1;
             if (state == LR_ACTIVE && r.cur == DONE) {
                 if (r.best.prim < 0)
@@ -824,6 +833,7 @@
                 for (int kk = 0; kk < HK_MAX_KINDS; ++kk) kind_count[kk] += (kk == k) ? add : 0;
                 pending &= ~m;
             }
+            }
             const unsigned long long want = __ballot(state == LR_EMPTY);
             const int avail = n - cursor;
             const int rank = __popcll(want & lt_mask);
@@ -848,8 +858,12 @@
     wq_close(q_escaped, count_ptr(st, depth, Q_ESCAPED, gw));
     if (lane == 0) {
         *count_ptr(st, depth, Q_MEDIUM, gw) = 0;
+        if constexpr (ONE)
+            *count_ptr(st, depth, Q_MAT0 + st.one_kind - 1, gw) = n - q_escaped.count;
+        else {
 #pragma unroll
-        for (int k = 0; k < HK_MAX_KINDS; ++k) *count_ptr(st, depth, Q_MAT0 + k, gw) = kind_count[k];
+            for (int k = 0; k < HK_MAX_KINDS; ++k) *count_ptr(st, depth, Q_MAT0 + k, gw) = kind_count[k];
+        }
     }
     }
     stats += global_wave();
@@ -861,14 +875,17 @@
     }
     HK_DBG_FLUSH(stats);
 }
-template <bool COUNT, int STACK, int BLOCK = HK_TRACE_BLOCK, int NC = 0, bool QN = false>
+#ifndef HK_CLOSEST_MIN_IDLE_ONE
+#define HK_CLOSEST_MIN_IDLE_ONE 24
+#endif
+template <bool COUNT, int STACK, int BLOCK = HK_TRACE_BLOCK, int NC = 0, bool QN = false, bool ONE = false>
 __global__ void __launch_bounds__(BLOCK) k_trace_lean(DPathState st, DScene sc, int depth, DStats* stats) {
     __shared__ int lds_stack[(BLOCK / 64) * STACK * 64];
     __shared__ float4 lds_box[NC > 0 ? 3 * NC : 1];
     __shared__ int2 lds_child[NC > 0 ? NC : 1];
     int* stack = lds_stack + (threadIdx.x >> 6) * (STACK * 64);
     const NodeCache cache = node_cache_fill<NC, BLOCK, QN>(sc, lds_box, lds_child);
-    trace_lean_body<COUNT, NC, QN, (NC >= 1024 ? HK_CLOSEST_MIN_IDLE_LDS : HK_TRACE_MIN_IDLE)>(st, sc, depth, stats, seg_open(st, ticket_ptr(st, depth, TK_TRACE), st.dynamic_segments != 0, depth, Q_RAY), stack, cache);
+    trace_lean_body<COUNT, NC, QN, (NC >= 1024 ? (ONE ? HK_CLOSEST_MIN_IDLE_ONE : HK_CLOSEST_MIN_IDLE_LDS) : HK_TRACE_MIN_IDLE), ONE>(st, sc, depth, stats, seg_open(st, ticket_ptr(st, depth, TK_TRACE), st.dynamic_segments != 0, depth, Q_RAY), stack, cache);
 }
 
 #ifndef HK_REFILL_MIN_IDLE
@@ -2339,14 +2356,14 @@
 #ifndef HK_SHADE_MIN_WAVES
 #define HK_SHADE_MIN_WAVES 1
 #endif
-template <int KIND, bool SIMPLE, bool FT, bool PRE>
+template <int KIND, bool SIMPLE, bool FT, bool PRE, bool ONE = false>
 __device__ __forceinline__ void shade_body(const DPathState& st, const DScene& sc, const DTables& T, const DFrame& fr, const DSobol& sob, int depth, int first_kind, DStats* stats, const SegTickets& src,
                                            uint32_t* __restrict__ elist) {
     const int lane = lane_id();
     unsigned n_vertices = 0, n_lnodes = 0;
     HK_FOR_EACH_SEGMENT_FROM(gw, st, src) {
     const uint32_t* __restrict__ queue = st.mat_q + ((size_t)KIND * st.n_waves + gw) * st.wave_cap;
-    const int n = *count_ptr(st, depth, Q_MAT0 + KIND, gw);
+    const int n = *count_ptr(st, depth, ONE ? Q_RAY : Q_MAT0 + KIND, gw);
     const DPathGen g = gen_at(st, depth), gn = st.gen[(depth + 1) & 1];
     const size_t seg = (size_t)gw * st.wave_cap;
     const bool ones = depth == 0 && fr.implicit_ones;
@@ -2355,8 +2372,18 @@
         q_shadow.count = *count_ptr(st, depth, Q_SHADOW, gw);
         q_next.count = *count_ptr(st, depth + 1, Q_RAY, gw);
     }
-    {
-        int n_emit = 0;
+    int n_emit = 0;
+    auto drain_emit = [&]() {
+        __builtin_amdgcn_fence(__ATOMIC_SEQ_CST, "wavefront");
+        const int take = n_emit < 64 ? n_emit : 64;
+        if (lane < take) shade_emission<KIND == HK_MAT_MATTE, SIMPLE>(st, g, ones, sc, T, elist[lane], n_lnodes, depth, seg);
+        const int rest = n_emit - take;
+        const uint32_t moved = lane < rest ? elist[64 + lane] : 0u;
+        __builtin_amdgcn_fence(__ATOMIC_SEQ_CST, "wavefront");
+        if (lane < rest) elist[lane] = moved;
+        n_emit = rest;
+    };
+    if constexpr (!ONE) {
         for (int base = 0; base < n || n_emit > 0; base += 64) {
             if (base < n) {
                 const int i = base + lane;
@@ -2367,25 +2394,43 @@
                 n_emit += __popcll(m);
                 if (n_emit < 64 && base + 64 < n) continue;
             }
-            __builtin_amdgcn_fence(__ATOMIC_SEQ_CST, "wavefront");
-            const int take = n_emit < 64 ? n_emit : 64;
-            if (lane < take) shade_emission<KIND == HK_MAT_MATTE, SIMPLE>(st, g, ones, sc, T, elist[lane], n_lnodes, depth, seg);
-            const int rest = n_emit - take;
-            const uint32_t moved = lane < rest ? elist[64 + lane] : 0u;
-            __builtin_amdgcn_fence(__ATOMIC_SEQ_CST, "wavefront");
-            if (lane < rest) elist[lane] = moved;
-            n_emit = rest;
-        }
-    }
-    for (int base = 0; base < n; base += 64) {
+            drain_emit();
+        }
+    }
+    uint32_t* __restrict__ wlist = elist + 128;
+    const bool sparse = ONE && 8 * *count_ptr(st, depth, Q_MAT0 + KIND, gw) < 7 * n;
+    int n_work = 0;
+    for (int base = 0; base < n || n_work > 0; base += 64) {
         int i = base + lane;
         bool active = i < n;
-        uint32_t slot = active ? queue[i] : 0u;
-        bool push_shadow = false, push_ray = false;
+        uint32_t slot = ONE ? (uint32_t)seg + (uint32_t)i : (active ? queue[i] : 0u);
+        if (sparse) {
+            if (base < n) {
+                const bool hit = active && reinterpret_cast<const int*>(st.hit)[4 * (size_t)slot + 1] >= 0;
+                const unsigned long long m = __ballot(hit);
+                if (hit) wlist[n_work + __popcll(m & ((1ull << lane) - 1ull))] = slot;
+                n_work += __popcll(m);
+                if (n_work < 64 && base + 64 < n) continue;
+            }
+            __builtin_amdgcn_fence(__ATOMIC_SEQ_CST, "wavefront");
+            const int take = n_work < 64 ? n_work : 64, rest = n_work - take;
+            active = lane < take;
+            slot = active ? wlist[lane] : 0u;
+            const uint32_t moved = lane < rest ? wlist[64 + lane] : 0u;
+            __builtin_amdgcn_fence(__ATOMIC_SEQ_CST, "wavefront");
+            if (lane < rest) wlist[lane] = moved;
+            n_work = rest;
+        }
+        bool push_shadow = false, push_ray = false, emits = false;
         float4 H = make_float4(0, 0, 0, 0);
+        if constexpr (ONE) {
+            if (active) H = stream_ld(&st.hit[slot]);
+            active = active && __float_as_int(H.y) >= 0;
+        }
         Surface sf;
         v3 wo = mk3(0, 0, 1);
         DTriMeta meta{0u, 0u, 0u};
+        auto mat_index = [&]() -> int { return ONE ? sc.mis[meta.mi].material : (st.mat_id[slot] & ~HK_MAT_EMISSIVE_BIT); };
         S4 lambda = s4(0.0f), beta = s4(0.0f), r_u = s4(0.0f), kd_matte = s4(0.0f);
         uint32_t fl = 0, pslot = 0;
         int pdepth = 0, medium = -1;
@@ -2396,7 +2441,7 @@
         S4 shLd = s4(0.0f), shRu = s4(0.0f), shRl = s4(0.0f);
         if (active) {
             ++n_vertices;
-            H = stream_ld(&st.hit[slot]);
+            if constexpr (!ONE) H = stream_ld(&st.hit[slot]);
             float4 O = ld_ray_o(st, g, slot, depth, seg), D = stream_ld(&g.ray_d[slot]);
             v3 ro = mk3(O.x, O.y, O.z), rd = mk3(D.x, D.y, D.z);
             float t_hit = H.x;
@@ -2404,6 +2449,7 @@
             sf = surface_at(sc, prim, H.z, H.w, ro, rd, t_hit);
             wo = -rd;
             meta = tri_meta(sc, prim);
+            if constexpr (ONE) emits = meta.arealight > 0;
             const uint2 pmeta = ld_meta(st, g, slot, depth);
             lambda = ld_lambda(st, g, slot, pmeta.y);
             if (ones)
@@ -2423,7 +2469,7 @@
             split_slot(fr, pslot, pix, k);
             sctx = sobol_ctx_slot(sob, T.sobol, fr.x0, fr.y0, fr.tiles_x, pix, k, fr.first_sample + k * fr.sample_stride);
 
-            if (KIND == HK_MAT_MATTE) kd_matte = matte_kd<SIMPLE>(sc, T, sc.materials[st.mat_id[slot] & ~HK_MAT_EMISSIVE_BIT], TexCtx(sf.uv, meta.prim_index, H.z, H.w), lambda);
+            if (KIND == HK_MAT_MATTE) kd_matte = matte_kd<SIMPLE>(sc, T, sc.materials[mat_index()], TexCtx(sf.uv, meta.prim_index, H.z, H.w), lambda);
 #ifdef HK_ABLATE
             {
                 float sink = 0.0f;
@@ -2453,7 +2499,7 @@
                 if (HK_ABLATE == 4) {
                     S4 l2 = lambda;
                     asm volatile("" : "+v"(l2.x), "+v"(l2.y), "+v"(l2.z), "+v"(l2.w));
-                    S4 k2 = matte_kd(sc, T, sc.materials[st.mat_id[slot] & ~HK_MAT_EMISSIVE_BIT], TexCtx(sf.uv, meta.prim_index, H.z, H.w), l2);
+                    S4 k2 = matte_kd(sc, T, sc.materials[mat_index()], TexCtx(sf.uv, meta.prim_index, H.z, H.w), l2);
                     sink = k2.x + k2.y + k2.z + k2.w;
                 }
                 if (HK_ABLATE == 5) {
@@ -2467,7 +2513,7 @@
                     asm volatile("" : "+v"(w2.x), "+v"(w2.y), "+v"(w2.z));
                     float p2;
                     S4 f2 = eval_matte_kd(kd_matte, w2, sf.n, sf.ns, p2);
-                    BSDFSample s2 = sample_matte_kd(sc, sc.materials[st.mat_id[slot] & ~HK_MAT_EMISSIVE_BIT], kd_matte, w2, sf.ns, TexCtx(sf.uv, meta.prim_index, H.z, H.w), mk2(H.z, H.w));
+                    BSDFSample s2 = sample_matte_kd(sc, sc.materials[mat_index()], kd_matte, w2, sf.ns, TexCtx(sf.uv, meta.prim_index, H.z, H.w), mk2(H.z, H.w));
                     sink = f2.x + f2.w + p2 + s2.pdf + s2.wi.x + s2.f.y;
                 }
                 asm volatile("" : : "v"(sink));
@@ -2475,7 +2521,7 @@
 #endif
 
             if (sc.n_lights > 0) {
-                const DMaterial& mat = sc.materials[st.mat_id[slot] & ~HK_MAT_EMISSIVE_BIT];
+                const DMaterial& mat = sc.materials[mat_index()];
                 float light_pmf;
                 int light_idx;
                 if constexpr (PRE) {
@@ -2546,7 +2592,7 @@
         if (active) {
             int new_depth = pdepth + 1;
             if (new_depth < fr.max_depth) {
-                const DMaterial& mat = sc.materials[st.mat_id[slot] & ~HK_MAT_EMISSIVE_BIT];
+                const DMaterial& mat = sc.materials[mat_index()];
                 const DMediumInterface mi = sc.mis[meta.mi];
                 float uc = (KIND == HK_MAT_GLASS || KIND > HK_MAT_CONDUCTOR) && KIND != HK_MAT_FALLBACK ? sobol_1d<FT>(sctx, base_dim + 4) : 0.0f;
                 v2 u = (KIND == HK_MAT_MIRROR || KIND == HK_MAT_GLASS || KIND == HK_MAT_THIN_DIELECTRIC) ? mk2(0.0f, 0.0f) : sobol_2d<FT>(sctx, base_dim + 6);
@@ -2591,7 +2637,15 @@
                 st_meta(st, gn, pn, nflags, pslot);
             }
         }
-    }
+        if constexpr (ONE) {
+            const unsigned long long m = __ballot(emits);
+            if (emits) elist[n_emit + __popcll(m & ((1ull << lane) - 1ull))] = slot;
+            n_emit += __popcll(m);
+            if (n_emit >= 64) drain_emit();
+        }
+    }
+    if constexpr (ONE)
+        if (n_emit > 0) drain_emit();
     if (lane == 0) {
         *count_ptr(st, depth, Q_SHADOW, gw) = q_shadow.count;
         *count_ptr(st, depth + 1, Q_RAY, gw) = q_next.count;
@@ -2601,11 +2655,11 @@
     wave_add(&stats->vertices, n_vertices);
     wave_add(&stats->light_nodes, n_lnodes);
 }
-template <int KIND, bool SIMPLE = false, bool FT = false, bool PRE = false>
+template <int KIND, bool SIMPLE = false, bool FT = false, bool PRE = false, bool ONE = false>
 __global__ void __attribute__((amdgpu_flat_work_group_size(256, 256), amdgpu_waves_per_eu(ShadeWaves<KIND>::value))) k_shade(DPathState st, DScene sc, DTables T, DFrame fr, DSobol sob, int depth, int first_kind, DStats* stats) {
-    __shared__ uint32_t emit_list[4 * 128];
-    shade_body<KIND, SIMPLE, FT, PRE>(st, sc, T, fr, sob, depth, first_kind, stats, seg_open(st, ticket_ptr(st, depth, TK_SHADE0 + KIND), st.dynamic_segments != 0, depth, Q_MAT0 + KIND),
-                                      emit_list + (threadIdx.x >> 6) * 128);
+    __shared__ uint32_t emit_list[4 * (ONE ? 256 : 128)];
+    shade_body<KIND, SIMPLE, FT, PRE, ONE>(st, sc, T, fr, sob, depth, first_kind, stats, seg_open(st, ticket_ptr(st, depth, TK_SHADE0 + KIND), st.dynamic_segments != 0, depth, ONE ? Q_RAY : Q_MAT0 + KIND),
+                                      emit_list + (threadIdx.x >> 6) * (ONE ? 256 : 128));
 }
 
 template <class W> HKD W wone();
diff --git a/hikari.jl_amd/csrc/hk_launch.h b/hikari.jl_amd/csrc/hk_launch.h
--- a/hikari.jl_amd/csrc/hk_launch.h
+++ b/hikari.jl_amd/csrc/hk_launch.h
@@ -10,6 +10,7 @@
 bool grey_compact_ok(const DScene& sc);
 bool preselect_lights(const DScene& sc, const DPathState& st);
 bool small_pass_fusable(const DScene& sc, uint32_t kinds_mask);
+int one_kind_of(const DScene& sc, uint32_t kinds_mask, bool has_mix, const DPathState& st);
 
 void launch_camera(hipStream_t s, int n_cu, const DPathState& st, const DFrame& fr, const DTables& T, const DFilter& flt, const DCamera& cam, const DSobol& sob, int initial_medium);
 void launch_trace(hipStream_t s, int n_cu, const DPathState& st, const DScene& sc, const DTables& T, const DFrame& fr, int depth, DStats* stats);
diff --git a/hikari.jl_amd/csrc/hk_launch_impl.h b/hikari.jl_amd/csrc/hk_launch_impl.h
--- a/hikari.jl_amd/csrc/hk_launch_impl.h
+++ b/hikari.jl_amd/csrc/hk_launch_impl.h
@@ -120,7 +120,9 @@
     if (lean_scene(sc)) {
         lean_dispatch<1024, 1536, HK_TRACE_NC32>(sc, fr, [&](auto COUNT, auto STACK, auto BLOCK, auto NC, auto QN) {
             constexpr int block = decltype(BLOCK)::value;
-            launch_resident<k_trace_lean<decltype(COUNT)::value, decltype(STACK)::value, block, decltype(NC)::value, decltype(QN)::value>>(s, n_cu, st, block, 8, sc, depth, stats);
+            with_bool(st.one_kind != 0, [&](auto ONE) {
+                launch_resident<k_trace_lean<decltype(COUNT)::value, decltype(STACK)::value, block, decltype(NC)::value, decltype(QN)::value, decltype(ONE)::value>>(s, n_cu, st, block, 8, sc, depth, stats);
+            });
         });
         return;
     }
@@ -231,6 +233,17 @@
 bool preselect_lights(const DScene& sc, const DPathState& st) {
     return sc.n_media == 0 && sc.num_bvh_lights >= HK_PRESELECT_MIN && st.sel_light != nullptr && knob_on("HK_PRESELECT");
 }
+#ifndef HK_ONE_KIND_DEFAULT
+#define HK_ONE_KIND_DEFAULT 1
+#endif
+int one_kind_of(const DScene& sc, uint32_t kinds_mask, bool has_mix, const DPathState& st) {
+    if (knob_int("HK_ONE_KIND", HK_ONE_KIND_DEFAULT) == 0) return 0;
+    if (!lean_scene(sc) || !st.meta32 || has_mix || preselect_lights(sc, st)) return 0;
+    if (kinds_mask == 0 || (kinds_mask & (kinds_mask - 1)) != 0) return 0;
+    int kind = 0;
+    while (!(kinds_mask & (1u << kind))) ++kind;
+    return kind < HK_MAX_KINDS ? kind + 1 : 0;
+}
 void launch_light_select(hipStream_t s, int n_cu, const DPathState& st, const DScene& sc, const DTables& T, const DFrame& fr, const DSobol& sob, int depth, uint32_t kinds_mask, DStats* stats) {
     const int min_idle = knob_int_in("HK_SELECT_MIN_IDLE", 1, 64, HK_SELECT_MIN_IDLE);
     const bool pool = knob_on("HK_SELECT_POOL");
@@ -242,7 +255,12 @@
 }
 void launch_shade(hipStream_t s, int n_cu, int kind, const DPathState& st, const DScene& sc, const DTables& T, const DFrame& fr, const DSobol& sob, int depth, int first_kind, DStats* stats) {
     auto shade = [&](auto KIND, auto SIMPLE, auto FT, auto PRE) {
-        launch_resident<k_shade<decltype(KIND)::value, decltype(SIMPLE)::value, decltype(FT)::value, decltype(PRE)::value>>(s, n_cu, st, 256, 8, sc, T, fr, sob, depth, first_kind, stats);
+        constexpr int k = decltype(KIND)::value;
+        constexpr bool simple = decltype(SIMPLE)::value, ft = decltype(FT)::value, pre = decltype(PRE)::value;
+        if constexpr (pre)
+            launch_resident<k_shade<k, simple, ft, true>>(s, n_cu, st, 256, 8, sc, T, fr, sob, depth, first_kind, stats);
+        else
+            with_bool(st.one_kind == kind + 1, [&](auto ONE) { launch_resident<k_shade<k, simple, ft, false, decltype(ONE)::value>>(s, n_cu, st, 256, 8, sc, T, fr, sob, depth, first_kind, stats); });
     };
     const bool ft = sobol_tables_cover(sob, depth);
     const bool light_kind = kind == HK_MAT_MATTE || kind == HK_MAT_MIRROR || kind == HK_MAT_GLASS || kind == HK_MAT_CONDUCTOR;
diff --git a/hikari.jl_amd/csrc/hk_render.cpp b/hikari.jl_amd/csrc/hk_render.cpp
--- a/hikari.jl_amd/csrc/hk_render.cpp
+++ b/hikari.jl_amd/csrc/hk_render.cpp
@@ -508,10 +508,10 @@
     int lists(std::initializer_list<std::pair<int, int>> dq, bool kinds_of_depth = false, int kd = 0) {
         int dd[HK_MAX_KINDS + 6], qq[HK_MAX_KINDS + 6], n = 0;
         for (auto& e : dq) dd[n] = e.first, qq[n] = e.second, ++n;
-        if (kinds_of_depth)
+        if (kinds_of_depth && !I->st.one_kind)
             for (int kind = 0; kind < HK_MAX_KINDS; ++kind)
                 if (sc->kinds_mask & (1u << kind)) dd[n] = kd, qq[n] = Q_MAT0 + kind, ++n;
-        if (I->st.small_pass) return HK_OK;
+        if (I->st.small_pass || n == 0) return HK_OK;
         return timed(3, [&] { hk::launch_segment_lists(s, I->st, n, dd, qq); });
     }
     int enqueue_depth(ShadowStream& sh, int depth);
@@ -611,6 +611,8 @@
     const bool fused = !c->time_kernels && !piped && hk::launch_small_pass(s, c->n_cu, I->st, sc->d, c->tables, fr, I->filter, dc, sob, I->p.max_depth, sc->kinds_mask, dstats, true, nullptr, 0);
     const int vm = fused ? 0 : view_mode;
     I->st.view_cache = vm;
+    I->st.one_kind = fused ? 0 : hk::one_kind_of(sc->d, sc->kinds_mask, sc->has_mix, I->st);
+    if (I->st.one_kind) c->one_kind_passes++;
     I->st.gen_cam = vm ? I->cam_gen : I->st.gen[0];
     const std::string view_key = vm ? view_key_of() : std::string();
     const bool view_hit = vm && I->view_key == view_key;
diff --git a/hikari.jl_amd/csrc/hk_scene.cpp b/hikari.jl_amd/csrc/hk_scene.cpp
--- a/hikari.jl_amd/csrc/hk_scene.cpp
+++ b/hikari.jl_amd/csrc/hk_scene.cpp
@@ -305,6 +305,7 @@
     for (int i = 0; i < d->n_materials; ++i) {
         bake_material(r2s, d->materials[i], dm[i]);
         if (dm[i].kind != HK_MAT_MIX) s->kinds_mask |= 1u << dm[i].kind;
+        else s->has_mix = true;
     }
     s->n_materials = d->n_materials;
     HIP_TRY(s->materials.upload(dm.data(), dm.size() * sizeof(DMaterial)));
diff --git a/hikari.jl_amd/csrc/hk_types.h b/hikari.jl_amd/csrc/hk_types.h
--- a/hikari.jl_amd/csrc/hk_types.h
+++ b/hikari.jl_amd/csrc/hk_types.h
@@ -320,6 +320,7 @@
     int sh_final;
     DPathGen gen_cam;
     int view_cache;
+    int one_kind;
 };
 
 struct DStats {
diff --git a/include/hikari_mi355x.h b/include/hikari_mi355x.h
--- a/include/hikari_mi355x.h
+++ b/include/hikari_mi355x.h
@@ -236,6 +236,7 @@
     uint64_t select_launches;
     uint64_t fused_passes;
     uint64_t view_cache_hits;
+    uint64_t one_kind_passes;
 } hk_stats;
 
 typedef struct hk_ctx hk_ctx;
```
